# ymartin101/RTS

Hardware: AMD Instinct MI355X
Metric: Mrays/s (primary+bounces) & ms/pulse, 100k-tri scene (higher is better)
Workload: dtype f64

## Files before the change

include/rts_amd.h:

```cpp
#ifndef RTS_AMD_H
#define RTS_AMD_H

#include <stdint.h>
#include "rts_prd.h"

#ifdef __cplusplus
extern "C" {
#endif

typedef struct RtsContext* RtsHandle;

enum {
    RTS_OK = 0,
    RTS_ERR_INVALID = 1,
    RTS_ERR_NO_DEVICE = 2,
    RTS_ERR_HIP = 3,
    RTS_ERR_UNSUPPORTED = 4,
    RTS_ERR_CAPACITY = 5,
    RTS_ERR_IO = 6
};

typedef struct RtsParams {
    uint32_t width;
    uint32_t max_refl;
    uint32_t max_refr;
    uint32_t interpolate_smooth;
    int32_t device;
    uint32_t flags;
} RtsParams;

#define RTS_FLAG_KEEP_ALL_RAYS 1u
#define RTS_FLAG_DEVICE_BUILD 4u
#define RTS_FLAG_HOST_BUILD 16u
#define RTS_FLAG_NO_PREFILTER 8u
#define RTS_FLAG_NO_HORIZON 32u
#define RTS_FLAG_COUNT_TRAVERSAL 2u

typedef struct RtsMesh {
    const uint32_t* triangles;
    const double* vertices;
    const double* normals;
    uint32_t n_triangles, n_vertices, n_normals;
    uint32_t reserved;
    double refl_coeff;
    double refr_index;
} RtsMesh;

typedef struct RtsTargetMotion {
    double position[3];
    double velocity[3];
    double rotation[9];
    int32_t has_rotation;
    int32_t reserved;
} RtsTargetMotion;

typedef struct RtsReceiverSphere {
    double centre[3];
    double radius;
    double min_theta, max_theta, min_phi, max_phi;
} RtsReceiverSphere;

typedef struct RtsPulse {
    double ray_origin[3];
    double tx_span[3];
    double tx_dir[2];
    uint64_t ray_first;
    uint64_t ray_count;
    const RtsTargetMotion* motion;
    uint32_t interleave_tile, interleave_parts, interleave_part, reserved;
} RtsPulse;
#define RTS_INTERLEAVE_LIST 0xffffffffu

typedef struct RtsStats {
    uint64_t rays;
    uint64_t segments;
    uint64_t shaded;
    uint64_t received;
    uint64_t node_visits;
    uint64_t tri_tests;
    uint32_t n_prims, n_nodes;
    float ms_scene;
    float ms_trace;
    float ms_compact;
    float ms_aggregate;
    uint32_t bvh_rebuilt;
    uint32_t stack_overflows;
    uint64_t walked_segments;
    uint32_t coop_tiles;
    uint32_t cost_records_dropped;
} RtsStats;

typedef struct RtsResponse {
    uint64_t ray;
    int32_t rx;
    uint32_t n;
    double power, delay, doppler, phase;
} RtsResponse;

#define RTS_MAX_DEPTH 16
typedef struct RtsGroup {
    int32_t rx;
    uint32_t direct;
    int32_t path[RTS_MAX_DEPTH];
    uint64_t min_ray;
    double n, sum_sqrt_power, sum_delay, sum_phase, sum_doppler;
} RtsGroup;

int rts_create(const RtsParams* params, RtsHandle* out);
int rts_destroy(RtsHandle h);
const char* rts_last_error(void);
const char* rts_build_id(void);
int rts_bind_host_to_device(int device, int* numa_node);
int rts_device_count(int* n);

int rts_set_scene(RtsHandle h, const RtsMesh* meshes, uint32_t n_targets);
int rts_set_receivers(RtsHandle h, const RtsReceiverSphere* rx, uint32_t n_rx);
int rts_share_scene(RtsHandle dst, RtsHandle src);
typedef struct RtsSceneInfo {
    uint32_t n_targets, n_prims, n_nodes, n_leaves;
    uint32_t handles_sharing;
    uint32_t builder;
    double build_ms;
    uint64_t shared_device_bytes;
    uint64_t handle_device_bytes;
    uint64_t version_bytes;
    uint64_t horizon_bytes;
} RtsSceneInfo;
int rts_scene_info(RtsHandle h, RtsSceneInfo* out);
int rts_get_horizon(RtsHandle h, float* out, uint32_t capacity_prims);

int rts_trace_pulse(RtsHandle h, const RtsPulse* pulse);

int rts_reserve(RtsHandle h, uint64_t n_rays);
int rts_trace_pulse_begin(RtsHandle h, const RtsPulse* pulse);
int rts_trace_pulse_end(RtsHandle h);
int rts_link_handles(RtsHandle a, RtsHandle b);
int rts_get_stats(RtsHandle h, RtsStats* out);
int rts_get_block_timeline(RtsHandle h, double* out, uint32_t n);

int rts_get_lane_stats(RtsHandle h, uint64_t* out3);
int rts_get_walk_stats(RtsHandle h, uint64_t* out, uint32_t n);
int rts_received_count(RtsHandle h, uint64_t* count);
int rts_get_received(RtsHandle h, struct PerRayData* rays, int32_t* paths, double* rcs_angles, uint64_t* slots,
                     uint64_t capacity);

int rts_received_prefetch(RtsHandle h);
int rts_received_view(RtsHandle h, const struct PerRayData** rays, const int32_t** paths, const double** rcs_angles, const uint64_t** slots,
                      uint64_t* count);
int rts_finalise_values(RtsHandle h, const double* power, const double* doppler, uint64_t count);
int rts_aggregated_view(RtsHandle h, const double** power, const double** doppler, const double** delay, const double** phase,
                        const int32_t** path_match, uint64_t* count);

int rts_get_all_rays(RtsHandle h, struct PerRayData* results, int32_t* targ_intersect, double* rcs_angle,
                     int32_t* hit_prim, float* hit_t, uint64_t capacity);

int rts_finalise_uniform(RtsHandle h, const double* rcs_per_target, double wavelength, double gt, double gr,
                         double carrier, double cspeed);

int rts_trace_pulse_end_uniform(RtsHandle h, const double* rcs_per_target, double wavelength, double gt, double gr,
                                double carrier, double cspeed, int32_t cube_pulse, uint64_t recv_index_base);

#define RTS_PATTERN_CONSTANT 0u
#define RTS_PATTERN_SEPARABLE 1u
#define RTS_PATTERN_GRID 2u
#define RTS_PATTERN_ABS_U 1u
#define RTS_PATTERN_ABS_V 2u
#define RTS_PATTERN_MAX_AXIS 65536u
#define RTS_PATTERN_MAX_GRID 4194304u
typedef struct RtsPattern {
    uint32_t kind;
    uint32_t flags;
    uint32_t n_u, n_v;
    double scale;
    const double* u_samples;
    const double* u_values;
    const double* v_samples;
    const double* v_values;
    double u0, du, v0, dv;
    const double* grid;
    uint64_t reserved[2];
} RtsPattern;
typedef struct RtsPatternPulse {
    double wavelength, carrier, cspeed;
    const double* rx_position;
    const double* rx_rotation;
} RtsPatternPulse;
int rts_set_patterns(RtsHandle h, const RtsPattern* tx, const RtsPattern* rx, uint32_t n_rx, const RtsPattern* rcs,
                     uint32_t n_targets);
int rts_finalise_patterns(RtsHandle h, const RtsPatternPulse* pulse);
int rts_trace_pulse_end_patterns(RtsHandle h, const RtsPatternPulse* pulse, int32_t cube_pulse, uint64_t recv_index_base);
int rts_pattern_eval(const RtsPattern* p, const double* u, const double* v, uint32_t n, double* out);

#define RTS_BASE_USE_ROWS 0xffffffffffffffffULL
int rts_aggregate(RtsHandle h, double cspeed, double carrier, uint64_t recv_index_base);
int rts_group_count(RtsHandle h, uint32_t* count);
int rts_get_groups(RtsHandle h, RtsGroup* groups, uint32_t capacity);
int rts_get_aggregated(RtsHandle h, struct PerRayData* rays, double* delay, double* phase, int32_t* path_match,
                       uint64_t capacity);

int rts_merge_groups(const RtsGroup* in, uint32_t n_in, uint32_t depth, RtsGroup* out, uint32_t* n_out);
int rts_groups_to_responses(const RtsGroup* groups, uint32_t n_groups, RtsResponse* out, uint32_t capacity,
                            uint32_t* n_out);

typedef struct RtsCubeParams {
    uint32_t n_rx, n_pulses, n_bins, reserved;
    double t0, dt;
} RtsCubeParams;
int rts_cube_attach(RtsHandle h, const RtsCubeParams* params, void* device_ptr);
int rts_cube_accumulate(RtsHandle h, uint32_t pulse_index, double cspeed, double carrier);
int rts_cube_get(RtsHandle h, double* host_out, uint64_t capacity_doubles);
int rts_cube_accumulate_paths(RtsHandle h, uint32_t pulse_index);
int rts_cube_doppler(RtsHandle h, uint32_t n_fft, void* device_out);
// ... 413 lines not shown
```

rts_amd/_lib.py:

```python
import ctypes as C
import os
import subprocess

import numpy as np

_HERE = os.path.dirname(os.path.abspath(__file__))
LIB_PATH = os.environ.get("RTS_AMD_LIB", os.path.join(_HERE, "librts_amd.so"))
CSRC = os.path.join(_HERE, "csrc")

RTS_OK, RTS_ERR_INVALID, RTS_ERR_NO_DEVICE, RTS_ERR_HIP, RTS_ERR_UNSUPPORTED, RTS_ERR_CAPACITY, RTS_ERR_IO = range(7)
RTS_FLAG_KEEP_ALL_RAYS = 1
RTS_FLAG_COUNT_TRAVERSAL = 2
RTS_FLAG_DEVICE_BUILD = 4
RTS_FLAG_HOST_BUILD = 16
RTS_FLAG_NO_PREFILTER = 8
RTS_FLAG_NO_HORIZON = 32
RTS_MAX_DEPTH = 16
RTS_BASE_USE_ROWS = 0xffffffffffffffff

PRD_DTYPE = np.dtype({
    "names": ["rayLength", "refrIndex", "reflDepth", "refrDepth", "maxRayIndex", "rayDirection",
              "firstHitPoint", "prevHitPoint", "power", "doppler", "received", "end"],
    "formats": ["<f8", ("<f8", 2), "<u4", "<u4", "<u4", ("<f8", 3), ("<f8", 3), ("<f8", 3), "<f8", "<f8", "<i4", "u1"],
    "offsets": [0, 16, 32, 36, 40, 48, 72, 96, 120, 128, 136, 140],
    "itemsize": 144,
})


class RtsParams(C.Structure):
    _fields_ = [("width", C.c_uint32), ("max_refl", C.c_uint32), ("max_refr", C.c_uint32),
                ("interpolate_smooth", C.c_uint32), ("device", C.c_int32), ("flags", C.c_uint32)]


class RtsMesh(C.Structure):
    _fields_ = [("triangles", C.c_void_p), ("vertices", C.c_void_p), ("normals", C.c_void_p),
                ("n_triangles", C.c_uint32), ("n_vertices", C.c_uint32), ("n_normals", C.c_uint32),
                ("reserved", C.c_uint32), ("refl_coeff", C.c_double), ("refr_index", C.c_double)]


class RtsTargetMotion(C.Structure):
    _fields_ = [("position", C.c_double * 3), ("velocity", C.c_double * 3), ("rotation", C.c_double * 9),
                ("has_rotation", C.c_int32), ("reserved", C.c_int32)]


class RtsReceiverSphere(C.Structure):
    _fields_ = [("centre", C.c_double * 3), ("radius", C.c_double), ("min_theta", C.c_double),
                ("max_theta", C.c_double), ("min_phi", C.c_double), ("max_phi", C.c_double)]


class RtsPulse(C.Structure):
    _fields_ = [("ray_origin", C.c_double * 3), ("tx_span", C.c_double * 3), ("tx_dir", C.c_double * 2),
                ("ray_first", C.c_uint64), ("ray_count", C.c_uint64), ("motion", C.POINTER(RtsTargetMotion)),
                ("interleave_tile", C.c_uint32), ("interleave_parts", C.c_uint32), ("interleave_part", C.c_uint32), ("reserved", C.c_uint32)]


class RtsCubeParams(C.Structure):
    _fields_ = [("n_rx", C.c_uint32), ("n_pulses", C.c_uint32), ("n_bins", C.c_uint32), ("reserved", C.c_uint32),
                ("t0", C.c_double), ("dt", C.c_double)]


class RtsPlanItem(C.Structure):
    _fields_ = [("pulse", C.c_uint32), ("interleave_tile", C.c_uint32), ("interleave_parts", C.c_uint32), ("interleave_part", C.c_uint32),
                ("ray_first", C.c_uint64), ("ray_count", C.c_uint64)]


RTS_SHARD_PULSES, RTS_SHARD_RAYS, RTS_SHARD_PULSES_WHOLE = 0, 1, 2


RTS_PATTERN_CONSTANT, RTS_PATTERN_SEPARABLE, RTS_PATTERN_GRID = 0, 1, 2
RTS_PATTERN_ABS_U, RTS_PATTERN_ABS_V = 1, 2
RTS_PATTERN_MAX_AXIS, RTS_PATTERN_MAX_GRID = 65536, 4194304


class RtsPattern(C.Structure):
    _fields_ = [("kind", C.c_uint32), ("flags", C.c_uint32), ("n_u", C.c_uint32), ("n_v", C.c_uint32), ("scale", C.c_double),
                ("u_samples", C.c_void_p), ("u_values", C.c_void_p), ("v_samples", C.c_void_p), ("v_values", C.c_void_p),
                ("u0", C.c_double), ("du", C.c_double), ("v0", C.c_double), ("dv", C.c_double), ("grid", C.c_void_p),
                ("reserved", C.c_uint64 * 2)]


class RtsPatternPulse(C.Structure):
    _fields_ = [("wavelength", C.c_double), ("carrier", C.c_double), ("cspeed", C.c_double),
                ("rx_position", C.c_void_p), ("rx_rotation", C.c_void_p)]


RTS_RENDER_RAYS, RTS_RENDER_PATHS = 0, 1
RTS_RENDER_DOPPLER = 1
RTS_WAVEFORM_MAX_SAMPLES, RTS_WAVEFORM_MAX_TAPS, RTS_COMPRESS_MAX_BINS = 4096, 64, 8192


class RtsWaveform(C.Structure):
    _fields_ = [("samples", C.c_void_p), ("n_samples", C.c_uint32), ("taps", C.c_uint32), ("reserved", C.c_uint64 * 2)]


RTS_CFAR_CA, RTS_CFAR_GO, RTS_CFAR_SO = 0, 1, 2
RTS_CFAR_LOCAL_MAX = 1
RTS_CFAR_MAX_HALF, RTS_CFAR_DEFAULT_MAX_DETECTIONS = 16, 65536


# ... 186 lines not shown

class RtsEigParams(C.Structure):
    _fields_ = [("n", C.c_uint32), ("reserved0", C.c_uint32), ("device_cov", C.c_void_p), ("reserved", C.c_uint64 * 2)]


class RtsDoaScanParams(C.Structure):
    _fields_ = [("n", C.c_uint32), ("first_vector", C.c_uint32), ("m", C.c_uint32), ("flags", C.c_uint32), ("n_dirs", C.c_uint64),
                ("g", C.c_void_p), ("device_steering", C.c_void_p), ("device_vectors", C.c_void_p), ("reserved", C.c_uint64 * 2)]


assert C.sizeof(RtsEigParams) == 32 and C.sizeof(RtsDoaScanParams) == 64


class RtsSceneInfo(C.Structure):
    _fields_ = [("n_targets", C.c_uint32), ("n_prims", C.c_uint32), ("n_nodes", C.c_uint32), ("n_leaves", C.c_uint32),
                ("handles_sharing", C.c_uint32), ("builder", C.c_uint32), ("build_ms", C.c_double),
                ("shared_device_bytes", C.c_uint64), ("handle_device_bytes", C.c_uint64), ("version_bytes", C.c_uint64),
                ("horizon_bytes", C.c_uint64)]


class RtsStats(C.Structure):
    _fields_ = [("rays", C.c_uint64), ("segments", C.c_uint64), ("shaded", C.c_uint64), ("received", C.c_uint64),
                ("node_visits", C.c_uint64), ("tri_tests", C.c_uint64), ("n_prims", C.c_uint32), ("n_nodes", C.c_uint32),
                ("ms_scene", C.c_float), ("ms_trace", C.c_float), ("ms_compact", C.c_float), ("ms_aggregate", C.c_float),
                ("bvh_rebuilt", C.c_uint32), ("stack_overflows", C.c_uint32), ("walked_segments", C.c_uint64), ("coop_tiles", C.c_uint32), ("cost_records_dropped", C.c_uint32)]


RESPONSE_DTYPE = np.dtype([("ray", "<u8"), ("rx", "<i4"), ("n", "<u4"), ("power", "<f8"), ("delay", "<f8"),
                           ("doppler", "<f8"), ("phase", "<f8")])
GROUP_DTYPE = np.dtype([("rx", "<i4"), ("direct", "<u4"), ("path", "<i4", (RTS_MAX_DEPTH,)), ("min_ray", "<u8"),
                        ("n", "<f8"), ("sum_sqrt_power", "<f8"), ("sum_delay", "<f8"), ("sum_phase", "<f8"),
                        ("sum_doppler", "<f8")])
assert RESPONSE_DTYPE.itemsize == 48 and GROUP_DTYPE.itemsize == 120


def is_stale():
    if not os.path.exists(LIB_PATH):
        return True
    try:
        return build_id() != source_hash()
    except (OSError, AttributeError):
        return True


def source_hash():
    import hashlib
    names = sorted(f for f in os.listdir(CSRC) if f.endswith((".hip", ".cpp", ".h")) and f != "rts_build_id.h")
    h = hashlib.sha256()
    for path in [os.path.join(CSRC, f) for f in names] + [os.path.join(_HERE, "..", "include", f) for f in ("rts_amd.h", "rts_prd.h")]:
        with open(path, "rb") as f:
            h.update(f.read())
    return h.hexdigest()[:16]


def build_id(path=None):
    L = C.CDLL(path or LIB_PATH)
    L.rts_build_id.restype = C.c_char_p
    return L.rts_build_id().decode()


def require_built():
    if not os.path.exists(LIB_PATH):
        raise SystemExit("librts_amd.so is not built: run `python __graft_entry__.py` (or make -C rts_amd/csrc) first")
    if "RTS_AMD_LIB" not in os.environ:
        have, want = build_id(), source_hash()
        if have != want:
            raise SystemExit("librts_amd.so is stale: built from sources %s, the tree is %s -- run `python __graft_entry__.py` first" % (have, want))


def build(force=False, verbose=False):
    if force or is_stale():
        cmd = ["make", "-C", CSRC, "-j", "5"] + ([] if verbose else ["-s"])
        subprocess.check_call(cmd)
    return LIB_PATH


_lib = None

EXPORTS = ["rts_create", "rts_destroy", "rts_last_error", "rts_device_count", "rts_set_scene", "rts_share_scene", "rts_scene_info", "rts_set_receivers",
           "rts_trace_pulse", "rts_reserve", "rts_trace_pulse_begin", "rts_trace_pulse_end", "rts_link_handles", "rts_get_stats", "rts_get_block_timeline", "rts_received_count", "rts_get_received", "rts_get_all_rays",
           "rts_finalise_uniform", "rts_trace_pulse_end_uniform", "rts_aggregate", "rts_group_count", "rts_get_groups", "rts_get_aggregated",
           "rts_merge_groups", "rts_groups_to_responses", "rts_kernel_wrapper", "rts_vertex_rotation",
           "rts_rotation_matrix", "rts_rect_mesh", "rts_sphere_mesh", "rts_file_mesh", "rts_rx_sphere", "rts_get_bvh",
           "rts_build_id", "rts_bind_host_to_device", "rts_get_lane_stats", "rts_get_walk_stats", "rts_get_horizon", "rts_self_test_math", "rts_cube_attach", "rts_cube_accumulate", "rts_cube_get", "rts_cube_accumulate_paths", "rts_cube_doppler", "rts_cube_doppler_get", "rts_plan_cpi", "rts_cube_reduce", "rts_kernel_wrapper_on",
           "rts_received_prefetch", "rts_received_view", "rts_finalise_values", "rts_aggregated_view", "rts_build_hierarchy_host",
           "rts_tile_records_get", "rts_tile_records_set", "rts_deal_tiles", "rts_set_tile_list",
           "rts_set_patterns", "rts_finalise_patterns", "rts_trace_pulse_end_patterns", "rts_pattern_eval",
           "rts_cube_set_waveform", "rts_cube_render", "rts_cube_compress", "rts_waveform_eval",
           "rts_cube_add_noise", "rts_noise_eval", "rts_cube_add_sources", "rts_sources_eval", "rts_cube_detect", "rts_cube_detections_get",
           "rts_cube_detect_os", "rts_cfar_os_alpha", "rts_cfar_os_eval",
           "rts_cube_plots", "rts_cube_plots_get", "rts_plots_eval",
           "rts_cube_track", "rts_cube_tracks_get", "rts_cube_tracks_set", "rts_cube_tracks_reset", "rts_cube_track_rounds", "rts_tracks_eval",
           "rts_cube_tbd_step", "rts_cube_tbd_extract", "rts_cube_tbd_tracks_get", "rts_cube_tbd_paths_get", "rts_cube_tbd_merit_get", "rts_cube_tbd_ring_get",
           "rts_cube_tbd_info", "rts_cube_tbd_reset", "rts_tbd_step_eval", "rts_tbd_extract_eval",
           "rts_cube_backproject", "rts_cube_image_get", "rts_backproject_eval",
           "rts_cube_spectrogram", "rts_cube_spectrogram_get", "rts_stft_eval", "rts_window_make",
           "rts_cube_render_beat", "rts_beat_eval", "rts_cube_range_transform", "rts_cube_range_get", "rts_range_eval",
           "rts_cube_beamform", "rts_cube_beam_get", "rts_beamform_eval", "rts_steering_make",
           "rts_cube_covariance", "rts_cube_covariance_get", "rts_covariance_eval", "rts_cube_mvdr", "rts_cube_mvdr_get", "rts_mvdr_eval",
           "rts_cube_st_covariance", "rts_st_covariance_eval", "rts_cube_st_apply", "rts_cube_st_get", "rts_st_apply_eval", "rts_st_steering_make",
           "rts_cube_eig", "rts_cube_eig_get", "rts_eig_eval", "rts_cube_doa_scan", "rts_cube_doa_get", "rts_doa_scan_eval", "rts_doa_weights", "rts_source_count"]


def lib():
    global _lib
    if _lib is not None:
        return _lib
    if not os.path.exists(LIB_PATH):
        raise RuntimeError("librts_amd.so is not built (run `make -C rts_amd/csrc` or __graft_entry__.build()); "
                           "there is no Python/CPU fallback for the RTS hot path")
    L = C.CDLL(LIB_PATH)
    vp, u32, u64, dbl, i32 = C.c_void_p, C.c_uint32, C.c_uint64, C.c_double, C.c_int32
    L.rts_last_error.restype = C.c_char_p
    sig = {
        "rts_create": [C.POINTER(RtsParams), C.POINTER(vp)],
        "rts_destroy": [vp],
        "rts_device_count": [C.POINTER(C.c_int)],
        "rts_set_scene": [vp, C.POINTER(RtsMesh), u32],
        "rts_share_scene": [vp, vp],
        "rts_scene_info": [vp, C.POINTER(RtsSceneInfo)],
        "rts_set_receivers": [vp, C.POINTER(RtsReceiverSphere), u32],
        "rts_trace_pulse": [vp, C.POINTER(RtsPulse)],
        "rts_reserve": [vp, u64],
        "rts_trace_pulse_begin": [vp, C.POINTER(RtsPulse)],
        "rts_get_block_timeline": [vp, vp, u32],
        "rts_trace_pulse_end": [vp],
        "rts_link_handles": [vp, vp],
        "rts_get_stats": [vp, C.POINTER(RtsStats)],
        "rts_received_count": [vp, C.POINTER(u64)],
        "rts_get_received": [vp, vp, vp, vp, vp, u64],
        "rts_get_all_rays": [vp, vp, vp, vp, vp, vp, u64],
        "rts_finalise_uniform": [vp, vp, dbl, dbl, dbl, dbl, dbl],
        "rts_build_hierarchy_host": [vp, vp, u32, dbl, vp, u32, vp, u32, C.POINTER(u32), C.POINTER(u32), C.POINTER(C.c_int32)],
        "rts_received_prefetch": [vp],
        "rts_received_view": [vp, C.POINTER(vp), C.POINTER(vp), C.POINTER(vp), C.POINTER(vp), C.POINTER(u64)],
        "rts_finalise_values": [vp, vp, vp, u64],
        "rts_aggregated_view": [vp, C.POINTER(vp), C.POINTER(vp), C.POINTER(vp), C.POINTER(vp), C.POINTER(vp), C.POINTER(u64)],
        "rts_aggregate": [vp, dbl, dbl, u64],
        "rts_trace_pulse_end_uniform": [vp, vp, dbl, dbl, dbl, dbl, dbl, C.c_int32, u64],
        "rts_group_count": [vp, C.POINTER(u32)],
        "rts_get_groups": [vp, vp, u32],
        "rts_get_aggregated": [vp, vp, vp, vp, vp, u64],
        "rts_merge_groups": [vp, u32, u32, vp, C.POINTER(u32)],
        "rts_groups_to_responses": [vp, u32, vp, u32, C.POINTER(u32)],
        "rts_kernel_wrapper": [vp, vp, C.c_uint, C.c_uint, C.c_uint, C.c_uint, dbl, dbl, vp, vp, vp, vp, vp, vp],
        "rts_kernel_wrapper_on": [vp, vp, vp, C.c_uint, C.c_uint, C.c_uint, C.c_uint, dbl, dbl, vp, vp, vp, vp, vp, vp],
        "rts_vertex_rotation": [vp, u32, C.c_float, C.c_float, C.c_float],
        "rts_rotation_matrix": [C.c_float, C.c_float, C.c_float, vp],
        "rts_rect_mesh": [C.c_float] * 6 + [vp, vp, vp],
        "rts_sphere_mesh": [u32, C.c_float, C.c_float, C.c_float, C.c_float, vp, C.POINTER(u32), vp, C.POINTER(u32), vp],
        "rts_file_mesh": [C.c_char_p, C.c_char_p, C.c_float, C.c_float, C.c_float, vp, vp, vp, C.POINTER(u32)],
        "rts_rx_sphere": [vp, dbl, dbl, dbl, dbl, dbl, C.POINTER(RtsReceiverSphere)],
        "rts_get_bvh": [vp, vp, vp, vp, u32, u32, vp],
        "rts_cube_attach": [vp, C.POINTER(RtsCubeParams), vp],
        "rts_cube_accumulate": [vp, u32, dbl, dbl],
        "rts_cube_get": [vp, vp, u64], "rts_get_lane_stats": [vp, vp], "rts_get_walk_stats": [vp, vp, C.c_uint32], "rts_get_horizon": [vp, vp, u32], "rts_bind_host_to_device": [C.c_int, C.POINTER(C.c_int)],
        "rts_cube_accumulate_paths": [vp, u32], "rts_cube_doppler": [vp, u32, vp], "rts_cube_doppler_get": [vp, vp, u64],
        "rts_plan_cpi": [u64, u32, u32, u32, u32, u32, u32, vp, u32, C.POINTER(u32)],
        "rts_cube_reduce": [vp, u32, C.c_int],
        "rts_tile_records_get": [vp, vp, u32], "rts_tile_records_set": [vp, vp, u32], "rts_deal_tiles": [vp, u32, u64, u32, u32, vp, vp], "rts_set_tile_list": [vp, u32, vp, u32],
        "rts_self_test_math": [vp, vp, vp, vp, vp, vp, vp, vp, u32],
        "rts_set_patterns": [vp, C.POINTER(RtsPattern), C.POINTER(RtsPattern), u32, C.POINTER(RtsPattern), u32],
        "rts_finalise_patterns": [vp, C.POINTER(RtsPatternPulse)],
        "rts_trace_pulse_end_patterns": [vp, C.POINTER(RtsPatternPulse), C.c_int32, u64],
        "rts_pattern_eval": [C.POINTER(RtsPattern), vp, vp, u32, vp],
        "rts_cube_set_waveform": [vp, C.POINTER(RtsWaveform)],
        "rts_cube_render": [vp, u32, u32, u32, C.c_double, C.c_double],
        "rts_cube_compress": [vp, u32, u32],
        "rts_waveform_eval": [C.POINTER(RtsWaveform), vp, u32, vp],
        "rts_cube_add_noise": [vp, u32, u32, C.c_double, u64],
        "rts_noise_eval": [u64, vp, u32, C.c_double, vp],
        "rts_cube_add_sources": [vp, C.POINTER(RtsSourceParams)],
        "rts_sources_eval": [C.POINTER(RtsCubeParams), C.POINTER(RtsSourceParams), vp],
        "rts_cube_detect": [vp, C.POINTER(RtsCfarParams), vp, u32],
        "rts_cube_detections_get": [vp, vp, u32, C.POINTER(u32)],
        "rts_cube_detect_os": [vp, C.POINTER(RtsCfarOsParams), vp, u32],
        "rts_cfar_os_alpha": [u32, u32, C.c_double, C.POINTER(C.c_double)],
        "rts_cfar_os_eval": [C.POINTER(RtsCubeParams), vp, u32, C.POINTER(RtsCfarOsParams), vp, u32, C.POINTER(u32)],
        "rts_cube_plots": [vp, C.POINTER(RtsPlotParams)],
        "rts_cube_plots_get": [vp, vp, u32, C.POINTER(u32)],
        "rts_plots_eval": [C.POINTER(RtsCubeParams), vp, u32, u32, C.POINTER(RtsPlotParams), vp, u32, C.POINTER(u32)],
        "rts_cube_track": [vp, C.POINTER(RtsTrackParams), C.c_double],
        "rts_cube_tracks_get": [vp, vp, u32, C.POINTER(u32), C.POINTER(u64)],
        "rts_cube_tracks_set": [vp, vp, u32, u64, C.c_double],
        "rts_cube_tracks_reset": [vp],
        "rts_cube_track_rounds": [vp, C.POINTER(u32)],
        "rts_tracks_eval": [C.POINTER(RtsTrackParams), vp, u32, u64, C.c_double, vp, u32, vp, u32, C.POINTER(u32), C.POINTER(u64)],
        "rts_cube_tbd_step": [vp, C.POINTER(RtsTbdParams), C.c_double, vp, u32],
        "rts_cube_tbd_extract": [vp, C.POINTER(RtsTbdExtractParams)],
        "rts_cube_tbd_tracks_get": [vp, vp, u32, C.POINTER(u32)],
        "rts_cube_tbd_paths_get": [vp, vp, u32],
        "rts_cube_tbd_merit_get": [vp, vp, u64],
        "rts_cube_tbd_ring_get": [vp, vp, vp, u32, C.POINTER(u32)],
        "rts_cube_tbd_info": [vp, C.POINTER(u32 * 4), C.POINTER(u64)],
        "rts_cube_tbd_reset": [vp],
        "rts_tbd_step_eval": [C.POINTER(RtsCubeParams), vp, u32, vp, C.POINTER(RtsTbdParams), C.c_double, vp, vp, vp],
        "rts_tbd_extract_eval": [C.POINTER(RtsCubeParams), u32, C.POINTER(RtsTbdParams), vp, vp, vp, u32, C.POINTER(RtsTbdExtractParams), vp, vp, u32, C.POINTER(u32)],
        "rts_cube_backproject": [vp, C.POINTER(RtsImageParams), vp],
        "rts_cube_image_get": [vp, vp, u64],
        "rts_backproject_eval": [C.POINTER(RtsCubeParams), vp, C.POINTER(RtsImageParams), vp],
        "rts_cube_spectrogram": [vp, C.POINTER(RtsStftParams), vp, C.POINTER(u32)],
        "rts_cube_spectrogram_get": [vp, vp, u64],
        "rts_stft_eval": [C.POINTER(RtsCubeParams), vp, C.POINTER(RtsStftParams), vp, C.POINTER(u32)],
        "rts_window_make": [u32, u32, vp],
        "rts_cube_render_beat": [vp, u32, C.POINTER(RtsBeatParams), C.c_double, C.c_double],
        "rts_beat_eval": [C.POINTER(RtsCubeParams), C.POINTER(RtsBeatParams), vp, u32, u32, vp],
        "rts_cube_range_transform": [vp, C.POINTER(RtsRangeParams), vp],
        "rts_cube_range_get": [vp, vp, u64],
        "rts_range_eval": [C.POINTER(RtsCubeParams), vp, C.POINTER(RtsRangeParams), vp],
        "rts_cube_beamform": [vp, C.POINTER(RtsBeamParams), vp],
        "rts_cube_beam_get": [vp, vp, u64],
        "rts_beamform_eval": [C.POINTER(RtsCubeParams), vp, u32, C.POINTER(RtsBeamParams), vp],
        "rts_steering_make": [vp, u32, vp, u32, C.c_double, vp, vp],
        "rts_cube_covariance": [vp, C.POINTER(RtsCovParams), vp],
        "rts_cube_covariance_get": [vp, vp, u64],
        "rts_covariance_eval": [C.POINTER(RtsCubeParams), vp, u32, C.POINTER(RtsCovParams), vp],
        "rts_cube_mvdr": [vp, C.POINTER(RtsMvdrParams), vp],
        "rts_cube_mvdr_get": [vp, vp, u64],
        "rts_mvdr_eval": [vp, u32, C.POINTER(RtsMvdrParams), vp],
        "rts_cube_st_covariance": [vp, C.POINTER(RtsStCovParams), vp],
        "rts_st_covariance_eval": [C.POINTER(RtsCubeParams), vp, u32, C.POINTER(RtsStCovParams), vp],
        "rts_cube_st_apply": [vp, C.POINTER(RtsStApplyParams), vp],
        "rts_cube_st_get": [vp, vp, u64],
        "rts_st_apply_eval": [C.POINTER(RtsCubeParams), vp, u32, C.POINTER(RtsStApplyParams), vp],
        "rts_st_steering_make": [vp, u32, u32, vp, u32, u32, vp, vp],
        "rts_cube_eig": [vp, C.POINTER(RtsEigParams), vp, vp],
        "rts_cube_eig_get": [vp, vp, vp, u64, u64],
        "rts_eig_eval": [vp, u32, vp, vp, C.POINTER(u32)],
        "rts_cube_doa_scan": [vp, C.POINTER(RtsDoaScanParams), vp],
        "rts_cube_doa_get": [vp, vp, u64],
        "rts_doa_scan_eval": [vp, vp, u32, u32, vp, u64, u32, vp],
        "rts_doa_weights": [u32, vp, u32, u32, C.c_double, C.POINTER(u32), C.POINTER(u32), vp, C.POINTER(u32)],
        "rts_source_count": [vp, u32, u64, u32, C.POINTER(u32)],
    }
    for name, args in sig.items():
        fn = getattr(L, name, None)
        if fn is None:
            continue
        fn.argtypes = args
# ... 19 lines not shown
```

rts_amd/api.py:

```python
import ctypes as C

import numpy as np

from . import _lib as L
from ._lib import PRD_DTYPE, RESPONSE_DTYPE, GROUP_DTYPE, check, ptr


def rect_mesh(w, h, d, yaw=0.0, pitch=0.0, roll=0.0):
    v = np.zeros((8, 3)); t = np.zeros((12, 3), np.uint32); n = np.zeros((12, 3))
    check(L.lib().rts_rect_mesh(w, h, d, yaw, pitch, roll, ptr(v), ptr(t), ptr(n)))
    return v, t, n


def sphere_mesh(subdivisions, radius, yaw=0.0, pitch=0.0, roll=0.0):
    nv = C.c_uint32(); nt = C.c_uint32()
    check(L.lib().rts_sphere_mesh(subdivisions, radius, yaw, pitch, roll, None, C.byref(nv), None, C.byref(nt), None))
    v = np.zeros((nv.value, 3)); t = np.zeros((nt.value, 3), np.uint32); n = np.zeros((nv.value, 3))
    check(L.lib().rts_sphere_mesh(subdivisions, radius, yaw, pitch, roll, ptr(v), C.byref(nv), ptr(t), C.byref(nt), ptr(n)))
    return v, t, n


def file_mesh(v_file, n_file, yaw=0.0, pitch=0.0, roll=0.0):
    nt = C.c_uint32(0)
    check(L.lib().rts_file_mesh(v_file.encode(), n_file.encode(), yaw, pitch, roll, None, None, None, C.byref(nt)))
# ... 600 lines not shown


def doa_weights(method, values, n_sources=0, loading=0.0):
    values = np.ascontiguousarray(np.asarray(values, np.float64).ravel())
    first, m, flags = C.c_uint32(0), C.c_uint32(0), C.c_uint32(0); g = np.zeros(max(len(values), 1), np.float64)
    check(L.lib().rts_doa_weights(_DOA_METHODS.get(method, method), ptr(values), len(values), int(n_sources), float(loading),
                                  C.byref(first), C.byref(m), ptr(g), C.byref(flags)))
    return first.value, g[:m.value].copy(), bool(flags.value & L.RTS_DOA_INVERSE)


def source_count(values, K, criterion="mdl"):
    values = np.ascontiguousarray(np.asarray(values, np.float64).ravel())
    k = C.c_uint32(0)
    check(L.lib().rts_source_count(ptr(values), len(values), int(K), {"aic": L.RTS_DOA_AIC, "mdl": L.RTS_DOA_MDL}.get(criterion, criterion), C.byref(k)))
    return k.value


def _st_cov_params(taps, source, first, count, first_bin, n_bins, skip, device_in, n_rows_in):
    c = _cov_params(source, first, count, first_bin, n_bins, skip, device_in, n_rows_in)
    p = L.RtsStCovParams()
    for name in ("source", "n_rows_in", "first_row", "n_rows", "first_bin", "n_bins", "skip_first_bin", "skip_n_bins", "device_in"):
        setattr(p, name, getattr(c, name))
    p.n_taps = int(taps)
    return p


def st_covariance_eval(inp, taps, first=0, count=None, first_bin=0, n_bins=None, skip=None):
    inp = np.ascontiguousarray(np.asarray(inp, np.complex128))
    n_rx, rows, nb = inp.shape
    q = L.RtsCubeParams(n_rx, rows, nb, 0, 0.0, 1.0)
    p = _st_cov_params(taps, "cube", first, count, first_bin, n_bins, skip, None, 0)
    D = n_rx * max(int(taps), 0)
    out = np.zeros((D, D), np.complex128)
    check(L.lib().rts_st_covariance_eval(C.byref(q), ptr(inp.view(np.float64)), rows, C.byref(p), ptr(out.view(np.float64))))
    return out


def _st_apply_params(weights, taps, n_rx, source, first, count, power, device_in, n_rows_in):
    w = np.ascontiguousarray(np.asarray(weights, np.complex128))
    if w.ndim != 2 or w.shape[1] != int(taps) * n_rx:
        raise ValueError("st_apply: weights of shape %s for %d taps of %d receivers ([n_filters][taps n_rx])" % (w.shape, taps, n_rx))
    p = L.RtsStApplyParams()
    p.n_filters, p.source, p.n_taps = w.shape[0], _BEAM_SOURCES.get(source, source), int(taps)
    p.first_row, p.n_rows, p.n_rows_in = int(first), int(count or 0), int(n_rows_in)
    p.flags = L.RTS_BEAM_POWER if power else 0
    p.weights = ptr(w.view(np.float64))
    p.device_in = device_in if device_in else None
    return p, w


def st_apply_eval(inp, weights, taps, first=0, count=None, power=False):
    inp = np.ascontiguousarray(np.asarray(inp, np.complex128))
    n_rx, rows, nb = inp.shape
    q = L.RtsCubeParams(n_rx, rows, nb, 0, 0.0, 1.0)
    p, keep = _st_apply_params(weights, taps, n_rx, "cube", first, count, power, None, 0)
    out = _beam_out(p.n_filters, (p.n_rows if p.n_rows else rows - p.first_row) - p.n_taps + 1, nb, power, False)
    check(L.lib().rts_st_apply_eval(C.byref(q), ptr(inp.view(np.float64)), rows, C.byref(p), ptr(out.view(np.float64))))
    return out


def st_steering(spatial, dopplers, taps, tap_taper=None):
    a = np.ascontiguousarray(np.atleast_2d(np.asarray(spatial, np.complex128)))
    f = np.ascontiguousarray(np.asarray(dopplers, np.float64).ravel())
    t = None if tap_taper is None else np.ascontiguousarray(np.asarray(tap_taper, np.float64).ravel())
    if t is not None and len(t) != int(taps):
        raise ValueError("st_steering: a taper of %d values for %d taps" % (len(t), taps))
    out = np.zeros((a.shape[0] * len(f), max(int(taps), 0) * a.shape[1]), np.complex128)
    check(L.lib().rts_st_steering_make(ptr(a.view(np.float64)), a.shape[1], a.shape[0], ptr(f), len(f), int(taps), ptr(t), ptr(out.view(np.float64))))
    return out


def device_count():
    n = C.c_int(0)
    rc = L.lib().rts_device_count(C.byref(n))
    return n.value if rc == 0 else 0


import os as _os
_PY_LAP = {} if _os.environ.get("RTS_PY_LAP") == "1" else None


class Tracer:

    def __init__(self, width, max_refl, max_refr=0, smooth=True, device=0, keep_all=False, count_traversal=False, device_build=None, pre_filter=True, horizon=True):
        p = L.RtsParams(width, max_refl, max_refr, 1 if smooth else 0, device,
                        (L.RTS_FLAG_KEEP_ALL_RAYS if keep_all else 0) | (L.RTS_FLAG_COUNT_TRAVERSAL if count_traversal else 0) |
                        (0 if device_build is None else (L.RTS_FLAG_DEVICE_BUILD if device_build else L.RTS_FLAG_HOST_BUILD)) |
                         (0 if pre_filter else L.RTS_FLAG_NO_PREFILTER) | (0 if horizon else L.RTS_FLAG_NO_HORIZON))
        self.h = C.c_void_p()
        check(L.lib().rts_create(C.byref(p), C.byref(self.h)))
        self.width = width; self.max_refl = max_refl; self.depth = max_refl + (2 if max_refr else 0)
        self.n_targets = 0; self.keep_all = keep_all; self.device = device
        self._keep = []

    def close(self):
        if self.h:
            L.lib().rts_destroy(self.h); self.h = C.c_void_p()

    def __del__(self):
        try:
            self.close()
        except Exception:
            pass

    def set_scene(self, meshes):
        arr = (L.RtsMesh * max(len(meshes), 1))()
        keep = []
        for i, m in enumerate(meshes):
            t = np.ascontiguousarray(m["tris"], np.uint32); v = np.ascontiguousarray(m["verts"], np.float64)
            n = np.ascontiguousarray(m["normals"], np.float64)
            keep += [t, v, n]
            arr[i] = L.RtsMesh(t.ctypes.data, v.ctypes.data, n.ctypes.data, t.shape[0], v.shape[0], n.shape[0], 0,
                               float(m.get("refl_coeff", 1.0)), float(m.get("refr_index", 1.0)))
        check(L.lib().rts_set_scene(self.h, arr, len(meshes)))
        self.n_targets = len(meshes)

    def horizon(self, n_prims):
        out = np.zeros((int(n_prims), 2), np.float32)
        check(L.lib().rts_get_horizon(self.h, ptr(out), int(n_prims)))
        return out

    def walk_stats(self):
        ls = (C.c_uint64 * 11)()
        check(L.lib().rts_get_walk_stats(self.h, ls, 11))
        return [int(v) for v in ls]

    def share_scene(self, other):
        check(L.lib().rts_share_scene(self.h, other.h))
        self.n_targets = other.n_targets

    def scene_info(self):
        s = L.RtsSceneInfo()
        check(L.lib().rts_scene_info(self.h, C.byref(s)))
        return {k: getattr(s, k) for k, _ in L.RtsSceneInfo._fields_}

    def set_receivers(self, spheres):
        arr = (L.RtsReceiverSphere * max(len(spheres), 1))()
        for i, s in enumerate(spheres):
            arr[i] = L.RtsReceiverSphere((C.c_double * 3)(*s["centre"]), s["radius"], s["minTheta"], s["maxTheta"],
                                         s["minPhi"], s["maxPhi"])
        check(L.lib().rts_set_receivers(self.h, arr, len(spheres)))

    def trace(self, origin, tx_span, tx_dir, motion=None, ray_first=0, ray_count=0, want_stats=True, interleave=None):
        check(L.lib().rts_trace_pulse(self.h, C.byref(self._pulse(origin, tx_span, tx_dir, motion, ray_first, ray_count, interleave))))
        return self.stats() if want_stats else None

    def reserve(self, n_rays=0):
        check(L.lib().rts_reserve(self.h, n_rays))

    def trace_begin(self, origin, tx_span, tx_dir, motion=None, ray_first=0, ray_count=0, interleave=None):
        if _PY_LAP is None:
            check(L.lib().rts_trace_pulse_begin(self.h, C.byref(self._pulse(origin, tx_span, tx_dir, motion, ray_first, ray_count, interleave))))
            return
        import time
        t0 = time.perf_counter(); p = self._pulse(origin, tx_span, tx_dir, motion, ray_first, ray_count, interleave)
        t1 = time.perf_counter(); f = L.lib().rts_trace_pulse_begin
        t2 = time.perf_counter(); rc = f(self.h, C.byref(p))
        t3 = time.perf_counter(); check(rc)
        t4 = time.perf_counter()
        for k, v in zip(("marshal", "lookup", "call", "check"), (t1 - t0, t2 - t1, t3 - t2, t4 - t3)):
            _PY_LAP[k] = _PY_LAP.get(k, 0.0) + v
        _PY_LAP["n"] = _PY_LAP.get("n", 0) + 1

    def block_timeline(self):
        out = np.zeros(9, np.float64)
        check(L.lib().rts_get_block_timeline(self.h, ptr(out), 9))
        return dict(zip(("start_first", "start_p50", "start_last", "end_first", "end_p10", "end_p50", "end_p90", "end_last", "blocks"), out.tolist()))

    def trace_end(self):
        check(L.lib().rts_trace_pulse_end(self.h))

    def tile_records_get(self):
        n = (self.width ** 3 + 63) // 64
        out = np.zeros(n, np.uint32)
        check(L.lib().rts_tile_records_get(self.h, ptr(out), n))
        return out

    def tile_records_set(self, records):
        r = np.ascontiguousarray(records, np.uint32)
        check(L.lib().rts_tile_records_set(self.h, ptr(r), r.shape[0]))

    def set_tile_list(self, tile, tile_ids):
        ids = np.ascontiguousarray(tile_ids, np.uint32)
        check(L.lib().rts_set_tile_list(self.h, tile, ptr(ids) if ids.shape[0] else None, ids.shape[0]))

    def link(self, other):
        check(L.lib().rts_link_handles(self.h, other.h))

    def _pulse(self, origin, tx_span, tx_dir, motion, ray_first, ray_count, interleave):
        p = self._pulse_struct = getattr(self, "_pulse_struct", None) or L.RtsPulse()
        p.ray_origin[:] = origin; p.tx_span[:] = tx_span; p.tx_dir[:] = tx_dir
        p.ray_first = ray_first; p.ray_count = ray_count
        p.interleave_tile, p.interleave_parts, p.interleave_part = interleave if interleave is not None else (0, 0, 0)
        if motion is not None:
            assert len(motion) == self.n_targets
            marr = getattr(self, "_motion_arr", None)
            if marr is None or len(marr) != max(len(motion), 1):
                marr = self._motion_arr = (L.RtsTargetMotion * max(len(motion), 1))()
                self._motion_ptr = C.cast(marr, C.POINTER(L.RtsTargetMotion))
            for i, m in enumerate(motion):
                q = marr[i]
                q.position[:] = m["position"]; q.velocity[:] = m.get("velocity", (0.0, 0.0, 0.0))
                rot = m.get("rotation")
                if rot is not None:
                    q.rotation[:] = np.asarray(rot, np.float64).reshape(9).tolist(); q.has_rotation = 1
                else:
                    q.has_rotation = 0
# ... 471 lines not shown
```

rts_amd/csrc/rts_api.hip:

```cpp
#include <cmath>
#include <cstdarg>
#include <cstdio>
#include <cstring>
#include <cstdlib>
#include <dlfcn.h>
#include <algorithm>
#include <chrono>
#include <map>
#include <mutex>
#include <stdexcept>
#include <string>
#include "rts_internal.h"
#include "rts_raygen.h"
#include <atomic>

static thread_local char g_err[1024] = "";
void rts_set_error(const char* fmt, ...) { va_list ap; va_start(ap, fmt); vsnprintf(g_err, sizeof(g_err), fmt, ap); va_end(ap); }
extern "C" const char* rts_last_error(void) { return g_err; }
#include "rts_build_id.h"
extern "C" const char* rts_build_id(void) { return RTS_SOURCE_HASH; }

#include <dirent.h>
#include <sched.h>
extern "C" int rts_bind_host_to_device(int device, int* numa_node)
// ... 393 lines not shown
    if (p->motion) {
        if (!c->motion_valid || memcmp(c->motion.data(), p->motion, sizeof(RtsTargetMotion)*n_targets) != 0) moved = true;
        if (n_targets) memcpy(c->motion.data(), p->motion, sizeof(RtsTargetMotion)*n_targets);
        c->motion_valid = true;
    } else if (!c->motion_valid) {
        for (auto& m : c->motion) memset(&m, 0, sizeof(m));
        c->motion_valid = true; moved = true;
    }
    c->stats.bvh_rebuilt = 0;
    *moved_out = moved;
    if (!moved) return RTS_OK;
    for (uint32_t t = 0; t < n_targets; t++) for (int k = 0; k < 3; k++)
        if (!std::isfinite(c->motion[t].position[k]) || !std::isfinite(c->motion[t].velocity[k])) { rts_set_error("rts_trace_pulse: target %u has a non-finite position/velocity", t); return RTS_ERR_INVALID; }
    if (n_targets > 256) { rts_set_error("rts_trace_pulse: more than 256 targets"); return RTS_ERR_UNSUPPORTED; }
    RtsTargetDev* td = c->pin.p->td;
    for (uint32_t t = 0; t < n_targets; t++) {
        td[t].reflCoeff = c->scene->meshes[t].refl_coeff; td[t].vx = c->motion[t].velocity[0]; td[t].vy = c->motion[t].velocity[1]; td[t].vz = c->motion[t].velocity[2];
        td[t].tri_base = c->scene->meshes[t].tri_base; td[t].perface_normals = c->scene->meshes[t].perface ? 1u : 0u; td[t].refrIndex = c->scene->meshes[t].refr_index;
        int rc = fill_target_placement(c, t, td[t]); if (rc != RTS_OK) { c->bvh_valid = false; c->motion_valid = false; return rc; }
        c->pin.p->motion[t] = c->motion[t];
    }
    c->bvh_valid = false;
    return RTS_OK;
}

static void pulse_fill_constants(RtsContext* c, const RtsPulse& p, const RtsRayRange& r, bool pre_filter)
{
    const uint32_t W = c->params.width;
    RtsLaunchConsts& lc = c->last_lc; memset(&lc, 0, sizeof(lc));
    fill_launch_constants(lc, p, W);
    lc.ray_first = r.first; lc.W = W; lc.il_tile = r.il_tile; lc.il_parts = r.il_parts; lc.il_part = r.il_part; lc.il_list = r.il_list ? c->d_il_list.p : nullptr;
    const RtsDivMagic d = rts_div_magic(W); lc.w_magic = d.magic; lc.w_more = d.more;
    fill_mask_frame(lc, pre_filter && c->scene->n_prims > 0);
    for (int k = 0; k < 3; k++) { lc.f_bs[k] = (float)(&lc.bsx)[k]; lc.f_st[k] = (float)(&lc.stx)[k]; }
    for (int i = 0; i < 3; i++) for (int j = 0; j < 3; j++) lc.f_m[3 * i + j] = (float)(lc.rot1[3 * i] * lc.rot[j] + lc.rot1[3 * i + 1] * lc.rot[3 + j] + lc.rot1[3 * i + 2] * lc.rot[6 + j]);
}

static uint32_t* pulse_mask_words(const RtsContext* c) { return c->d_tile_ctr.p + RTS_ZERO_WORDS; }

static int pulse_upload_and_fill(RtsContext* c, bool moved)
{
    const uint32_t n_targets = (uint32_t)c->scene->meshes.size(); const RtsMaskFrame& mask = c->last_lc.mask;
    c->pin.p->lc = c->last_lc;
    RTS_HIP(hipMemcpyAsync(c->d_params.p, &c->pin.p->lc, moved && n_targets ? offsetof(RtsPinned, td) + sizeof(RtsTargetDev) * n_targets : sizeof(RtsLaunchConsts), hipMemcpyHostToDevice, c->stream));
    { int rc = rts_zero_block_reserve(c); if (rc != RTS_OK) return rc; }
    RTS_HIP(hipMemsetAsync(c->d_tile_ctr.p, 0, sizeof(uint32_t) * (((RTS_ZERO_WORDS + (mask.n ? (size_t)mask.n * mask.n / 32u + 1u : 0u)) + 63u) & ~(size_t)63u), c->stream));
    return RTS_OK;
}

static int pulse_scene_place(RtsContext* c, bool moved)
{
    { int rc = rts_scene_place(c, c->last_lc, moved, pulse_mask_words(c)); if (rc != RTS_OK) return rc; }
    if (moved) { RTS_STAGE(c, "scene_place"); c->bvh_valid = true; c->stats.bvh_rebuilt = 1; }
    RTS_HIP(hipEventRecord(c->ev[1], c->stream));
    return RTS_OK;
}

static int pulse_args_and_buffers(RtsContext* c, RtsPulseLaunch& L)
{
    RtsTraceArgs& a = L.a; memset(&a, 0, sizeof(a));
    const uint32_t n = L.n; const RtsLaunchConsts& lc = c->last_lc; hipStream_t st = c->stream;
    a.lc = c->p_lc;
    a.ray_first = L.r.first; a.n_rays = n; a.W = c->params.width; a.max_refl = c->params.max_refl; a.smooth = c->params.interpolate_smooth ? 1u : 0u;
    a.n_prims = c->scene->n_prims; a.n_targets = (uint32_t)c->scene->meshes.size(); a.n_rx = c->n_rx; a.keep_all = L.keep_all ? 1u : 0u;
    a.max_refr = c->params.max_refr; a.rows = a.max_refr ? c->params.max_refl + 3 : 1;
    if ((uint64_t)n * rts_chains(a.max_refr) > 0xfffffff0ULL) { rts_set_error("rts_trace_pulse: rays x chains exceeds 2^32"); return RTS_ERR_UNSUPPORTED; }
    a.total_threads = L.grid * RTS_BLOCK;
    a.coop_spread = c->tune.coop_spread;
    a.coop_walk_steps_lo = std::min(c->tune.coop_walk_steps_lo, c->tune.coop_walk_steps);
    a.coop_walk_steps = c->tune.coop_walk_steps; a.coop_min_cost = c->tune.coop_walk_steps ? std::min<uint32_t>(c->tune.coop_floor, 1875u) : 0u;
    a.slab_threads = a.total_threads + rts_coop_threads(c);
    const RtsLaunchSizes sz = rts_launch_sizes(n, a.total_threads, a.total_threads, rts_coop_threads(c), (uint64_t)L.grid + c->tune.coop_grid_max, a.max_refl, a.max_refr, L.keep_all);
    { int rc = rts_launch_buffers_reserve(c, sz); if (rc != RTS_OK) return rc; }
    if (L.keep_all) {
        rts_fill_i32(st, c->d_hit_prim.p, -2, sz.hit_prim - 1);
        RTS_HIP(hipMemsetAsync(c->d_hit_t.p, 0, sizeof(float) * (sz.hit_t - 1), st));
    }
    a.pmask = lc.mask.n ? pulse_mask_words(c) : nullptr; a.pre_filter = L.pre_filter ? 1u : 0u;
    a.nodes4 = c->scene->d_nodes4.p; a.nodes4v = c->tune.node_versions ? c->scene->d_nodes4v.p : nullptr; a.stack_lds = c->tune.stack_lds; a.leaves = c->d_leaves.p; a.tri_nidx = c->scene->d_tri_nidx.p; a.normals = c->d_normals_world.p;
    a.targets = c->p_targets; a.rx = c->d_rx.p;
    a.recv_records = c->d_recv.p; a.all_records = c->d_all.p; a.counters = c->p_counters; a.block_counters = c->d_block_counters.p; a.dir_hist = c->d_dir_hist.p;
    a.hit_prim = c->d_hit_prim.p; a.hit_t = c->d_hit_t.p; a.stack_ovf = c->d_stack_ovf.p; a.child = c->d_child.p;
    a.rx_window_screen = c->tune.rx_window_screen ? 1u : 0u;
    a.horizon = (c->params.flags & RTS_FLAG_NO_HORIZON) ? 0u : 1u;
    a.coop_versions = c->tune.coop_versions ? 1u : 0u;
    a.tile_ctr = c->d_tile_ctr.p;
    return RTS_OK;
}

static int pulse_tile_order(RtsContext* c, RtsPulseLaunch& L)
{
    RtsTraceArgs& a = L.a;
    const RtsLaunchShape s = rts_launch_shape(L.n, L.r.first, L.r.il_tile, L.r.il_parts, L.r.il_part, rts_lattice_size(c->params.width));
    const uint32_t n_tiles = s.n_tiles, resident_waves = L.grid * (RTS_BLOCK / RTS_WTILE);
    a.batch_dead = s.aligned ? (uint32_t)c->tune.batch_dead : 0u;
    if (!(c->tune.tile_lpt && s.aligned && n_tiles > resident_waves)) { c->tile_cost_pending = false; c->tile_last_valid = false; return RTS_OK; }
    { int rc = rts_hist_ensure(c, s.n_hist); if (rc != RTS_OK) return rc; }
    if (c->tile_cost_pending || c->hist->any) {
        c->coop_big_now = (L.r.il_parts > 1 && !L.shared_gpu && c->tune.coop_big_part > c->tune.coop_big) ? c->tune.coop_big_part : c->tune.coop_big;
        int rc = rts_tile_order_build(c, c->tile_cost_sig, c->tile_cost_pending, s.sig, n_tiles, resident_waves); if (rc != RTS_OK) return rc;
        a.tile_order = c->d_tile_order.p; a.tile_head = c->tune.coop_frac > 0.0 ? c->d_tile_ctr.p + RTS_OFF_HEAD + 2 : nullptr; a.tile_head_all = a.tile_head; c->hist->any = true;
        a.tile_live = c->d_tile_ctr.p + RTS_OFF_LIVE;
    }
    const bool merged_all = c->tile_cost_pending && rts_wave_tiles(c->tile_cost_sig[0]) >= n_tiles && c->d_tile_cost.cap >= n_tiles;
    RTS_HIP(c->d_tile_cost.reserve(n_tiles));
    if (!merged_all) RTS_HIP(hipMemsetAsync(c->d_tile_cost.p, 0, sizeof(uint32_t) * n_tiles, c->stream));
    a.tile_cost = c->d_tile_cost.p;
    c->tile_cost_pending = true; memcpy(c->tile_cost_sig, s.sig, sizeof(s.sig)); memcpy(c->tile_last_sig, s.sig, sizeof(s.sig)); c->tile_last_valid = true;
    return RTS_OK;
}

static int pulse_timelines(RtsContext* c, RtsPulseLaunch& L)
{
    const size_t blocks2 = (size_t)L.grid * 2;
    RtsLaunchTuning lt; if (L.count_trav) rts_tuning_read(&lt, rts_env);
    L.tl_path = lt.timeline;
    L.cnt_tl = blocks2 + 2 * (size_t)rts_wave_tiles(L.n);
    c->tl_blocks = 0;
    const size_t words = L.tl_path ? L.cnt_tl + 1 : (!L.count_trav && c->tune.timeline_blocks) ? blocks2 + 1 : 0;
    if (!words) return RTS_OK;
    RTS_HIP(c->d_timeline.reserve(words)); RTS_HIP(hipMemsetAsync(c->d_timeline.p, 0, sizeof(unsigned long long) * words, c->stream)); L.a.timeline = c->d_timeline.p;
    if (!L.tl_path) c->tl_blocks = L.grid;
    return RTS_OK;
}

static int pulse_launch(RtsContext* c, RtsPulseLaunch& L)
{
    RtsTraceArgs& a = L.a; hipStream_t st = c->stream;
    RTS_STAGE(c, "pre-trace");
    c->tstream_now = (c->tune.trace_own_stream && !L.shared_gpu && c->gate->refs.load() == 1) ? st : c->tstream;
    if (c->tstream_now != st) {
        RTS_HIP(hipEventRecord(c->ev[8], st));
        RTS_HIP(hipStreamWaitEvent(c->tstream_now, c->ev[8], 0));
    }
    RTS_HIP(hipEventRecord(c->ev[2], c->tstream_now));
    unsigned coop_grid = 0;
    if (a.tile_head) {
        if (c->hist->head_hint_valid) c->n_head_hint = c->hist->head_hint;
        const bool grouped = a.nodes4v && a.coop_versions && !L.keep_all && !a.max_refr;
        coop_grid = rts_coop_grid(c->n_head_hint, grouped, c->tune.coop_grid_max);
        if (coop_grid == 0) a.tile_head = nullptr;
        c->last_args = a;
    }
    if (c->tune.debug_coop) fprintf(stderr, "[rts] launch: n_rays %u grid %u head hint %u coop grid %u walk-steps threshold %u min cost %u order %d\n", L.n, L.grid, c->n_head_hint, coop_grid, a.coop_walk_steps, a.coop_min_cost, a.tile_order ? 1 : 0);
    c->last_coop_grid = coop_grid;
    int rc = rts_trace_launch(c, a, L.count_trav, coop_grid);
    if (rc != RTS_OK) return rc;
    RTS_STAGE(c, "k_trace");
    RTS_HIP(hipEventRecord(c->ev[3], c->tstream_now));
    if (c->tstream_now != st) RTS_HIP(hipStreamWaitEvent(st, c->ev[3], 0));
    return RTS_OK;
}

static int pulse_timeline_dump(RtsContext* c, const RtsPulseLaunch& L)
{
    RTS_HIP(hipStreamSynchronize(c->stream));
    std::vector<unsigned long long> h(L.cnt_tl + 2);
    h[0] = L.grid; h[1] = rts_wave_tiles(L.n);
    RTS_HIP(hipMemcpy(h.data() + 2, c->d_timeline.p, sizeof(unsigned long long) * L.cnt_tl, hipMemcpyDeviceToHost));
    if (FILE* f = fopen(L.tl_path, "wb")) { fwrite(h.data(), sizeof(unsigned long long), h.size(), f); fclose(f); }
    return RTS_OK;
}

extern "C" int rts_trace_pulse_begin(RtsHandle c, const RtsPulse* p)
{
    if (!c) { rts_set_error("null handle"); return RTS_ERR_INVALID; }
    RtsLapTimer lt(c);
// ... 781 lines not shown
```

rts_amd/csrc/rts_bvh.hip:

```cpp
#include <cstring>
#include <hip/hip_runtime.h>
#include "rts_internal.h"
#include "rts_ray_ops.h"

__device__ __forceinline__ void place_one(const double* __restrict__ local, double* __restrict__ world, const uint32_t* __restrict__ targ_of,
                                          const RtsTargetMotion* __restrict__ motion, uint32_t i, bool add_position)
{
    const RtsTargetMotion m = motion[targ_of[i]];
    double x = local[3*i], y = local[3*i+1], z = local[3*i+2];
    if (m.has_rotation) {
        double rx = 0.0, ry = 0.0, rz = 0.0;
        rx += m.rotation[0] * x; rx += m.rotation[1] * y; rx += m.rotation[2] * z;
        ry += m.rotation[3] * x; ry += m.rotation[4] * y; ry += m.rotation[5] * z;
        rz += m.rotation[6] * x; rz += m.rotation[7] * y; rz += m.rotation[8] * z;
        x = rx; y = ry; z = rz;
    }
    if (add_position) { x += m.position[0]; y += m.position[1]; z += m.position[2]; }
    world[3*i] = x; world[3*i+1] = y; world[3*i+2] = z;
}
__global__ void k_place(const double* __restrict__ v_local, double* __restrict__ v_world, const uint32_t* __restrict__ v_targ, uint32_t n_verts,
                        const double* __restrict__ n_local, double* __restrict__ n_world, const uint32_t* __restrict__ n_targ, uint32_t n_normals,
                        const RtsTargetMotion* __restrict__ motion)
{
    const uint32_t i = blockIdx.x * blockDim.x + threadIdx.x;
// ... 5 lines not shown
static_assert(RTS_MASK_N / 32u <= RTS_MASK_TILE_WORDS, "a band of the mask tile holds at least one whole row");
struct RtsMaskLds { uint32_t tile[RTS_MASK_TILE_WORDS]; int box[4]; };
__device__ __forceinline__ void rts_mask_mark(RtsMaskLds& S, const bool have, const double (&p)[9], const double ox, const double oy, const double oz, const RtsMaskFrame& f, uint32_t* __restrict__ mask)
{
    uint32_t* flag = mask + (size_t)f.n * f.n / 32u;
    if (threadIdx.x == 0) { S.box[0] = 0x7fffffff; S.box[1] = 0x7fffffff; S.box[2] = -1; S.box[3] = -1; }
    __syncthreads();
    int iu0 = 0, iu1 = -1, iv0 = 0, iv1 = -1;
    if (have) {
        double u[3], v[3]; bool finite = true, front = true;
        for (int k = 0; k < 3; k++) {
            const double px = p[3*k] - ox, py = p[3*k + 1] - oy, pz = p[3*k + 2] - oz;
            finite = finite && isfinite(px) && isfinite(py) && isfinite(pz);
            const double w = px * (double)f.bx + py * (double)f.by + pz * (double)f.bz;
            front = front && (w > 0.0) && (w * w > 1.0e-6 * (px*px + py*py + pz*pz));
            u[k] = (px * (double)f.ux + py * (double)f.uy + pz * (double)f.uz) / w;
            v[k] = (px * (double)f.vx + py * (double)f.vy + pz * (double)f.vz) / w;
        }
        if (finite && !front) atomicExch(flag, 1u);
        if (finite && front) {
            const double fu0 = (fmin(fmin(u[0], u[1]), u[2]) - (double)f.u0) * (double)f.inv_du, fu1 = (fmax(fmax(u[0], u[1]), u[2]) - (double)f.u0) * (double)f.inv_du;
            const double fv0 = (fmin(fmin(v[0], v[1]), v[2]) - (double)f.v0) * (double)f.inv_dv, fv1 = (fmax(fmax(v[0], v[1]), v[2]) - (double)f.v0) * (double)f.inv_dv;
            const double nn = (double)f.n;
            if (!(fu1 < -1.0 || fv1 < -1.0 || fu0 > nn || fv0 > nn)) {
                iu0 = (int)fmax(floor(fu0) - 1.0, 0.0); iu1 = (int)fmin(floor(fu1) + 1.0, nn - 1.0);
                iv0 = (int)fmax(floor(fv0) - 1.0, 0.0); iv1 = (int)fmin(floor(fv1) + 1.0, nn - 1.0);
                if ((long long)(iu1 - iu0 + 1) * (long long)(iv1 - iv0 + 1) > RTS_MASK_MAX_CELLS) { atomicExch(flag, 1u); iu1 = iu0 - 1; }
            }
        }
    }
    const bool any = iu1 >= iu0 && iv1 >= iv0;
    {
        int b0 = any ? iu0 : 0x7fffffff, b1 = any ? iv0 : 0x7fffffff, b2 = any ? iu1 : -1, b3 = any ? iv1 : -1;
        for (int d = warpSize / 2; d > 0; d >>= 1) {
            b0 = min(b0, __shfl_xor(b0, d)); b1 = min(b1, __shfl_xor(b1, d)); b2 = max(b2, __shfl_xor(b2, d)); b3 = max(b3, __shfl_xor(b3, d));
        }
        if ((threadIdx.x & (warpSize - 1)) == 0 && b2 >= 0) { atomicMin(&S.box[0], b0); atomicMin(&S.box[1], b1); atomicMax(&S.box[2], b2); atomicMax(&S.box[3], b3); }
    }
    __syncthreads();
    if (S.box[2] < 0) return;
    const int W0 = S.box[0] >> 5, V0 = S.box[1], TW = (S.box[2] >> 5) - W0 + 1, TH = S.box[3] - V0 + 1;
    const int band = RTS_MASK_TILE_WORDS / TW;
    for (int b0 = 0; b0 < TH; b0 += band) {
        const int B0 = V0 + b0, bh = min(band, TH - b0), nw = TW * bh;
        if (b0) __syncthreads();
        for (int w = threadIdx.x; w < nw; w += blockDim.x) S.tile[w] = 0u;
        __syncthreads();
        if (any) {
            for (int iv = max(iv0, B0); iv <= min(iv1, B0 + bh - 1); iv++) {
                for (int w0 = iu0 >> 5; w0 <= (iu1 >> 5); w0++) {
                    const int lo = max(iu0, w0 << 5) & 31, hi = min(iu1, (w0 << 5) + 31) & 31;
                    const uint32_t bits = (hi == 31 ? 0xffffffffu : ((1u << (hi + 1)) - 1u)) & ~((1u << lo) - 1u);
                    atomicOr(&S.tile[(iv - B0) * TW + (w0 - W0)], bits);
                }
            }
        }
        __syncthreads();
        for (int w = threadIdx.x; w < nw; w += blockDim.x) {
            const uint32_t bits = S.tile[w];
            if (bits) atomicOr(&mask[((size_t)(B0 + w / TW) * f.n >> 5) + (size_t)(W0 + w % TW)], bits);
        }
    }
}

__device__ __forceinline__ void place_vertex(const double* __restrict__ local, const RtsTargetMotion& m, uint32_t i, double* __restrict__ out3)
{
    double x = local[3*(size_t)i], y = local[3*(size_t)i+1], z = local[3*(size_t)i+2];
    if (m.has_rotation) {
        double rx = 0.0, ry = 0.0, rz = 0.0;
        rx += m.rotation[0] * x; rx += m.rotation[1] * y; rx += m.rotation[2] * z;
        ry += m.rotation[3] * x; ry += m.rotation[4] * y; ry += m.rotation[5] * z;
        rz += m.rotation[6] * x; rz += m.rotation[7] * y; rz += m.rotation[8] * z;
        x = rx; y = ry; z = rz;
    }
    x += m.position[0]; y += m.position[1]; z += m.position[2];
    out3[0] = x; out3[1] = y; out3[2] = z;
}
template <bool LEAVES, bool MASK, bool PLACE = false>
__global__ void __launch_bounds__(256) k_leaves(const uint32_t* __restrict__ order, const uint32_t* __restrict__ tri_vidx, const double* __restrict__ verts,
                                                const uint32_t* __restrict__ prim_targ, RtsLeafTri* __restrict__ leaves, uint32_t n,
                                                double ox, double oy, double oz, RtsMaskFrame f, uint32_t* __restrict__ mask,
                                                const RtsTargetMotion* __restrict__ motion = nullptr, uint32_t prim_blocks = 0, const double* __restrict__ n_local = nullptr,
                                                double* __restrict__ n_world = nullptr, const uint32_t* __restrict__ n_targ = nullptr, uint32_t n_normals = 0,
                                                const float* __restrict__ horizon = nullptr)
{
    __shared__ __attribute__((aligned(16))) uint32_t s_raw[MASK ? sizeof(RtsMaskLds) / 4 : 1];
    if (PLACE && blockIdx.x >= prim_blocks) {
        const uint32_t q = (blockIdx.x - prim_blocks) * blockDim.x + threadIdx.x;
        if (q < n_normals) place_one(n_local, n_world, n_targ, motion, q, false);
        return;
    }
    const uint32_t i = blockIdx.x * blockDim.x + threadIdx.x;
    double p[9] = {0, 0, 0, 0, 0, 0, 0, 0, 0};
    if (i < n) {
        const uint32_t g = order[i];
        const uint32_t a = tri_vidx[3*(size_t)g], b = tri_vidx[3*(size_t)g+1], c = tri_vidx[3*(size_t)g+2];
        if (PLACE) {
            const RtsTargetMotion m = motion[prim_targ[g]];
            place_vertex(verts, m, a, p); place_vertex(verts, m, b, p + 3); place_vertex(verts, m, c, p + 6);
        } else {
        p[0] = verts[3*(size_t)a]; p[1] = verts[3*(size_t)a+1]; p[2] = verts[3*(size_t)a+2];
        p[3] = verts[3*(size_t)b]; p[4] = verts[3*(size_t)b+1]; p[5] = verts[3*(size_t)b+2];
        p[6] = verts[3*(size_t)c]; p[7] = verts[3*(size_t)c+1]; p[8] = verts[3*(size_t)c+2];
        }
        if (LEAVES) {
            dvec3 e0, e1, nn;
            tri_terms(mk3(p[0], p[1], p[2]), mk3(p[3], p[4], p[5]), mk3(p[6], p[7], p[8]), e0, e1, nn);
            RtsLeafTri L;
            L.p0x = p[0]; L.p0y = p[1]; L.p0z = p[2]; L.e0x = e0.x; L.e0y = e0.y; L.e0z = e0.z; L.e1x = e1.x; L.e1y = e1.y; L.e1z = e1.z;
            L.nx = nn.x; L.ny = nn.y; L.nz = nn.z;
            L.prim = g; L.targ = prim_targ[g]; L.hz[0] = horizon ? horizon[2*(size_t)g] : 1.0f; L.hz[1] = horizon ? horizon[2*(size_t)g+1] : 1.0f;
            leaves[g] = L;
        }
    }
    if (MASK) rts_mask_mark(*reinterpret_cast<RtsMaskLds*>(s_raw), i < n, p, ox, oy, oz, f, mask);
}

static inline unsigned blocks_for(size_t n, unsigned bs) { return (unsigned)((n + bs - 1) / bs); }

int rts_scene_place(RtsContext* c, const RtsLaunchConsts& lc, bool place, uint32_t* pmask)
{
    hipStream_t st = c->stream;
    const RtsMaskFrame& f = lc.mask;
    const bool mask = f.n != 0;
    const RtsScene* sc = c->scene;
    if (place && sc->n_prims) {
        const unsigned gp = blocks_for(sc->n_prims, 256), gn = blocks_for(sc->n_normals, 256);
        if (mask) k_leaves<true, true, true><<<gp + gn, 256, 0, st>>>(sc->d_prim_order.p, sc->d_tri_vidx.p, sc->d_verts_local.p, sc->d_prim_targ.p, c->d_leaves.p, sc->n_prims, lc.ox, lc.oy, lc.oz, f, pmask,
                                                                     c->p_motion, gp, sc->d_normals_local.p, c->d_normals_world.p, sc->d_norm_targ.p, sc->n_normals, sc->d_horizon.p);
        else k_leaves<true, false, true><<<gp + gn, 256, 0, st>>>(sc->d_prim_order.p, sc->d_tri_vidx.p, sc->d_verts_local.p, sc->d_prim_targ.p, c->d_leaves.p, sc->n_prims, lc.ox, lc.oy, lc.oz, f, nullptr,
                                                                  c->p_motion, gp, sc->d_normals_local.p, c->d_normals_world.p, sc->d_norm_targ.p, sc->n_normals, sc->d_horizon.p);
        c->verts_world_valid = false;
        RTS_HIP(hipGetLastError());
        return RTS_OK;
    }
    if (place) {
        if (sc->n_verts + sc->n_normals) k_place<<<blocks_for((size_t)sc->n_verts + sc->n_normals, 256), 256, 0, st>>>(sc->d_verts_local.p, c->d_verts_world.p, sc->d_vert_targ.p, sc->n_verts,
                                                                                                                         sc->d_normals_local.p, c->d_normals_world.p, sc->d_norm_targ.p, sc->n_normals, c->p_motion);
        c->verts_world_valid = true;
    } else if (mask) {
        if (!c->verts_world_valid && sc->n_verts) {
            k_place<<<blocks_for((size_t)sc->n_verts, 256), 256, 0, st>>>(sc->d_verts_local.p, c->d_verts_world.p, sc->d_vert_targ.p, sc->n_verts, sc->d_normals_local.p, c->d_normals_world.p, sc->d_norm_targ.p, 0u, c->p_motion);
            c->verts_world_valid = true;
        }
        if (sc->n_prims) k_leaves<false, true><<<blocks_for(sc->n_prims, 256), 256, 0, st>>>(sc->d_prim_order.p, sc->d_tri_vidx.p, c->d_verts_world.p, sc->d_prim_targ.p, nullptr, sc->n_prims, lc.ox, lc.oy, lc.oz, f, pmask);
    }
    RTS_HIP(hipGetLastError());
    return RTS_OK;
}
```

rts_amd/csrc/rts_horizon.hip:

```cpp
#include <cmath>
#include "rts_internal.h"
#include "rts_ray_ops.h"

#define RTS_HZ_BLOCK 64u
#define RTS_HZ_WORK_CAP (1ull << 31)
#define RTS_HZ_SLICES 8u

struct RtsHzPrim { double cx, cy, cz, r, nx, ny, nz, d; };
struct RtsHzBlk { double cx, cy, cz, r; uint32_t tlo, thi; };

__global__ void k_hz_prims(const uint32_t* __restrict__ order, const uint32_t* __restrict__ tri_vidx, const double* __restrict__ verts, const uint32_t* __restrict__ prim_targ,
                           uint32_t n, const RtsHorizonMesh* __restrict__ mesh, uint32_t* __restrict__ mesh_off, RtsHzPrim* __restrict__ hp, double* __restrict__ pv)
{
    const uint32_t i = blockIdx.x * blockDim.x + threadIdx.x;
    if (i >= n) return;
    const uint32_t g = order[i], t = prim_targ[g];
    double p[9];
    for (int k = 0; k < 3; k++) { const uint32_t v = tri_vidx[3 * (size_t)g + k]; for (int a = 0; a < 3; a++) p[3 * k + a] = verts[3 * (size_t)v + a]; }
    for (int k = 0; k < 9; k++) pv[(size_t)i * 9 + k] = p[k];
    dvec3 e0, e1, nn;
    tri_terms(mk3(p[0], p[1], p[2]), mk3(p[3], p[4], p[5]), mk3(p[6], p[7], p[8]), e0, e1, nn);
    const double nl = sqrt(nn.x * nn.x + nn.y * nn.y + nn.z * nn.z);
    const double l0 = sqrt(e0.x * e0.x + e0.y * e0.y + e0.z * e0.z), l1 = sqrt(e1.x * e1.x + e1.y * e1.y + e1.z * e1.z);
    const double e2x = p[6] - p[3], e2y = p[7] - p[4], e2z = p[8] - p[5], l2 = sqrt(e2x * e2x + e2y * e2y + e2z * e2z);
    const double longest = fmax(l0, fmax(l1, l2));
    const bool good = isfinite(nl) && isfinite(longest) && longest > 0.0 && nl / longest >= RTS_HZ_DEGEN * mesh[t].extent;
    if (!good) atomicOr(&mesh_off[t], 1u);
    RtsHzPrim q;
    q.cx = (p[0] + p[3] + p[6]) / 3.0; q.cy = (p[1] + p[4] + p[7]) / 3.0; q.cz = (p[2] + p[5] + p[8]) / 3.0;
    double r2 = 0.0;
    for (int k = 0; k < 3; k++) { const double dx = p[3 * k] - q.cx, dy = p[3 * k + 1] - q.cy, dz = p[3 * k + 2] - q.cz; r2 = fmax(r2, dx * dx + dy * dy + dz * dz); }
    q.r = sqrt(r2) * (1.0 + 1e-12);
    const double inv = good ? 1.0 / nl : 0.0;
    q.nx = nn.x * inv; q.ny = nn.y * inv; q.nz = nn.z * inv; q.d = q.nx * p[0] + q.ny * p[1] + q.nz * p[2];
    hp[i] = q;
}

__global__ void k_hz_blocks(const uint32_t* __restrict__ order, const uint32_t* __restrict__ prim_targ, uint32_t n, uint32_t n_blocks, const RtsHzPrim* __restrict__ hp, RtsHzBlk* __restrict__ hb)
{
    const uint32_t b = blockIdx.x * blockDim.x + threadIdx.x;
    if (b >= n_blocks) return;
    const uint32_t i0 = b * RTS_HZ_BLOCK, i1 = min(n, i0 + RTS_HZ_BLOCK);
    double cx = 0, cy = 0, cz = 0; uint32_t tlo = 0xffffffffu, thi = 0u;
    for (uint32_t i = i0; i < i1; i++) { cx += hp[i].cx; cy += hp[i].cy; cz += hp[i].cz; const uint32_t t = prim_targ[order[i]]; tlo = min(tlo, t); thi = max(thi, t); }
    const double m = 1.0 / (double)(i1 - i0); cx *= m; cy *= m; cz *= m;
    double r = 0.0;
    for (uint32_t i = i0; i < i1; i++) { const double dx = hp[i].cx - cx, dy = hp[i].cy - cy, dz = hp[i].cz - cz; r = fmax(r, sqrt(dx * dx + dy * dy + dz * dz) + hp[i].r); }
    RtsHzBlk o; o.cx = cx; o.cy = cy; o.cz = cz; o.r = isfinite(r) ? r * (1.0 + 1e-12) : INFINITY; o.tlo = tlo; o.thi = thi;
    hb[b] = o;
}

__device__ __forceinline__ double hz_raise(double s, double hmax, double gap, double h0)
{
    if (!(hmax <= h0)) s = (gap > 0.0) ? fmax(s, fmin(1.0, hmax / gap)) : 1.0;
    return s;
}

__global__ void __launch_bounds__(256) k_hz_main(const uint32_t* __restrict__ order, const uint32_t* __restrict__ prim_targ, uint32_t n, uint32_t n_blocks, const RtsHorizonMesh* __restrict__ mesh,
                                                 const uint32_t* __restrict__ mesh_off, const RtsHzPrim* __restrict__ hp, const RtsHzBlk* __restrict__ hb, const double* __restrict__ pv,
                                                 uint32_t* __restrict__ horizon)
{
    const uint32_t i = blockIdx.x * blockDim.x + threadIdx.x, slice = blockIdx.y;
    if (i >= n) return;
    const uint32_t g = order[i], t = prim_targ[g];
    double sp = 0.0, sm = 0.0;
    if (mesh_off[t]) { sp = 1.0; sm = 1.0; }
    else {
        const RtsHzPrim T = hp[i];
        const double h0 = RTS_HZ_H0 * mesh[t].extent, rho = RTS_HZ_RHO * mesh[t].extent;
        for (uint32_t b = slice; b < n_blocks && !(sp >= 1.0 && sm >= 1.0); b += RTS_HZ_SLICES) {
            const RtsHzBlk B = hb[b];
            if (t < B.tlo || t > B.thi) continue;
            const double hc = T.nx * B.cx + T.ny * B.cy + T.nz * B.cz - T.d;
            const double dx = B.cx - T.cx, dy = B.cy - T.cy, dz = B.cz - T.cz;
            const double gap = sqrt(dx * dx + dy * dy + dz * dz) - B.r - T.r - rho;
            if (hz_raise(sp, hc + B.r, gap, h0) <= sp && hz_raise(sm, -hc + B.r, gap, h0) <= sm) continue;
            const uint32_t j0 = b * RTS_HZ_BLOCK, j1 = min(n, j0 + RTS_HZ_BLOCK);
            for (uint32_t j = j0; j < j1; j++) {
                if (j == i || prim_targ[order[j]] != t) continue;
                const RtsHzPrim U = hp[j];
                const double* u = pv + (size_t)j * 9;
                const double a0 = T.nx * u[0] + T.ny * u[1] + T.nz * u[2] - T.d, a1 = T.nx * u[3] + T.ny * u[4] + T.nz * u[5] - T.d, a2 = T.nx * u[6] + T.ny * u[7] + T.nz * u[8] - T.d;
                const double ex = U.cx - T.cx, ey = U.cy - T.cy, ez = U.cz - T.cz;
                const double pg = sqrt(ex * ex + ey * ey + ez * ez) - U.r - T.r - rho;
                sp = hz_raise(sp, fmax(a0, fmax(a1, a2)), pg, h0);
                sm = hz_raise(sm, fmax(-a0, fmax(-a1, -a2)), pg, h0);
            }
        }
    }
    float fp = (float)sp, fm = (float)sm;
    if ((double)fp < sp) fp = __uint_as_float(__float_as_uint(fp) + 1u);
    if ((double)fm < sm) fm = __uint_as_float(__float_as_uint(fm) + 1u);
    atomicMax(&horizon[2 * (size_t)g], __float_as_uint(fminf(fp, 1.0f))); atomicMax(&horizon[2 * (size_t)g + 1], __float_as_uint(fminf(fm, 1.0f)));
}

int rts_horizon_build(RtsContext* c, RtsScene* ns, const RtsSceneFlat& flat)
{
    const uint32_t n = ns->n_prims, n_targets = (uint32_t)ns->meshes.size();
    ns->hz.assign(n_targets, RtsHorizonMesh{0.0, 0.0, 0.0});
    if (!n) return RTS_OK;
    const uint32_t n_blocks = (n + RTS_HZ_BLOCK - 1u) / RTS_HZ_BLOCK;
    std::vector<uint32_t> off(n_targets, 0u);
    for (uint32_t t = 0; t < n_targets; t++) {
        RtsBlasInfo b; rts_mesh_bounds(flat, t, &b);
        double e2 = 0; for (int a = 0; a < 3; a++) e2 += (b.hi[a] - b.lo[a]) * (b.hi[a] - b.lo[a]);
        const double E = std::sqrt(e2);
        ns->hz[t].extent = E; ns->hz[t].h0 = RTS_HZ_H0 * E; ns->hz[t].rho = RTS_HZ_RHO * E;
        if (!(E > 0.0) || !std::isfinite(E) || (unsigned long long)ns->meshes[t].n_tris * n_blocks > RTS_HZ_WORK_CAP) off[t] = 1u;
    }
    DevBuf<RtsHorizonMesh> d_mesh; DevBuf<uint32_t> d_off; DevBuf<RtsHzPrim> d_hp; DevBuf<RtsHzBlk> d_hb; DevBuf<double> d_pv;
    RTS_HIP(d_mesh.reserve(n_targets)); RTS_HIP(d_off.reserve(n_targets)); RTS_HIP(d_hp.reserve(n)); RTS_HIP(d_hb.reserve(n_blocks)); RTS_HIP(d_pv.reserve((size_t)n * 9));
    RTS_HIP(ns->d_horizon.reserve((size_t)n * 2));
    RTS_HIP(hipStreamSynchronize(c->stream));
    RTS_HIP(hipMemcpy(d_mesh.p, ns->hz.data(), sizeof(RtsHorizonMesh) * n_targets, hipMemcpyHostToDevice));
    RTS_HIP(hipMemcpy(d_off.p, off.data(), sizeof(uint32_t) * n_targets, hipMemcpyHostToDevice));
    k_hz_prims<<<(n + 255u) / 256u, 256, 0, c->stream>>>(ns->d_prim_order.p, ns->d_tri_vidx.p, ns->d_verts_local.p, ns->d_prim_targ.p, n, d_mesh.p, d_off.p, d_hp.p, d_pv.p);
    k_hz_blocks<<<(n_blocks + 255u) / 256u, 256, 0, c->stream>>>(ns->d_prim_order.p, ns->d_prim_targ.p, n, n_blocks, d_hp.p, d_hb.p);
    RTS_HIP(hipMemsetAsync(ns->d_horizon.p, 0, sizeof(float) * 2 * (size_t)n, c->stream));
    k_hz_main<<<dim3((n + 255u) / 256u, RTS_HZ_SLICES), 256, 0, c->stream>>>(ns->d_prim_order.p, ns->d_prim_targ.p, n, n_blocks, d_mesh.p, d_off.p, d_hp.p, d_hb.p, d_pv.p, reinterpret_cast<uint32_t*>(ns->d_horizon.p));
    RTS_HIP(hipGetLastError());
    RTS_HIP(hipMemcpyAsync(off.data(), d_off.p, sizeof(uint32_t) * n_targets, hipMemcpyDeviceToHost, c->stream));
    RTS_HIP(hipStreamSynchronize(c->stream));
    for (uint32_t t = 0; t < n_targets; t++) if (off[t]) ns->hz[t].rho = 0.0;
    return RTS_OK;
}

extern "C" int rts_get_horizon(RtsHandle c, float* out, uint32_t capacity_prims)
{
    CHECK_HANDLE(c);
    if (!out) { rts_set_error("rts_get_horizon: null argument"); return RTS_ERR_INVALID; }
    const RtsScene* sc = c->scene;
    if (capacity_prims < sc->n_prims) { rts_set_error("rts_get_horizon: capacity too small (%u primitives)", sc->n_prims); return RTS_ERR_CAPACITY; }
    RTS_HIP(hipStreamSynchronize(c->stream));
    if (sc->n_prims) RTS_HIP(hipMemcpy(out, sc->d_horizon.p, sizeof(float) * 2 * (size_t)sc->n_prims, hipMemcpyDeviceToHost));
    return RTS_OK;
}
```

rts_amd/csrc/rts_internal.h:

```cpp
#pragma once
#include <hip/hip_runtime.h>
#include <stdint.h>
#include <stddef.h>
#include <atomic>
#include <string>
#include <vector>
#include "../../include/rts_amd.h"
#include "rts_device_math.h"
#include "rts_pattern.h"
#include "rts_waveform.h"
#include "rts_noise.h"
#include "rts_image.h"
#include "rts_cube_source.h"
#include "rts_stft.h"
#include "rts_beat.h"
#include "rts_beam.h"
#include "rts_adapt.h"
#include "rts_stap.h"
#include "rts_doa.h"
#include "rts_cfar_os.h"
#include "rts_track.h"
#include "rts_tbd.h"
#include "rts_source.h"
#include "rts_plot.h"
#include "rts_owned.h"
#include "rts_launch_plan.h"
#include "rts_post_plan.h"
#include "rts_pulse_state.h"
#include "rts_scene_host.h"
#include "rts_tuning.h"
static_assert(RtsTuning().img_split_below == RTS_IMAGE_SPLIT_BELOW, "the default of RTS_IMAGE_SPLIT_BELOW is rts_image.h's");


struct __attribute__((aligned(16))) RtsLeafTri {
    double p0x, p0y, p0z, e0x, e0y, e0z, e1x, e1y, e1z, nx, ny, nz;
    uint32_t prim;
    uint32_t targ;
    float hz[2];
};
static_assert(sizeof(RtsLeafTri) == 112, "leaf size");
#define RTS_HZ_H0 9.5367431640625e-07
#define RTS_HZ_RHO 0.00390625
#define RTS_HZ_DEGEN 9.5367431640625e-07
#define RTS_HZ_MARGIN 0.00390625f
struct RtsHorizonMesh { double extent, h0, rho; };
static_assert(offsetof(RtsLeafTri, p0x) == 0 && offsetof(RtsLeafTri, p0z) == 16 && offsetof(RtsLeafTri, e0y) == 32 && offsetof(RtsLeafTri, e1x) == 48 &&
              offsetof(RtsLeafTri, e1z) == 64 && offsetof(RtsLeafTri, ny) == 80 && offsetof(RtsLeafTri, prim) == 96 && offsetof(RtsLeafTri, targ) == 100,
              "leaf record offsets of the walk step's decode");

struct RtsTargetDev {
    double reflCoeff;
    double refrIndex;
    double vx, vy, vz;
    uint32_t tri_base;
    uint32_t perface_normals;
    double rinv[9];
    double px, py, pz;
    double cx, cy, cz, r2;
    float hz_h0, hz_rho;
    float ew;
    int32_t root;
};

struct RtsRxDev { double cx, cy, cz, radius, minTheta, maxTheta, minPhi, maxPhi; };

struct __attribute__((aligned(16))) RtsEndRecord {
    double rayLength, power, doppler;
    double prevx, prevy, prevz;
    double firstx, firsty, firstz;
    uint64_t path_lo, path_hi;
    uint32_t slot;
    int32_t received;
    uint32_t reflDepth;
    uint32_t pad;
};
static_assert(sizeof(RtsEndRecord) == 112, "end record size");
static_assert(sizeof(RtsDetection) == 72 && sizeof(RtsCfarParams) == 72 && sizeof(RtsCfarOsParams) == 72, "CFAR ABI sizes (rts_amd/_lib.py mirrors them)");
static_assert(sizeof(RtsPlot) == 104 && sizeof(RtsPlotParams) == 56, "plot ABI sizes (rts_amd/_lib.py mirrors them)");
static_assert(sizeof(RtsTrack) == 88 && sizeof(RtsTrackParams) == 96, "track ABI sizes (rts_amd/_lib.py mirrors them)");
static_assert(sizeof(RtsTbdParams) == 72 && sizeof(RtsTbdExtractParams) == 40 && sizeof(RtsTbdTrack) == 48, "track-before-detect ABI sizes (rts_amd/_lib.py mirrors them)");
static_assert(sizeof(RtsSourceParams) == 72, "source ABI size (rts_amd/_lib.py mirrors it)");
struct RtsTrackMeta { uint64_t next_id; uint32_t n, total, rounds, reserved; };

struct __attribute__((aligned(16))) RtsChildState {
    double prevx, prevy, prevz, firstx, firsty, firstz;
    double rayLength, power, doppler, refx, refy;
    float dx, dy, dz;
    uint32_t refrDepth, refr_code, end, pad0, pad1;
};
static_assert(sizeof(RtsChildState) == 128, "child state size");

#ifndef RTS_TILE_CTRS
#define RTS_TILE_CTRS 64
#endif
#define RTS_TILE_BUCKETS 1024
#define RTS_TILE_CTR_STRIDE 32
#define RTS_XCD 8
#define RTS_SEG_STRIPES 8
#define RTS_TILE_CTRS_LAYOUT ((RTS_XCD + 1) * RTS_SEG_STRIPES + 8)
#define RTS_OFF_CTR_COOP (RTS_TILE_CTRS_LAYOUT * RTS_TILE_CTR_STRIDE)
#define RTS_OFF_HEAD (2 * RTS_TILE_CTRS_LAYOUT * RTS_TILE_CTR_STRIDE)
#define RTS_OFF_LIVE (RTS_OFF_HEAD + 4)
#define RTS_OFF_COUNTERS (RTS_OFF_HEAD + 8)
#define RTS_OFF_BINS (RTS_OFF_COUNTERS + 48)
#define RTS_OFF_TAKEN (RTS_OFF_BINS + RTS_TILE_BUCKETS)
#define RTS_ZERO_WORDS (RTS_OFF_TAKEN + RTS_TILE_BUCKETS)
#ifndef RTS_RX_LDS
#define RTS_RX_LDS 16
#endif

#define RTS_MASK_MIN_CELL 1.0e-5
#define RTS_MASK_N 1024u
#define RTS_MASK_WORDS (RTS_MASK_N * RTS_MASK_N / 32u + 1u)
#define RTS_MASK_MAX_CELLS 4096
struct RtsMaskFrame { float bx, by, bz, ux, uy, uz, vx, vy, vz; float u0, v0, inv_du, inv_dv; uint32_t n, pad0, pad1; };

struct RtsLaunchConsts {
    double ox, oy, oz;
    double bsx, bsy, bsz;
    double stx, sty, stz;
    double rot[9];
    double rot1[9];
    double w1x, w1y, w1z;
    uint64_t ray_first;
    uint32_t W, pad;
    uint32_t w_magic, w_more;
    uint32_t il_tile, il_parts, il_part, pad2;
    const uint32_t* il_list;
    RtsMaskFrame mask;
    float f_bs[3], f_st[3], f_m[9], f_pad;
};
static_assert(sizeof(RtsLaunchConsts) % 8 == 0, "launch constants are copied to LDS dword by dword");

struct RtsTraceArgs {
    const RtsLaunchConsts* lc;
    uint64_t ray_first;
    uint32_t n_rays, W;
    uint32_t max_refl, smooth;
    uint32_t n_prims, n_targets, n_rx, keep_all;
    uint32_t max_refr, rows;
    RtsChildState* child;
    const RtsNode4* nodes4;
    const RtsNode4* nodes4v;
    const RtsLeafTri* leaves;
    const uint32_t* tri_nidx;
    const double* normals;
    const RtsTargetDev* targets;
    const RtsRxDev* rx;
    RtsEndRecord* recv_records;
    RtsEndRecord* all_records;
    unsigned long long* counters;
    unsigned long long* block_counters;
    float* dir_hist;
    int32_t* hit_prim;
    float* hit_t;
    int32_t* stack_ovf;
    uint32_t total_threads;
    uint32_t slab_threads;
    const uint32_t* tile_order;
    uint32_t* tile_cost;
    uint32_t* tile_ctr;
    uint32_t coop_spread;
    const uint32_t* tile_head;
    const uint32_t* tile_head_all;
    const uint32_t* tile_live;
    uint32_t rx_window_screen;
    uint32_t coop_versions;
    uint32_t batch_dead;
    uint32_t coop_walk_steps_lo;
    uint32_t coop_min_cost, coop_walk_steps;
    unsigned long long* timeline;
    uint32_t pre_filter;
    const uint32_t* pmask;
    uint32_t stack_lds;
    uint32_t horizon;
};

#define RTS_PIN_GROUPS 4096
static inline uint32_t rts_agg_spec(uint32_t R) { return R < RTS_PIN_GROUPS ? R : RTS_PIN_GROUPS; }
struct RtsPinned {
    RtsLaunchConsts lc;
    RtsTargetMotion motion[256];
    RtsTargetDev td[256];
    unsigned long long cnt[24];
    uint32_t G, pad;
    double rcs[256];
    double gsum[5 * RTS_PIN_GROUPS]; uint64_t gkey[RTS_PIN_GROUPS]; uint64_t grow[RTS_PIN_GROUPS]; uint32_t gmin[RTS_PIN_GROUPS];
};

struct RtsGate { hipStream_t tstream = nullptr; std::atomic<int> refs{0}; int device = 0; };

struct RtsScene {
    std::atomic<int> refs{1}; int device = 0;
    std::vector<RtsMeshHost> meshes;
    uint32_t n_prims = 0, n_verts = 0, n_normals = 0;
    DevBuf<uint32_t> d_tri_vidx, d_tri_nidx, d_vert_targ, d_norm_targ, d_prim_targ;
    DevBuf<double> d_verts_local, d_normals_local;
    std::vector<RtsBlasInfo> blas; uint32_t n_nodes = 0, n_leaves = 0;
    DevBuf<RtsNode4> d_nodes4; DevBuf<uint32_t> d_leaf_prim;
    DevBuf<uint32_t> d_prim_order;
    DevBuf<RtsNode4> d_nodes4v;
    DevBuf<float> d_horizon;
    std::vector<RtsHorizonMesh> hz;
    double build_ms = 0; uint32_t builder = 0;
    size_t device_bytes() const {
        return d_tri_vidx.cap * 4 + d_tri_nidx.cap * 4 + d_vert_targ.cap * 4 + d_norm_targ.cap * 4 + d_prim_targ.cap * 4 + d_verts_local.cap * 8 +
               d_normals_local.cap * 8 + (d_nodes4.cap + d_nodes4v.cap) * sizeof(RtsNode4) + d_leaf_prim.cap * 4 + d_prim_order.cap * 4 + d_horizon.cap * 4;
    }
};

struct RtsTileHist { std::atomic<int> refs{1}; DevBuf<uint32_t> d; uint32_t n = 0; bool any = false; uint32_t head_hint = 0; bool head_hint_valid = false; };

struct RtsSpecParams { std::vector<double> rcs; double wl = 0, gt = 0, gr = 0, carrier = 0, cspeed = 0; int32_t cube_pulse = -1; uint64_t base = 0;
                       int mode = 0;
                       int fin = 0;
                       std::vector<double> pat_rx; double pat_org[3] = {0, 0, 0}, pat_dir[2] = {0, 0};
};
struct RtsPatArgs { const RtsPatView* pats; const double* rx; uint32_t n_rx, n_targets; double ox, oy, oz, tx_az, tx_el, wl, carrier, cspeed; };
struct RtsHostMirror {
    PinBuf<char> buf; uint32_t cap = 0, D = 0;
    size_t o_rays = 0, o_paths = 0, o_angles = 0, o_slots = 0, o_apower = 0, o_adoppler = 0, o_adelay = 0, o_aphase = 0, o_apm = 0, o_vpower = 0, o_vdoppler = 0;
    bool recv_valid = false, agg_valid = false;
    bool want = false;
};
struct RtsAggPending { bool valid = false, rows = false; uint32_t R = 0, D = 0, spec = 0; RtsKeyPlan key = {}; uint64_t base = 0; double* gsum = nullptr; };

struct RtsCubeProduct {
    DevBuf<double> own; double* p = nullptr; size_t doubles = 0; bool valid = false;
    hipError_t place(void* device_out, size_t n, double** out)
    {
        *out = (double*)device_out; if (*out) return hipSuccess;
        if (n > own.cap) { p = nullptr; doubles = 0; valid = false; }
        const hipError_t e = own.reserve(n); *out = own.p; return e;
    }
    void record(double* out, size_t n) { p = out; doubles = n; valid = true; }
};

struct RtsCubeState {
    RtsCubeParams params = {}; double* p = nullptr; DevBuf<double> own; bool set = false;
    DevBuf<double> d_wave; uint32_t wave_M = 0, wave_L = 0; bool wave_set = false;
    RtsCubeProduct doppler; uint32_t doppler_n = 0;
    DevBuf<uint32_t> d_det_cnt, d_det_off; DevBuf<uint8_t> d_det_tmp; DevBuf<RtsDetection> d_det; uint32_t det_nseg = 0, det_max = 0; bool det_valid = false;
    uint32_t det_nd = 0;
    DevBuf<uint64_t> d_plot_key; DevBuf<uint32_t> d_plot_parent, d_plot_idx, d_plot_lab_s, d_plot_idx_s, d_plot_len, d_plot_flag, d_plot_off; DevBuf<uint8_t> d_plot_tmp;
    DevBuf<RtsPlot> d_plot; uint32_t plot_cap = 0, plot_max = 0; bool plot_valid = false, plot_own_list = false;
    DevBuf<RtsTrack> d_trk[2]; DevBuf<RtsTrackMeta> d_trk_meta; DevBuf<RtsTrackPred> d_trk_pred;
    DevBuf<double> d_trk_zd, d_trk_zf, d_trk_pw, d_trk_cd, d_trk_md2; DevBuf<uint64_t> d_trk_best_d;
    DevBuf<uint32_t> d_trk_zrx, d_trk_cj, d_trk_cn, d_trk_of_track, d_trk_of_plot, d_trk_best_t, d_trk_rounds, d_trk_flag, d_trk_off; DevBuf<uint8_t> d_trk_tmp;
    uint32_t trk_cur = 0, trk_max = 0, trk_loaded = 0; bool trk_live = false; double trk_time = 0.0;
    DevBuf<double> d_tbd_merit[2]; DevBuf<uint8_t> d_tbd_ptr, d_tbd_tmp; DevBuf<int32_t> d_tbd_shift;
    DevBuf<uint32_t> d_tbd_cnt, d_tbd_off, d_tbd_paths; DevBuf<RtsTbdTrack> d_tbd_out;
    uint32_t tbd_rx = 0, tbd_nd = 0, tbd_nb = 0, tbd_depth = 0, tbd_hd = 0, tbd_hr = 0, tbd_cur = 0; uint64_t tbd_frames = 0;
    double tbd_time = 0.0, tbd_t0 = 0.0, tbd_dt = 0.0;
    uint32_t tbd_ext_nseg = 0, tbd_ext_max = 0, tbd_ext_depth = 0; bool tbd_ext_valid = false;
    StagedUpload<double> os_alpha; std::vector<double> os_tab; uint32_t os_tab_key[5] = {0, 0, 0, 0, 0}; double os_tab_pfa = 0.0; bool os_tab_sent = false;
    RtsCubeProduct image; uint32_t img_nx = 0, img_ny = 0;
    StagedUpload<double> img_geo; DevBuf<double> d_img_scratch;
    RtsCubeProduct stft;
    StagedUpload<double> stft_win; DevBuf<double> d_stft_part;
    DevBuf<double> d_beat_part;
    RtsCubeProduct range;
    StagedUpload<double> range_win;
    RtsCubeProduct beam;
    StagedUpload<double> beam_w;
    StagedUpload<double> src_tab;
    RtsCubeProduct cov; uint32_t cov_n = 0; DevBuf<double> d_cov_part;
    RtsCubeProduct mvdr;
    StagedUpload<double> mvdr_s; DevBuf<uint32_t> d_mvdr_status;
    RtsCubeProduct st;
    StagedUpload<double> st_w;
    RtsCubeProduct eig_val, eig_vec; uint32_t eig_n = 0; DevBuf<uint32_t> d_eig_status;
    RtsCubeProduct doa;
    StagedUpload<double> doa_g;
    void end_products() { doppler.valid = false; det_valid = false; plot_valid = false; image.valid = false; stft.valid = false; range.valid = false; beam.valid = false; cov.valid = false; mvdr.valid = false; st.valid = false;
                          eig_val.valid = false; eig_vec.valid = false; doa.valid = false; }
};

struct RtsPulseResults {
    uint64_t n_recv = 0;
    const unsigned long long* recv_dev = nullptr;
    std::vector<RtsGroup> groups; bool agg_valid = false; uint64_t recv_index_base = 0;
    RtsAggPending agg_pending;
    bool agg_delay_in = true;
    int64_t agg_base_local = 0;
    RtsHostMirror mirror;
// ... 150 lines not shown
```

rts_amd/csrc/rts_results_api.hip:

```cpp
#include <cstring>
#include "rts_internal.h"

template <class T> static hipError_t rts_copy_home(T* dst, const T* src, size_t n) { return dst && n ? hipMemcpy(dst, src, sizeof(T) * n, hipMemcpyDeviceToHost) : hipSuccess; }

template <class T> static hipError_t rts_view_fill(RtsPulseResults& r, unsigned bit, std::vector<T>& v, const T* src, size_t n, const T** out)
{
    if (!(r.v_recv_have & bit)) { v.resize(n); const hipError_t e = hipMemcpy(v.data(), src, sizeof(T) * n, hipMemcpyDeviceToHost); if (e != hipSuccess) return e; r.v_recv_have |= bit; }
    if (out) *out = v.data();
    return hipSuccess;
}

extern "C" int rts_get_stats(RtsHandle c, RtsStats* out)
{
    if (!c || !out) { rts_set_error("rts_get_stats: null argument"); return RTS_ERR_INVALID; }
    CHECK_CLOSED(c);
    if (c->stats_pending) {
        RTS_HIP(hipSetDevice(c->device));
        RTS_HIP(hipStreamSynchronize(c->stream));
        RtsStats& s = c->stats; float ms = 0;
        RTS_HIP(hipEventElapsedTime(&s.ms_scene, c->ev[0], c->ev[1]));
        RTS_HIP(hipEventElapsedTime(&s.ms_trace, c->ev[2], c->ev[3]));
        RTS_HIP(hipEventElapsedTime(&s.ms_compact, c->ev[4], c->ev[5]));
        s.ms_aggregate = 0;
        if (c->res.fin_timed || c->res.agg_timed) { RTS_HIP(hipEventElapsedTime(&ms, c->ev[6], c->ev[7])); s.ms_aggregate = ms; }
        c->stats_pending = false;
    }
    *out = c->stats; return RTS_OK;
}

extern "C" int rts_get_block_timeline(RtsHandle c, double* out, uint32_t n)
{
    if (!c || !out) { rts_set_error("rts_get_block_timeline: null argument"); return RTS_ERR_INVALID; }
    CHECK_CLOSED(c);
    if (!c->tune.timeline_blocks || c->tl_summary[8] == 0.0) { rts_set_error("rts_get_block_timeline: the handle records no block timeline (create it with RTS_TIMELINE_BLOCKS=1, product build) or has not traced yet"); return RTS_ERR_INVALID; }
    for (uint32_t k = 0; k < n && k < 9; k++) out[k] = c->tl_summary[k];
    return RTS_OK;
}

static int rts_walk_counters(RtsContext* c, const char* who, uint64_t* out, uint32_t n)
{
    if (!c || !out) { rts_set_error("%s: null argument", who); return RTS_ERR_INVALID; }
    CHECK_CLOSED(c);
    const int src[11] = {8, 9, 10, 11, 15, 16, 17, 18, 19, 20, 21};
    for (uint32_t k = 0; k < n && k < 11u; k++) out[k] = c->pin.p->cnt[src[k]];
    return RTS_OK;
}
extern "C" int rts_get_lane_stats(RtsHandle c, uint64_t* out3) { return rts_walk_counters(c, "rts_get_lane_stats", out3, 3); }
extern "C" int rts_get_walk_stats(RtsHandle c, uint64_t* out, uint32_t n) { return rts_walk_counters(c, "rts_get_walk_stats", out, n); }

extern "C" int rts_received_count(RtsHandle c, uint64_t* count)
{
    if (!c || !count) { rts_set_error("rts_received_count: null argument"); return RTS_ERR_INVALID; }
    CHECK_CLOSED(c);
    *count = c->res.n_recv; return RTS_OK;
}

extern "C" int rts_get_received(RtsHandle c, PerRayData* rays, int32_t* paths, double* rcs_angles, uint64_t* slots, uint64_t capacity)
{
    CHECK_HANDLE(c);
    CHECK_CLOSED(c);
    const uint64_t R = c->res.n_recv; const uint32_t D = c->depth;
    if (capacity < R) { rts_set_error("rts_get_received: capacity %llu < %llu received rays", (unsigned long long)capacity, (unsigned long long)R); return RTS_ERR_CAPACITY; }
    if (R == 0) return RTS_OK;
    RTS_HIP(hipStreamSynchronize(c->stream));
    RTS_HIP(rts_copy_home(rays, c->d_rx_rays.p, R)); RTS_HIP(rts_copy_home(paths, c->d_rx_paths.p, R * D));
    RTS_HIP(rts_copy_home(rcs_angles, c->d_rx_angles.p, 2 * R * D)); RTS_HIP(rts_copy_home(slots, c->d_rx_slots.p, R));
    return RTS_OK;
}

extern "C" int rts_get_all_rays(RtsHandle c, PerRayData* results, int32_t* targ_intersect, double* rcs_angle, int32_t* hit_prim, float* hit_t, uint64_t capacity)
{
    CHECK_HANDLE(c);
    CHECK_CLOSED(c);
    if (!(c->params.flags & RTS_FLAG_KEEP_ALL_RAYS)) { rts_set_error("rts_get_all_rays: handle was not created with RTS_FLAG_KEEP_ALL_RAYS"); return RTS_ERR_INVALID; }
    const uint64_t n1 = c->n_rays, n = n1 * c->last_args.rows; const uint32_t D = c->depth, H = rts_hit_rows(c->params.max_refl);
    if (capacity < n) { rts_set_error("rts_get_all_rays: capacity too small (%llu rows)", (unsigned long long)n); return RTS_ERR_CAPACITY; }
    if (n == 0) return RTS_OK;
    RTS_HIP(hipStreamSynchronize(c->stream));
    RTS_HIP(rts_copy_home(results, c->d_all_rays.p, n)); RTS_HIP(rts_copy_home(targ_intersect, c->d_all_paths.p, n * D)); RTS_HIP(rts_copy_home(rcs_angle, c->d_all_angles.p, 2 * n * D));
    RTS_HIP(rts_copy_home(hit_prim, c->d_hit_prim.p, n1 * H)); RTS_HIP(rts_copy_home(hit_t, c->d_hit_t.p, n1 * H));
    return RTS_OK;
}

extern "C" int rts_received_view(RtsHandle c, const PerRayData** rays, const int32_t** paths, const double** rcs_angles, const uint64_t** slots, uint64_t* count)
{
    CHECK_HANDLE(c);
    if (!count) { rts_set_error("rts_received_view: null count"); return RTS_ERR_INVALID; }
    CHECK_CLOSED(c);
    RtsPulseResults& r = c->res; const uint64_t R = r.n_recv; const uint32_t D = c->depth;
    *count = R;
    if (rays) *rays = nullptr; if (paths) *paths = nullptr; if (rcs_angles) *rcs_angles = nullptr; if (slots) *slots = nullptr;
    if (R == 0) return RTS_OK;
    RTS_HIP(rts_stream_wait(c, c->stream));
    const RtsHostMirror& m = r.mirror;
    if (m.recv_valid && R <= m.cap) {
        if (rays) *rays = (const PerRayData*)(m.buf.p + m.o_rays); if (paths) *paths = (const int32_t*)(m.buf.p + m.o_paths);
        if (rcs_angles) *rcs_angles = (const double*)(m.buf.p + m.o_angles); if (slots) *slots = (const uint64_t*)(m.buf.p + m.o_slots);
        return RTS_OK;
    }
    if (rays) RTS_HIP(rts_view_fill(r, 1u, r.v_rays, c->d_rx_rays.p, R, rays));
    if (paths && D) RTS_HIP(rts_view_fill(r, 2u, r.v_paths, c->d_rx_paths.p, R * D, paths));
    if (rcs_angles && D) RTS_HIP(rts_view_fill(r, 4u, r.v_angles, c->d_rx_angles.p, 2 * R * D, rcs_angles));
    if (slots) RTS_HIP(rts_view_fill(r, 8u, r.v_slots, c->d_rx_slots.p, R, slots));
    return RTS_OK;
}

extern "C" int rts_finalise_values(RtsHandle c, const double* power, const double* doppler, uint64_t count)
{
    CHECK_HANDLE(c);
    CHECK_CLOSED(c);
    if (count != c->res.n_recv) { rts_set_error("rts_finalise_values: %llu values for %llu received rays", (unsigned long long)count, (unsigned long long)c->res.n_recv); return RTS_ERR_INVALID; }
    if (count == 0) return RTS_OK;
    if (!power || !doppler) { rts_set_error("rts_finalise_values: null array"); return RTS_ERR_INVALID; }
    return rts_finalise_bracket(c, [&]() -> int {
        RtsHostMirror& m = c->res.mirror;
        if (!m.buf.p) { int rc = rts_mirror_reserve(c, RTS_SMALL_CAP32); if (rc != RTS_OK) return rc; }
        if (count <= m.cap) {
            memcpy(m.buf.p + m.o_vpower, power, sizeof(double) * count); memcpy(m.buf.p + m.o_vdoppler, doppler, sizeof(double) * count);
            return rts_post_set_values(c, (const double*)(m.buf.dev + m.o_vpower), (const double*)(m.buf.dev + m.o_vdoppler));
        }
        RTS_HIP(c->d_delay.reserve(count)); RTS_HIP(c->d_phase.reserve(count));
        RTS_HIP(hipMemcpyAsync(c->d_delay.p, power, sizeof(double) * count, hipMemcpyHostToDevice, c->stream));
        RTS_HIP(hipMemcpyAsync(c->d_phase.p, doppler, sizeof(double) * count, hipMemcpyHostToDevice, c->stream));
        int rc = rts_post_set_values(c, c->d_delay.p, c->d_phase.p); if (rc != RTS_OK) return rc;
        RTS_HIP(hipStreamSynchronize(c->stream));
        return RTS_OK;
    });
// ... 64 lines not shown
```

rts_amd/csrc/rts_scene.hip:

```cpp
#include <cstdio>
#include <cstring>
#include <algorithm>
#include <chrono>
#include <memory>
#include <thread>
#include "rts_internal.h"
#include "rts_prim_order.h"

__global__ void k_children_to_prims(RtsNode4* __restrict__ nodes, uint32_t n, const uint32_t* __restrict__ leaf_prim)
{
    const uint32_t i = blockIdx.x * blockDim.x + threadIdx.x;
    if (i >= n) return;
    for (int k = 0; k < 4; k++) { const int32_t ch = nodes[i].child[k]; nodes[i].pad[k] = ch; if (ch < 0) nodes[i].child[k] = ~(int32_t)leaf_prim[~ch]; }
}

__global__ void k_node_versions(const RtsNode4* __restrict__ nodes, uint32_t n, RtsNode4* __restrict__ out, int key_mode)
{
    const uint32_t g = blockIdx.x * blockDim.x + threadIdx.x;
    if (g >= n * 8u) return;
    const uint32_t i = g >> 3, o = g & 7u;
    const RtsNode4 nd = nodes[i];
    const bool mx = (o & 1u) != 0u, my = (o & 2u) != 0u, mz = (o & 4u) != 0u;
    float key[4]; int ord[4];
    for (int k = 0; k < 4; k++) {
// ... 97 lines not shown
    }
    return RTS_OK;
}

int rts_attach_scene(RtsContext* c)
{
    const RtsScene* sc = c->scene; const uint32_t n_targets = (uint32_t)sc->meshes.size();
    RTS_HIP(c->d_leaves.reserve((size_t)sc->n_prims + 1));
    RTS_HIP(c->d_verts_world.reserve(3*(size_t)sc->n_verts + 1)); RTS_HIP(c->d_normals_world.reserve(3*(size_t)sc->n_normals + 1));
    {
        const size_t span = offsetof(RtsPinned, cnt);
        RTS_HIP(c->d_params.reserve(span));
        c->p_lc = reinterpret_cast<RtsLaunchConsts*>(c->d_params.p + offsetof(RtsPinned, lc));
        c->p_motion = reinterpret_cast<RtsTargetMotion*>(c->d_params.p + offsetof(RtsPinned, motion));
        c->p_targets = reinterpret_cast<RtsTargetDev*>(c->d_params.p + offsetof(RtsPinned, td));
        c->rcs_uploaded = false;
    }
    c->verts_world_valid = false; c->order_sum_valid = false;
    if (c->hist->refs.load() > 1) { rts_hist_unref(c->hist); c->hist = new RtsTileHist(); }
    c->motion.assign(n_targets, RtsTargetMotion{}); c->motion_valid = false; c->bvh_valid = false; c->hist->n = 0; c->hist->any = false; c->hist->head_hint_valid = false; c->tile_cost_pending = false; c->tile_last_valid = false;
    return RTS_OK;
}

static int scene_swap(RtsContext* c, RtsScene* ns)
{
    rts_scene_unref(c->scene);
    c->scene = ns;
    return rts_attach_scene(c);
}

extern "C" int rts_set_scene(RtsHandle c, const RtsMesh* meshes, uint32_t n_targets)
{
    CHECK_HANDLE(c);
    CHECK_CLOSED(c);
    { int rc = check_key_width(c->depth, n_targets, c->n_rx, "rts_set_scene"); if (rc != RTS_OK) return rc; }
    RtsSceneFlat flat;
    { int rc = rts_scene_flatten(meshes, n_targets, c->params.interpolate_smooth, &flat); if (rc != RTS_OK) return rc; }
    std::unique_ptr<RtsScene> ns(new RtsScene()); ns->device = c->device;
    { int rc = scene_upload(c, ns.get(), flat); if (rc != RTS_OK) return rc; }
    const auto t_build0 = std::chrono::steady_clock::now();
    RtsSceneTuning st; st.device_build = (c->params.flags & RTS_FLAG_HOST_BUILD) == 0;
    rts_tuning_read(&st, rts_env);
    { int rc = scene_build(c, ns.get(), meshes, flat, st); if (rc != RTS_OK) return rc; }
    { int rc = scene_finish(c, ns.get(), st); if (rc != RTS_OK) return rc; }
    {
        const auto t_hz0 = std::chrono::steady_clock::now();
        int rc = rts_horizon_build(c, ns.get(), flat); if (rc != RTS_OK) return rc;
        if (st.debug_build) fprintf(stderr, "[rts] horizon: %.2f ms\n", std::chrono::duration<double, std::milli>(std::chrono::steady_clock::now() - t_hz0).count());
    }
    ns->build_ms = std::chrono::duration<double, std::milli>(std::chrono::steady_clock::now() - t_build0).count();
    return scene_swap(c, ns.release());
}

extern "C" int rts_share_scene(RtsHandle dst, RtsHandle src)
{
    if (!dst || !src || dst == src) { rts_set_error("rts_share_scene: needs two distinct handles"); return RTS_ERR_INVALID; }
    if (dst->device != src->device) { rts_set_error("rts_share_scene: handles live on different devices (%d, %d)", dst->device, src->device); return RTS_ERR_INVALID; }
    if (dst->params.interpolate_smooth && !src->params.interpolate_smooth) {
        for (const RtsMeshHost& m : src->scene->meshes) if (m.n_tris && m.n_normals == 0) { rts_set_error("rts_share_scene: the scene has a mesh without normals but the receiving handle interpolates normals"); return RTS_ERR_INVALID; }
    }
    RtsContext* c = dst;
    CHECK_HANDLE(c);
    CHECK_CLOSED(c);
    RTS_HIP(hipStreamSynchronize(c->stream));
    if (dst->scene == src->scene) return RTS_OK;
    rts_scene_unref(dst->scene);
    dst->scene = src->scene; dst->scene->refs++;
    { int rc = rts_attach_scene(dst); if (rc != RTS_OK) return rc; }
    if (dst->tune.share_history && src->tune.share_history && dst->params.width == src->params.width) {
        rts_hist_unref(dst->hist);
        dst->hist = src->hist; dst->hist->refs++;
    }
    return RTS_OK;
}

extern "C" int rts_scene_info(RtsHandle c, RtsSceneInfo* out)
{
    if (!c || !out) { rts_set_error("rts_scene_info: null argument"); return RTS_ERR_INVALID; }
    const RtsScene* sc = c->scene;
    memset(out, 0, sizeof(*out));
    out->n_targets = (uint32_t)sc->meshes.size(); out->n_prims = sc->n_prims; out->n_nodes = sc->n_nodes; out->n_leaves = sc->n_leaves;
    out->handles_sharing = (uint32_t)sc->refs.load(); out->builder = sc->builder; out->build_ms = sc->build_ms;
    out->shared_device_bytes = sc->device_bytes(); out->version_bytes = sc->d_nodes4v.cap * sizeof(RtsNode4);
    out->horizon_bytes = sc->d_horizon.cap * sizeof(float);
    out->handle_device_bytes = c->d_leaves.cap * sizeof(RtsLeafTri) + c->d_verts_world.cap * 8 + c->d_normals_world.cap * 8 + c->d_params.cap;
    return RTS_OK;
}

extern "C" int rts_get_bvh(RtsHandle c, void* nodes128, uint32_t* leaf_prim, int32_t* roots, uint32_t node_capacity, uint32_t leaf_capacity, uint32_t* n_leaves)
{
    CHECK_HANDLE(c);
    if (n_leaves) *n_leaves = c->scene->n_leaves;
    if ((nodes128 && node_capacity < c->scene->n_nodes) || (leaf_prim && leaf_capacity < c->scene->n_leaves)) { rts_set_error("rts_get_bvh: capacity too small (%u nodes, %u leaves)", c->scene->n_nodes, c->scene->n_leaves); return RTS_ERR_CAPACITY; }
    RTS_HIP(hipStreamSynchronize(c->stream));
    if (nodes128 && c->scene->n_nodes) {
        RTS_HIP(hipMemcpy(nodes128, c->scene->d_nodes4.p, sizeof(RtsNode4)*c->scene->n_nodes, hipMemcpyDeviceToHost));
        RtsNode4* nd = static_cast<RtsNode4*>(nodes128);
        for (uint32_t i = 0; i < c->scene->n_nodes; i++) for (int k = 0; k < 4; k++) { nd[i].child[k] = nd[i].pad[k]; nd[i].pad[k] = 0; }
    }
    if (leaf_prim && c->scene->n_leaves) RTS_HIP(hipMemcpy(leaf_prim, c->scene->d_leaf_prim.p, sizeof(uint32_t)*c->scene->n_leaves, hipMemcpyDeviceToHost));
    if (roots) for (size_t t = 0; t < c->scene->blas.size(); t++) roots[t] = c->scene->blas[t].root;
    return RTS_OK;
}
```

rts_amd/csrc/rts_trace.hip:

```cpp
#include "rts_internal.h"
#include "rts_raygen.h"
#include "rts_ray_ops.h"

struct RtsSlabRay { float iNx, cNx, iFx, cFx, iNy, cNy, iFy, cFy, iNz, cNz, iFz, cFz; };
__device__ __forceinline__ void rts_slab_axis(float o, float d, float E, float& iN_, float& cN_, float& iF_, float& cF_)
{
    const float iv = 1.0f / d;
    const bool pos = !(iv < 0.0f);
    const float oN = o + (pos ? E : -E), oF = o - (pos ? E : -E);
    const float iN = iv * 0.9999994f, iF = iv * 1.0000006f;
    const float cN = -(oN * iN), cF = -(oF * iF);
    const bool drop = !(fabsf(iv) < 1.0e30f);
    const float NINF = -__builtin_inff(), PINF = __builtin_inff();
    iN_ = drop ? 0.0f : iN; cN_ = drop ? NINF : cN;
    iF_ = drop ? 0.0f : iF; cF_ = drop ? PINF : cF;
}
__device__ __forceinline__ RtsSlabRay rts_slab_setup(const dvec3& o, const dvec3& d, float extra)
{
    RtsSlabRay r;
    const float ox = (float)o.x, oy = (float)o.y, oz = (float)o.z;
    const float E = fmaxf(fmaxf(fabsf(ox), fabsf(oy)), fabsf(oz)) * 4.5e-7f + extra + 1.0e-30f;
    rts_slab_axis(ox, (float)d.x, E, r.iNx, r.cNx, r.iFx, r.cFx);
    rts_slab_axis(oy, (float)d.y, E, r.iNy, r.cNy, r.iFy, r.cFy);
    rts_slab_axis(oz, (float)d.z, E, r.iNz, r.cNz, r.iFz, r.cFz);
// ... 179 lines not shown
        if (h.ok) {
            const float tf = (float)h.t;
            if ((tf > tmin) && (tf < best_t || (tf == best_t && L.prim < best_prim))) {
                best_t = tf; best_leaf = leaf; best_prim = L.prim;
                t_prune = f32_next_up_pos(tf);
            }
        }
        node = below; sp--;
    }
}

__device__ __forceinline__ float rts_wave_min_f32(float v) { for (int o = 32; o > 0; o >>= 1) v = fminf(v, __shfl_xor(v, o)); return v; }
__device__ __forceinline__ unsigned long long rts_wave_min_u64(unsigned long long v) { for (int o = 32; o > 0; o >>= 1) { const unsigned long long w = __shfl_xor(v, o); v = w < v ? w : v; } return v; }
template <bool COUNT, bool VERS = false, uint32_t CG = 64u>
__device__ __forceinline__ void rts_walk_coop(const RtsTraceArgs& a, int32_t* s_stack, int32_t* s_exch, uint32_t tid, uint32_t gtid, uint32_t lane, int lds_cap, uint32_t* n_spill_lds,
                                              int root, const RtsSlabRay& lr, const dvec3& prev, const dvec3& dir, float tmin,
                                              float& best_t, int& best_leaf, uint32_t& best_prim, float& t_prune, uint32_t& n_nodes, uint32_t& n_tris, bool& hard_overflow)
{
    const int SENTINEL = RTS_STACK_SENTINEL;
    const uint32_t g0 = lane & ~(CG - 1u);
    const unsigned long long gmask = CG == 64u ? ~0ULL : (((1ULL << (CG & 63u)) - 1ULL) << g0);
    const unsigned long long below_me = (1ULL << lane) - 1ULL;
    volatile int32_t* row = s_exch + (tid & ~63u) + g0;
    s_stack[tid] = SENTINEL;
    int sp = 1, bot = 1;
    int node = (lane & (CG - 1u)) == 0u ? root : SENTINEL;
    uint32_t steps = 0;
    const RtsSlabRay lp = VERS ? lr : rts_slab_by_plane(lr);
    for (;;) {
        const bool busy = node != SENTINEL;
        const unsigned long long busy_m = __ballot(busy);
        if (busy_m == 0ULL) break;
        if (++steps > (1u << 24)) { hard_overflow = true; break; }
        const unsigned long long idle_m = __ballot(true) & ~busy_m;
        if (idle_m != 0ULL) {
            const bool can = busy && sp > bot && bot < lds_cap;
            const unsigned long long can_m = __ballot(can);
            if (can_m != 0ULL) {
                const unsigned long long idle_g = idle_m & gmask, can_g = can_m & gmask;
                const uint32_t n_give = min((uint32_t)__popcll(idle_g), (uint32_t)__popcll(can_g));
                const uint32_t r_can = (uint32_t)__popcll(can_g & below_me), r_idle = (uint32_t)__popcll(idle_g & below_me);
                if (can && r_can < n_give) { row[r_can] = s_stack[bot * RTS_BLOCK + tid]; s_stack[bot * RTS_BLOCK + tid] = SENTINEL; bot++; }
                __builtin_amdgcn_wave_barrier();
                if (!busy && r_idle < n_give) { node = row[r_idle]; sp = 1; bot = 1; }
                __builtin_amdgcn_wave_barrier();
            }
        }
        bool improved = false;
        if (node != SENTINEL) {
            const float before = t_prune;
            rts_walk_step<COUNT, VERS ? RTS_WALK_VERSIONS : RTS_WALK_PLANES>(a, s_stack, tid, gtid, lds_cap, n_spill_lds, node, sp, lp, prev, dir, tmin, best_t, best_leaf, best_prim, t_prune, n_nodes, n_tris, hard_overflow);
            improved = t_prune != before;
        }
        if (__any(improved)) { for (int o = (int)CG / 2; o > 0; o >>= 1) t_prune = fminf(t_prune, __shfl_xor(t_prune, o)); }
    }
    const unsigned long long key = best_leaf >= 0 ? (((unsigned long long)__float_as_uint(best_t) << 32) | best_prim) : ~0ULL;
    unsigned long long kmin = key;
    for (int o = (int)CG / 2; o > 0; o >>= 1) { const unsigned long long w = __shfl_xor(kmin, o); kmin = w < kmin ? w : kmin; }
    const unsigned long long has_m = __ballot(key == kmin) & gmask;
    const int win = has_m ? __ffsll((long long)has_m) - 1 : (int)lane;
    const int leaf_w = __shfl(best_leaf, win);
    if (kmin != ~0ULL) {
        best_leaf = leaf_w; best_t = __uint_as_float((uint32_t)(kmin >> 32)); best_prim = (uint32_t)kmin;
        t_prune = f32_next_up_pos(best_t);
    }
}

#define RTS_RXP_QQW 3
#define RTS_RXP_R2W 4
#define RTS_RXP_QN 5
#define RTS_RXP_QQ 6
#define RTS_RXP_R2 7
#define RTS_RXP_E2 8
#define RTS_RXP_CT 9
#define RTS_RXP_ST 10
#define RTS_RXP_CH 11
#define RTS_RXP_SLO 12
#define RTS_RXP_SHI 13
#define RTS_RXP_OK 14
#define RTS_RXP_RW 15
#define RTS_RXP_N 16
struct RtsUnitLds { int32_t* stack; int32_t* exch; double* first; unsigned long long* path; uint32_t* n; const RtsRxDev* rx; const float (*rxp)[RTS_RXP_N]; uint32_t* lane_scratch; uint32_t* walk; };
#define RTS_SKIP_SHIFT 23
#define RTS_SHADED_MASK 0x007fffffu
struct RtsRay { dvec3 dir, prev; double rayLength, power, doppler, refx, refy; uint32_t reflDepth, refrDepth; int received; bool end, chain_start; };

template <bool KEEP_ALL, bool REFR, bool COOP, uint32_t CG = 64u>
__device__ __forceinline__ bool rts_shade(const RtsTraceArgs& a, const RtsUnitLds& L_, const uint32_t tid, const uint32_t gtid, const uint32_t lane, const uint32_t slot,
                                          const uint32_t chain, const uint32_t D, const uint32_t max_refr, const dvec3& origin, const bool primary, const bool may_rx,
                                          const float best_t, const int best_leaf, const uint32_t best_prim, const float tmin, RtsRay& S, uint32_t& pending, uint32_t& refr_code0)
{
    double* const s_first = L_.first; unsigned long long* const s_path = L_.path; uint32_t* const s_n = L_.n; const RtsRxDev* const s_rx = L_.rx;
    dvec3& dir = S.dir; dvec3& prev = S.prev;
    double& rayLength = S.rayLength; double& power = S.power; double& doppler = S.doppler; double& refx = S.refx; double& refy = S.refy;
    uint32_t& reflDepth = S.reflDepth; uint32_t& refrDepth = S.refrDepth; int& received = S.received; bool& end = S.end; bool& chain_start = S.chain_start;
        if (KEEP_ALL && chain == 0 && (!COOP || (lane & (CG - 1u)) == 0u)) {
            const size_t hidx = (size_t)slot * (a.max_refl + 1) + reflDepth;
            a.hit_prim[hidx] = (best_leaf >= 0) ? (int32_t)best_prim : -1;
            a.hit_t[hidx] = (best_leaf >= 0) ? best_t : 0.0f;
        }

        if (best_leaf < 0) {
            if (end == false && (!primary || may_rx)) {
                for (uint32_t Rx_i = 0; Rx_i < a.n_rx; Rx_i++) {
                    const RtsRxDev rx = Rx_i < RTS_RX_LDS ? s_rx[Rx_i] : a.rx[Rx_i];
                    double t[2] = {0, 0};
                    const double A = (dir.x)*(dir.x) + (dir.y)*(dir.y) + (dir.z)*(dir.z);
                    const double B = 2*(((prev.x - rx.cx)*dir.x) + ((prev.y - rx.cy)*dir.y) + ((prev.z - rx.cz)*dir.z));
                    const double C = prev.x*prev.x + prev.y*prev.y + prev.z*prev.z + (rx.cx*rx.cx) + (rx.cy*rx.cy) + (rx.cz*rx.cz) -
                                     2*((rx.cx*prev.x) + (rx.cy*prev.y) + (rx.cz*prev.z)) - rx.radius*rx.radius;
                    double discriminant = B*B - 4*A*C;
                    if (discriminant > 0.f) {
                        discriminant = sqrt(discriminant);
                        t[0] = (-B - discriminant)/(2*A);
                        t[1] = (-B + discriminant)/(2*A);
                        unsigned int received_root = 2;
    #pragma unroll
                        for (int i = 0; i < 2; i++) {
                            if ((t[i] >= 0) && ((rayLength + t[i]) > SCENE_EPS) && ((rayLength + t[i]) > SCENE_EPS_R)) {
                                const dvec3 ep = mk3(prev.x + t[i]*dir.x, prev.y + t[i]*dir.y, prev.z + t[i]*dir.z);
                                double theta = rts_atan2f((float)(ep.y - rx.cy), (float)(ep.x - rx.cx));
                                double phi = rts_atan2f((float)(ep.z - rx.cz), (float)sqrt(((ep.y - rx.cy) * (ep.y - rx.cy)) + ((ep.x - rx.cx) * (ep.x - rx.cx))));
                                if ((phi < -RTS_PI/2)) { theta += RTS_PI; phi = -RTS_PI - phi; }
                                if ((phi > RTS_PI/2)) { theta += RTS_PI; phi = RTS_PI - phi; }
                                double maxTheta1 = rx.maxTheta, minTheta1 = rx.minTheta, maxTheta2 = maxTheta1, minTheta2 = minTheta1;
                                double maxPhi1 = rx.maxPhi, minPhi1 = rx.minPhi, maxPhi2 = maxPhi1, minPhi2 = minPhi1;
                                if ((minPhi1 < -RTS_PI/2)) { maxTheta2 += RTS_PI; minTheta2 += RTS_PI; maxPhi2 = -RTS_PI - minPhi1; minPhi2 = -RTS_PI/2; minPhi1 = -RTS_PI/2; }
                                if ((maxPhi1 > RTS_PI/2)) { maxTheta2 += RTS_PI; minTheta2 += RTS_PI; minPhi2 = RTS_PI - maxPhi1; maxPhi2 = RTS_PI/2; maxPhi1 = RTS_PI/2; }
                                if (((rts_angle_in_range(theta, minTheta1, maxTheta1)) && (rts_angle_in_range(phi, minPhi1, maxPhi1))) ||
                                    ((rts_angle_in_range(theta, minTheta2, maxTheta2)) && (rts_angle_in_range(phi, minPhi2, maxPhi2)))) {
                                    if (received_root == 2) received_root = i;
                                    else if (t[received_root] > t[i]) received_root = i;
                                }
                            }
                        }
                        if (received_root < 2) {
                            end = true;
                            const double tr = received_root == 0 ? t[0] : t[1];
                            const dvec3 ep = mk3(prev.x + tr*dir.x, prev.y + tr*dir.y, prev.z + tr*dir.z);
                            if ((reflDepth == 0) && (refrDepth == 0)) {
                                const dvec3 RxRange = sub3(ep, origin);
                                if (len3(RxRange) >= SCENE_EPS) {
                                    power = 1/(4*RTS_PI*4*RTS_PI*(magsq3(RxRange)));
                                    doppler = 0;
                                    rayLength += tr;
                                    received = (int)Rx_i;
                                }
                            } else {
                                const dvec3 RxRange = sub3(ep, prev);
                                if (len3(RxRange) >= SCENE_EPS_R) {
                                    power *= 1/((magsq3(RxRange))*4*RTS_PI*4*RTS_PI);
                                    rayLength += tr;
                                    received = (int)Rx_i;
                                }
                            }
                        }
                    }
                }
            }
            if (KEEP_ALL && end == false && rayLength > 0) {
                const double d_earthRadius = 6378136;
                const double A = (dir.x)*(dir.x) + (dir.y)*(dir.y) + (dir.z)*(dir.z);
                const double B = 2*(prev.x*dir.x + prev.y*dir.y + prev.z*dir.z);
                const double C = prev.x*prev.x + prev.y*prev.y + prev.z*prev.z - d_earthRadius*d_earthRadius;
                double discriminant = B*B - 4*A*C;
                if (discriminant > 0.f) {
                    discriminant = sqrt(discriminant);
// ... 15 lines not shown
                const uint64_t code = (uint64_t)(L.targ + 1);
                unsigned long long* pw = &s_path[(col < 8 ? 0 : RTS_BLOCK) + tid];
                const uint32_t sh = 8 * (col & 7u);
                *pw = (*pw & ~(0xffULL << sh)) | (code << sh);
            }
        }
        const float hit_t = best_t;
        const dvec3 hitPoint = mk3(prev.x + (double)hit_t*dir.x, prev.y + (double)hit_t*dir.y, prev.z + (double)hit_t*dir.z);
        rayLength += hit_t;
        if ((reflDepth == 0) && (refrDepth == 0)) {
            s_first[tid] = hitPoint.x; s_first[RTS_BLOCK + tid] = hitPoint.y; s_first[2 * RTS_BLOCK + tid] = hitPoint.z;
            const dvec3 TxRange = sub3(hitPoint, origin);
            if (len3(TxRange) >= SCENE_EPS) power = 1/((magsq3(TxRange))*4*RTS_PI);
            else end = true;
        } else {
            const dvec3 TargRange = sub3(hitPoint, prev);
            if (len3(TargRange) >= SCENE_EPS_R) power *= 1/((magsq3(TargRange))*4*RTS_PI);
            else end = true;
        }
        const TriHit h = tri_test(L, prev, dir, tmin, RTS_DEFAULT_TMAX);
        prev = hitPoint;
        dvec3 normal;
        if (a.smooth) {
            const uint32_t* ni = a.tri_nidx + 3*(size_t)L.prim;
            if (T.perface_normals) {
                const double* n = a.normals + 3*(size_t)ni[0];
                normal = mk3(n[0], n[1], n[2]);
            } else {
                const double* n0 = a.normals + 3*(size_t)ni[0]; const double* n1 = a.normals + 3*(size_t)ni[1]; const double* n2 = a.normals + 3*(size_t)ni[2];
                const double w = 1.0f - h.beta - h.gamma;
                normal = mk3(n1[0]*h.beta + n2[0]*h.gamma + n0[0]*w, n1[1]*h.beta + n2[1]*h.gamma + n0[1]*w, n1[2]*h.beta + n2[2]*h.gamma + n0[2]*w);
            }
            normal = unit3(normal);
        } else {
            normal = unit3(h.n);
        }
        const fvec3 dirf = (chain == 0 && chain_start) ? unit3_to_f32(dir) : mk3f((float)dir.x, (float)dir.y, (float)dir.z);
        const fvec3 nf = unit3_to_f32(normal);

        const double rrefx = refy;
        if (REFR) {
            if ((fabs(T.reflCoeff) != 1.00000f) && (refrDepth < max_refr) && (reflDepth == 0)) {
                const double rrefy = (rrefx == 1) ? T.refrIndex : 1.0;
                const float ratio = (float)(rrefy / rrefx);
                fvec3 rd;
                if (refract3f(rd, dirf, nf, ratio)) {
                    RtsChildState cs;
                    cs.prevx = prev.x; cs.prevy = prev.y; cs.prevz = prev.z; cs.firstx = s_first[tid]; cs.firsty = s_first[RTS_BLOCK + tid]; cs.firstz = s_first[2 * RTS_BLOCK + tid];
                    cs.rayLength = rayLength; cs.refx = rrefx; cs.refy = rrefy; cs.end = end ? 1u : 0u;
                    double cpower = power;
                    if ((reflDepth + 1) < (a.max_refl + 1)) cpower *= (1 - fabs(T.reflCoeff));
                    cs.power = cpower;
                    cs.refrDepth = refrDepth + 1;
                    const dvec3 k0 = unit3(dir);
                    const dvec3 nd3 = widen3(rd);
                    const dvec3 k1 = unit3(nd3);
                    cs.doppler = doppler + dot3(mk3(T.vx, T.vy, T.vz), sub3(k1, k0));
                    cs.dx = rd.x; cs.dy = rd.y; cs.dz = rd.z;
                    cs.refr_code = (chain == 0) ? (L.targ + 1) : (uint32_t)(s_path[tid] & 0xff);
                    if (chain == 0) refr_code0 = L.targ + 1;
                    a.child[(size_t)chain * a.slab_threads + gtid] = cs;
                    pending |= 1u << (chain + 1);
                    float* dh = a.dir_hist + (size_t)((chain + 1) * (a.max_refl + 1)) * 3 * a.n_rays;
                    if (!COOP || (lane & (CG - 1u)) == 0u) { dh[slot] = rd.x; dh[(size_t)a.n_rays + slot] = rd.y; dh[2*(size_t)a.n_rays + slot] = rd.z; }
                }
            }
        }
        reflDepth++;
        refy = rrefx; refx = rrefx;
        chain_start = false;
        if (!(reflDepth < a.max_refl + 1)) return false;
        const fvec3 nd = reflect3f(dirf, nf);
        power *= T.reflCoeff;
        if (KEEP_ALL || REFR) {
            const dvec3 k0 = unit3(dir);
            const dvec3 k1 = unit3(widen3(nd));
            doppler += dot3(mk3(T.vx, T.vy, T.vz), sub3(k1, k0));
        }
        dir = widen3(nd);
        if (!REFR) {
            uint32_t skip = 0u;
            if (a.horizon) {
                const double dn = dir.x*L.nx + dir.y*L.ny + dir.z*L.nz, dl = sqrt(dir.x*dir.x + dir.y*dir.y + dir.z*dir.z), nl = sqrt(L.nx*L.nx + L.ny*L.ny + L.nz*L.nz);
                const double c = fabs(dn) / (dl * nl), S = (double)(dn > 0.0 ? L.hz[0] : L.hz[1]);
                const double ht = fabs((double)hit_t);
                const double delta = ht * 0x1p-22 + (fmax(fmax(fabs(prev.x), fabs(prev.y)), fabs(prev.z)) + ht) * 0x1p-45;
                const double reach = dl * (double)SCENE_EPS_R;
                if ((c - delta / reach > S + (double)RTS_HZ_MARGIN) && (c * reach >= 2.0 * ((double)T.hz_h0 + delta)) && (4.0 * delta <= (double)T.hz_rho)) skip = L.targ + 1u;
            }
            atomicAnd(&s_n[RTS_BLOCK + tid], RTS_SHADED_MASK); if (skip) atomicOr(&s_n[RTS_BLOCK + tid], skip << RTS_SKIP_SHIFT);
        }
        {
            const size_t plane = REFR ? (size_t)chain * (a.max_refl + 1) + reflDepth : (size_t)(reflDepth - 1);
            float* dh = a.dir_hist + plane * 3 * a.n_rays;
            if (!COOP || (lane & (CG - 1u)) == 0u) { dh[slot] = nd.x; dh[(size_t)a.n_rays + slot] = nd.y; dh[2*(size_t)a.n_rays + slot] = nd.z; }
        }
    return true;
}


template <bool KEEP_ALL, bool REFR, bool COOP, uint32_t CG = 64u>
__device__ __forceinline__ void rts_write_back(const RtsTraceArgs& a, const RtsUnitLds& L_, const uint32_t tid, const uint32_t lane, const uint32_t slot, const uint32_t chain,
                                               const RtsRay& S, const uint32_t pending, const uint32_t refr_code0)
{
    const double* const s_first = L_.first; const unsigned long long* const s_path = L_.path;
    const dvec3& prev = S.prev; const double rayLength = S.rayLength, power = S.power, doppler = S.doppler;
    const uint32_t reflDepth = S.reflDepth, refrDepth = S.refrDepth; const int received = S.received;
    const bool recv = received >= 0;
    if ((recv || KEEP_ALL) && (!COOP || (lane & (CG - 1u)) == 0u)) {
        RtsEndRecord r;
        r.rayLength = rayLength; r.power = power; r.doppler = (KEEP_ALL || REFR) ? doppler : 0.0;
        r.prevx = prev.x; r.prevy = prev.y; r.prevz = prev.z;
        r.firstx = s_first[tid]; r.firsty = s_first[RTS_BLOCK + tid]; r.firstz = s_first[2 * RTS_BLOCK + tid];
        r.path_lo = s_path[tid]; r.path_hi = s_path[RTS_BLOCK + tid]; r.slot = slot; r.received = received; r.reflDepth = reflDepth;
        r.pad = chain | (refrDepth << 2) | ((chain == 0 ? refr_code0 : 0u) << 8) | ((pending & 6u) << 15);
        if (KEEP_ALL) a.all_records[(size_t)chain * a.n_rays + slot] = r;
        if (recv) {
            unsigned long long idx = atomicAdd(&a.counters[0], 1ULL);
            a.recv_records[idx] = r;
        }
    }
}

__device__ __forceinline__ bool rts_rx_maybe(const float* K, const float dx, const float dy, const float dz, const float dd, const float delta)
{
    const float qx = K[0], qy = K[1], qz = K[2], qn = K[RTS_RXP_QN];
    const float b = qx*dx + qy*dy + qz*dz;
    const float R = K[RTS_RXP_RW] + qn * delta, r2w = delta > 0.0f ? R * R : K[RTS_RXP_R2W];
    const bool inside = K[RTS_RXP_QQW] <= K[RTS_RXP_R2W] * 1.01f;
    const bool ahead = b > -(1.0e-3f + delta) * qn && (b*b - (K[RTS_RXP_QQW] - r2w) * dd) >= 0.0f;
    if (!(inside || ahead)) return false;
    if (K[RTS_RXP_OK] == 0.0f) return true;
    const float e2 = K[RTS_RXP_E2], s2 = b*b - (K[RTS_RXP_QQ] - K[RTS_RXP_R2]);
    if (!(s2 >= 16.0f * e2)) return true;
    const float s = __builtin_sqrtf(s2);
    float dt = 0.0f;
    if (delta > 0.0f) {
        const float qd = qn * delta;
        if (!(s2 - qd * (2.2f * fabsf(b) + qd) >= 0.5f * s2)) return true;
        dt = qd * (1.0f + (2.0f * fabsf(b) + qd) / (1.7f * s));
    }
    const float et = 0.75f * e2 / s + 1.0e-6f * qn;
    const float tl_min = fabsf(b >= 0.0f ? b + s : b - s) - et - dt;
    const bool small_gone = tl_min > 0.0f && (fabsf(K[RTS_RXP_QQ] - K[RTS_RXP_R2]) + e2) / tl_min + et < 0.004999f;
    bool maybe = false;
#pragma unroll
    for (int k = 0; k < 2; k++) {
        const float t = k == 0 ? b - s : b + s;
        if (t + et + dt < 0.004999f) continue;
        if (small_gone && (k == 0) == (b >= 0.0f)) continue;
        const float px = __builtin_fmaf(t, dx, -qx), py = __builtin_fmaf(t, dy, -qy), pz = __builtin_fmaf(t, dz, -qz);
        const float ep = et + dt + (fabsf(t) + qn) * (2.0e-6f + delta);
        const float rho = __builtin_sqrtf(px*px + py*py);
        if (!(ep <= 0.25f * rho)) { maybe = true; continue; }
        const bool az_out = (px * K[RTS_RXP_CT] + py * K[RTS_RXP_ST]) < rho * (K[RTS_RXP_CH] - 1.1f * ep / rho - 2.0e-6f);
        const bool el_out = pz < K[RTS_RXP_SLO] - 2.0f * ep - 2.0e-6f * qn || pz > K[RTS_RXP_SHI] + 2.0f * ep + 2.0e-6f * qn;
        maybe = maybe || !(az_out || el_out);
    }
    return maybe;
}

__device__ __forceinline__ void rts_prefilter(const RtsLaunchConsts& lc, const uint32_t slot, const bool mask_on, const uint32_t* __restrict__ pmask, const uint32_t n_rx,
                                              const float (*rxp)[RTS_RXP_N], bool& may_target, bool& may_rx)
{
    uint32_t lx, ly, lz; rts_lattice_coords(lc, slot, lx, ly, lz);
    const float vx = __builtin_fmaf(lc.f_st[0], (float)lx, lc.f_bs[0]), vy = __builtin_fmaf(lc.f_st[1], (float)ly, lc.f_bs[1]), vz = __builtin_fmaf(lc.f_st[2], (float)lz, lc.f_bs[2]);
    float dx = lc.f_m[0]*vx + lc.f_m[1]*vy + lc.f_m[2]*vz, dy = lc.f_m[3]*vx + lc.f_m[4]*vy + lc.f_m[5]*vz, dz = lc.f_m[6]*vx + lc.f_m[7]*vy + lc.f_m[8]*vz;
    const float inv = __frsqrt_rn(dx*dx + dy*dy + dz*dz); dx *= inv; dy *= inv; dz *= inv;
    if (mask_on) {
        const RtsMaskFrame& mf = lc.mask;
        const float w = dx * mf.bx + dy * mf.by + dz * mf.bz;
        const float iw = __builtin_amdgcn_rcpf(w);
        const float fu = ((dx * mf.ux + dy * mf.uy + dz * mf.uz) * iw - mf.u0) * mf.inv_du, fv = ((dx * mf.vx + dy * mf.vy + dz * mf.vz) * iw - mf.v0) * mf.inv_dv;
        if (w > 0.0f && fu >= 0.0f && fv >= 0.0f && fu < (float)mf.n && fv < (float)mf.n) {
            const uint32_t cell = (uint32_t)fv * mf.n + (uint32_t)fu;
            may_target = ((pmask[cell >> 5] >> (cell & 31u)) & 1u) != 0u;
        }
    }
    may_rx = false;
    const float dd = dx*dx + dy*dy + dz*dz;
    for (uint32_t Rx_i = 0; Rx_i < n_rx; Rx_i++) may_rx = may_rx || rts_rx_maybe(rxp[Rx_i], dx, dy, dz, dd, 0.0f);
}

__device__ __forceinline__ bool rts_segment_maybe(const RtsLaunchConsts& lc, const uint32_t lx_a, const uint32_t lx_b, const uint32_t ly, const uint32_t lz, const bool has_prims, const bool mask_on,
                                                  const uint32_t* __restrict__ pmask, const uint32_t n_rx, const float (*rxp)[RTS_RXP_N])
{
    const float vy = __builtin_fmaf(lc.f_st[1], (float)ly, lc.f_bs[1]), vz = __builtin_fmaf(lc.f_st[2], (float)lz, lc.f_bs[2]);
    const float vxa = __builtin_fmaf(lc.f_st[0], (float)lx_a, lc.f_bs[0]), vxb = __builtin_fmaf(lc.f_st[0], (float)lx_b, lc.f_bs[0]);
    float ax = lc.f_m[0]*vxa + lc.f_m[1]*vy + lc.f_m[2]*vz, ay = lc.f_m[3]*vxa + lc.f_m[4]*vy + lc.f_m[5]*vz, az = lc.f_m[6]*vxa + lc.f_m[7]*vy + lc.f_m[8]*vz;
    float bx = lc.f_m[0]*vxb + lc.f_m[1]*vy + lc.f_m[2]*vz, by = lc.f_m[3]*vxb + lc.f_m[4]*vy + lc.f_m[5]*vz, bz = lc.f_m[6]*vxb + lc.f_m[7]*vy + lc.f_m[8]*vz;
    { const float ia = __frsqrt_rn(ax*ax + ay*ay + az*az), ib = __frsqrt_rn(bx*bx + by*by + bz*bz); ax *= ia; ay *= ia; az *= ia; bx *= ib; by *= ib; bz *= ib; }
    if (has_prims) {
        if (!mask_on) return true;
        const RtsMaskFrame& mf = lc.mask;
        const float wa = ax * mf.bx + ay * mf.by + az * mf.bz, wb = bx * mf.bx + by * mf.by + bz * mf.bz;
        if (!(wa > 0.0f && wb > 0.0f)) return true;
        const float iwa = __builtin_amdgcn_rcpf(wa), iwb = __builtin_amdgcn_rcpf(wb);
        const float fua = ((ax * mf.ux + ay * mf.uy + az * mf.uz) * iwa - mf.u0) * mf.inv_du, fva = ((ax * mf.vx + ay * mf.vy + az * mf.vz) * iwa - mf.v0) * mf.inv_dv;
        const float fub = ((bx * mf.ux + by * mf.uy + bz * mf.uz) * iwb - mf.u0) * mf.inv_du, fvb = ((bx * mf.vx + by * mf.vy + bz * mf.vz) * iwb - mf.v0) * mf.inv_dv;
        const float ulo = fminf(fua, fub), uhi = fmaxf(fua, fub), vlo = fminf(fva, fvb), vhi = fmaxf(fva, fvb);
        if (!(ulo >= 0.0f && vlo >= 0.0f && uhi < (float)mf.n && vhi < (float)mf.n)) return true;
        const bool major_u = (uhi - ulo) >= (vhi - vlo);
        float a0 = major_u ? fua : fva, a1 = major_u ? fub : fvb, b0 = major_u ? fva : fua, b1 = major_u ? fvb : fub;
        if (a0 > a1) { const float t0 = a0; a0 = a1; a1 = t0; const float t1 = b0; b0 = b1; b1 = t1; }
        const uint32_t c0 = (uint32_t)a0, c1 = (uint32_t)a1;
        if (c1 - c0 > 96u) return true;
        const float slope = (a1 - a0) > 1.0e-6f ? (b1 - b0) / (a1 - a0) : 0.0f;
        const float nmax = (float)(mf.n - 1u);
        uint32_t found = 0u;
        for (uint32_t c = c0; c <= c1; c++) {
            const float la = fmaxf(a0, (float)c), ha = fminf(a1, (float)(c + 1u));
            const float bl = b0 + slope * (la - a0), bh = b0 + slope * (ha - a0);
            const uint32_t r0 = (uint32_t)fminf(fmaxf(fminf(bl, bh) - 0.03125f, 0.0f), nmax), r1 = (uint32_t)fminf(fmaxf(fmaxf(bl, bh) + 0.03125f, 0.0f), nmax);
            for (uint32_t r = r0; r <= r1; r++) { const uint32_t cell = major_u ? r * mf.n + c : c * mf.n + r; found |= pmask[cell >> 5] >> (cell & 31u); }
        }
        if (found & 1u) return true;
    }
    const float ex = ax - bx, ey = ay - by, ez = az - bz;
    const float delta = 1.6f * __builtin_sqrtf(ex*ex + ey*ey + ez*ez) + 4.0e-6f;
    const float dd = ax*ax + ay*ay + az*az;
    for (uint32_t Rx_i = 0; Rx_i < n_rx; Rx_i++) if (rts_rx_maybe(rxp[Rx_i], ax, ay, az, dd, delta)) return true;
    return false;
}
__device__ __forceinline__ bool rts_tile_maybe(const RtsLaunchConsts& lc, const uint32_t tile, const uint32_t n_rays, const bool has_prims, const bool mask_on, const uint32_t* __restrict__ pmask,
                                               const uint32_t n_rx, const float (*rxp)[RTS_RXP_N])
{
    const uint32_t s0 = tile * 64u, s1 = min(s0 + 63u, n_rays - 1u);
    uint32_t lx, ly, lz;
    rts_lattice_coords(lc, s0, lx, ly, lz);
    uint32_t left = s1 - s0 + 1u;
    bool maybe = false;
    while (left != 0u && !maybe) {
        const uint32_t n = min(left, lc.W - lx);
        maybe = rts_segment_maybe(lc, lx, lx + n - 1u, ly, lz, has_prims, mask_on, pmask, n_rx, rxp);
        left -= n; lx = 0u;
        if (++ly == lc.W) { ly = 0u; lz++; }
    }
    return maybe;
}

__device__ __forceinline__ void rts_primary_setup(const RtsTraceArgs& a, const RtsLaunchConsts& lc, const RtsUnitLds& L_, const uint32_t tid, const uint32_t slot, const bool pre_on,
                                                  const bool mask_on, const dvec3& origin, RtsRay& S, bool& may_target, bool& may_rx, const bool pre_done = false)
{
    double* const s_first = L_.first; unsigned long long* const s_path = L_.path; const float (*const s_rxp)[RTS_RXP_N] = L_.rxp;
    dvec3& dir = S.dir; dvec3& prev = S.prev; double& rayLength = S.rayLength; double& power = S.power; double& doppler = S.doppler;
    if (pre_on && !pre_done) rts_prefilter(lc, slot, mask_on, a.pmask, a.n_rx, s_rxp, may_target, may_rx);
    dir = (may_target || may_rx) ? rts_primary_dir(lc, slot) : mk3(0.0, 0.0, 0.0);
    prev = origin;
    s_first[tid] = 0.0; s_first[RTS_BLOCK + tid] = 0.0; s_first[2 * RTS_BLOCK + tid] = 0.0;
    s_path[tid] = 0ULL; s_path[RTS_BLOCK + tid] = 0ULL; atomicAnd(&L_.n[RTS_BLOCK + tid], RTS_SHADED_MASK);
    rayLength = 0; power = 0; doppler = 0;
}

template <bool COUNT, bool KEEP_ALL, bool REFR, bool COOP, bool VERS = false>
__device__ __forceinline__ void rts_trace_unit(const RtsTraceArgs& a, const RtsLaunchConsts& lc, const RtsUnitLds& L_, const uint32_t tid, const uint32_t gtid, const uint32_t lane,
                                               const uint32_t slot, const bool pre_on, const bool mask_on, const uint32_t D, const uint32_t max_refr, const dvec3& origin,
                                               uint32_t& n_nodes, uint32_t& n_tris, bool& hard_overflow, unsigned long long (&lane_stats)[11],
                                               const uint32_t pre = 0u)
{
      int32_t* const s_stack = L_.stack; int32_t* const s_exch = L_.exch; double* const s_first = L_.first; unsigned long long* const s_path = L_.path; uint32_t* const s_n = L_.n;
      constexpr uint32_t CG = (COOP && VERS) ? (uint32_t)RTS_COOP_GROUP : 64u;

      uint32_t pending = 0;
      uint32_t refr_code0 = 0;
      for (uint32_t chain = 0; chain < (REFR ? 3u : 1u); chain++) {
        RtsRay S;
        dvec3& dir = S.dir; dvec3& prev = S.prev;
        double& rayLength = S.rayLength; double& power = S.power; double& doppler = S.doppler; double& refx = S.refx; double& refy = S.refy;
        uint32_t& reflDepth = S.reflDepth; uint32_t& refrDepth = S.refrDepth; bool& end = S.end; bool& chain_start = S.chain_start;
        refx = 1; refy = 1; reflDepth = 0; refrDepth = 0; S.received = -1; end = false;
        bool may_target = a.n_prims > 0, may_rx = a.n_rx > 0;
        if (pre & 1u) { may_target = (pre & 2u) != 0u; may_rx = (pre & 4u) != 0u; }
        if (chain == 0) {
            rts_primary_setup(a, lc, L_, tid, slot, pre_on, mask_on, origin, S, may_target, may_rx, (pre & 1u) != 0u);
        } else {
            if (!REFR || !(pending & (1u << chain))) continue;
            const RtsChildState cs = a.child[(size_t)(chain - 1) * a.slab_threads + gtid];
            dir = mk3((double)cs.dx, (double)cs.dy, (double)cs.dz);
            prev = mk3(cs.prevx, cs.prevy, cs.prevz);
            s_first[tid] = cs.firstx; s_first[RTS_BLOCK + tid] = cs.firsty; s_first[2 * RTS_BLOCK + tid] = cs.firstz;
            rayLength = cs.rayLength; power = cs.power; doppler = cs.doppler; refx = cs.refx; refy = cs.refy;
            refrDepth = cs.refrDepth; end = cs.end != 0;
            const uint64_t code = cs.refr_code;
            uint64_t path_lo = 0, path_hi = 0;
            for (uint32_t col = 0; col < (chain == 1 ? D : 2u); col++) { if (col < 8) path_lo |= code << (8 * col); else path_hi |= code << (8 * (col - 8)); }
            s_path[tid] = path_lo; s_path[RTS_BLOCK + tid] = path_hi;
        }
        chain_start = true;

        for (;;) {
            if (!COOP || (lane & (CG - 1u)) == 0u) atomicAdd(&s_n[tid], RTS_SEG_ONE);
            if (!COOP) { const unsigned long long ex_ = __ballot(true);
                         if (__builtin_amdgcn_mbcnt_hi((uint32_t)(ex_ >> 32), __builtin_amdgcn_mbcnt_lo((uint32_t)ex_, 0u)) == 0u) atomicAdd(&L_.walk[2u * __builtin_amdgcn_readfirstlane(tid >> 6) + 1u], 1u); }
            const float tmin = chain_start ? SCENE_EPS : SCENE_EPS_R;
            float best_t = RTS_DEFAULT_TMAX;
            int best_leaf = -1; uint32_t best_prim = 0xffffffffu;
            const bool primary = chain == 0 && chain_start;
            const bool may_hit = primary ? may_target : a.n_prims > 0;
            uint32_t steps = 0;
            bool escaped = false;
            if (may_hit) {
                float t_prune = RTS_DEFAULT_TMAX;
                for (uint32_t targ = 0; targ < a.n_targets; targ++) {
                    const RtsTargetDev& TG = a.targets[targ];
                    if (TG.root < 0) continue;
                    if (!REFR && (s_n[RTS_BLOCK + tid] >> RTS_SKIP_SHIFT) == targ + 1u) { if (COUNT) escaped = true; continue; }
                    {
                        const dvec3 q = mk3(TG.cx - prev.x, TG.cy - prev.y, TG.cz - prev.z);
                        const double qq = q.x*q.x + q.y*q.y + q.z*q.z, b = q.x*dir.x + q.y*dir.y + q.z*dir.z;
                        if (qq > TG.r2) {
                            const double dd = dir.x*dir.x + dir.y*dir.y + dir.z*dir.z;
                            if (!(b > 0.0) || !(b*b >= (qq - TG.r2) * dd * 0.999999)) continue;
                        }
                    }
                    const dvec3 q = mk3(prev.x - TG.px, prev.y - TG.py, prev.z - TG.pz);
                    const dvec3 ol = mk3(TG.rinv[0]*q.x + TG.rinv[1]*q.y + TG.rinv[2]*q.z, TG.rinv[3]*q.x + TG.rinv[4]*q.y + TG.rinv[5]*q.z, TG.rinv[6]*q.x + TG.rinv[7]*q.y + TG.rinv[8]*q.z);
                    const dvec3 dl = mk3(TG.rinv[0]*dir.x + TG.rinv[1]*dir.y + TG.rinv[2]*dir.z, TG.rinv[3]*dir.x + TG.rinv[4]*dir.y + TG.rinv[5]*dir.z, TG.rinv[6]*dir.x + TG.rinv[7]*dir.y + TG.rinv[8]*dir.z);
                    const RtsSlabRay lr = rts_slab_setup(ol, dl, TG.ew);
                    const uint32_t oct = VERS ? ((__float_as_uint(lr.iNx) >> 31) | ((__float_as_uint(lr.iNy) >> 31) << 1) | ((__float_as_uint(lr.iNz) >> 31) << 2)) : 0u;
                    const int SENTINEL = RTS_STACK_SENTINEL;
                    const int lds_cap = (int)a.stack_lds;
                    if (COOP) {
                        rts_walk_coop<COUNT, VERS, CG>(a, s_stack, s_exch, tid, gtid, lane, lds_cap, &s_n[2 * RTS_BLOCK + tid], VERS ? (int)(((uint32_t)TG.root << 3) | oct) : TG.root, lr, prev, dir, tmin, best_t, best_leaf, best_prim, t_prune,
                                             n_nodes, n_tris, hard_overflow);
                        if (COUNT) steps = 1u;
                    } else {
                        s_stack[tid] = SENTINEL;
                        int sp = 1;
                        int node = VERS ? (int)(((uint32_t)TG.root << 3) | oct) : TG.root;
                        uint32_t wave_steps = 0;
                        while (node != SENTINEL) {
                            wave_steps = __builtin_amdgcn_readfirstlane(wave_steps) + 1u;
                            if (wave_steps > (1u << 24)) { hard_overflow = true; break; }
                            if (COUNT) steps++;
                            rts_walk_step<COUNT, VERS ? RTS_WALK_VERSIONS : RTS_WALK_ROLES>(a, s_stack, tid, gtid, lds_cap, &s_n[2 * RTS_BLOCK + tid], node, sp, lr, prev, dir, tmin, best_t, best_leaf, best_prim, t_prune,
                                                 n_nodes, n_tris, hard_overflow);
                        }
                        { const unsigned long long ex_ = __ballot(true);
                          if (__builtin_amdgcn_mbcnt_hi((uint32_t)(ex_ >> 32), __builtin_amdgcn_mbcnt_lo((uint32_t)ex_, 0u)) == 0u) { atomicAdd(&L_.walk[2u * __builtin_amdgcn_readfirstlane(tid >> 6)], wave_steps); } }
                    }
                }
            }
            if (COUNT && !COOP) {
                uint32_t* ls = L_.lane_scratch + 2u * (tid >> 6);
                const unsigned long long act = __ballot(true);
                if (lane == (uint32_t)(__ffsll((long long)act) - 1)) { ls[0] = 0u; ls[1] = 0u; }
                atomicMax(&ls[0], steps); atomicAdd(&ls[1], steps);
                const uint32_t smax = ls[0], ssum = ls[1];
                lane_stats[0] += 64ull * smax; lane_stats[1] += (unsigned long long)__popcll(act) * smax; lane_stats[2] += ssum;
                lane_stats[3] += (unsigned long long)__popcll(__ballot(steps > 0u));
                lane_stats[4] += (unsigned long long)__popcll(__ballot(steps == 0u)) * smax;
            }
            if (COUNT && escaped && (!COOP || (lane & (CG - 1u)) == 0u)) lane_stats[5] += 1ull;
            if (COUNT && !COOP) {
                const unsigned long long act_ = __ballot(true);
                if (lane == (uint32_t)(__ffsll((long long)act_) - 1)) {
                    const uint32_t smax_ = L_.lane_scratch[2u * (tid >> 6)];
                    if (primary) { lane_stats[9] += smax_; lane_stats[10] += 1ull; }
                    else { lane_stats[8] += 1ull; lane_stats[6] += smax_; if (smax_ == 0u) lane_stats[7] += 1ull; }
                }
            }
            if (COUNT && COOP && steps) lane_stats[3] += 1ull;
            {
                const bool go_on_ = rts_shade<KEEP_ALL, REFR, COOP, CG>(a, L_, tid, gtid, lane, slot, chain, D, max_refr, origin, primary, may_rx, best_t, best_leaf, best_prim, tmin, S, pending, refr_code0);
                if (!go_on_) break;
            }
        }

        rts_write_back<KEEP_ALL, REFR, COOP, CG>(a, L_, tid, lane, slot, chain, S, pending, refr_code0);
      }
}

#define RTS_COST_UNITS(ticks) (((unsigned long long)(ticks) * 3ULL) >> 3)

template <bool COUNT, bool KEEP_ALL, bool REFR, bool COOP, bool VERS = false>
__global__ void __launch_bounds__(RTS_BLOCK, (REFR && COOP) ? 2 : ((REFR || COOP) ? 3 : 4)) k_trace(const RtsTraceArgs a)
{
    __shared__ __attribute__((aligned(16))) int32_t s_stack[RTS_STACK_LDS * RTS_BLOCK];
    const uint32_t tid = threadIdx.x;
    const uint32_t gtid = (COOP ? a.total_threads : 0u) + blockIdx.x * RTS_BLOCK + tid;
    __shared__ __attribute__((aligned(16))) RtsLaunchConsts s_lc;
    __shared__ __attribute__((aligned(16))) RtsRxDev s_rx[RTS_RX_LDS];
    __shared__ __attribute__((aligned(16))) double s_first[3 * RTS_BLOCK];
    __shared__ __attribute__((aligned(16))) unsigned long long s_path[2 * RTS_BLOCK];
    __shared__ uint32_t s_n[3 * RTS_BLOCK];
    s_n[threadIdx.x] = 0; s_n[RTS_BLOCK + threadIdx.x] = 0; s_n[2 * RTS_BLOCK + threadIdx.x] = 0;
    {
        const uint32_t* src = reinterpret_cast<const uint32_t*>(a.lc); uint32_t* dst = reinterpret_cast<uint32_t*>(&s_lc);
        for (uint32_t i = threadIdx.x; i < sizeof(RtsLaunchConsts) / 4; i += RTS_BLOCK) dst[i] = src[i];
        const uint32_t n_rx_lds = a.n_rx < RTS_RX_LDS ? a.n_rx : RTS_RX_LDS;
        const uint32_t* rsrc = reinterpret_cast<const uint32_t*>(a.rx); uint32_t* rdst = reinterpret_cast<uint32_t*>(s_rx);
        for (uint32_t i = threadIdx.x; i < n_rx_lds * (sizeof(RtsRxDev) / 4); i += RTS_BLOCK) rdst[i] = rsrc[i];
    }
    __syncthreads();
    const RtsLaunchConsts& lc = s_lc;
    const dvec3 origin = mk3(lc.ox, lc.oy, lc.oz);
    __shared__ float s_rxp[RTS_RX_LDS][RTS_RXP_N];
    if (tid < RTS_RX_LDS && tid < a.n_rx) {
        const RtsRxDev r = s_rx[tid];
        const double qx = r.cx - lc.ox, qy = r.cy - lc.oy, qz = r.cz - lc.oz, qq = qx*qx + qy*qy + qz*qz;
        const double w2 = lc.ox*lc.ox + lc.oy*lc.oy + lc.oz*lc.oz + r.cx*r.cx + r.cy*r.cy + r.cz*r.cz;
        const double r2wd = r.radius * r.radius * 1.001 + 1.0e-5 * qq + 1.0e-6 + 1.0e-14 * w2;
        s_rxp[tid][0] = (float)qx; s_rxp[tid][1] = (float)qy; s_rxp[tid][2] = (float)qz; s_rxp[tid][RTS_RXP_QQW] = (float)qq * 1.000001f;
        s_rxp[tid][RTS_RXP_R2W] = (float)r2wd;
        s_rxp[tid][RTS_RXP_QN] = (float)sqrt(qq);
        const double th_c = 0.5 * (r.minTheta + r.maxTheta), th_h = 0.5 * (r.maxTheta - r.minTheta);
        const bool ok = r.minPhi >= -RTS_PI / 2 && r.maxPhi <= RTS_PI / 2 && r.minPhi < r.maxPhi && th_h > 0.0 && th_h < 1.5 && r.radius > 0.0 && isfinite(th_c) && isfinite(qq);
        s_rxp[tid][RTS_RXP_QQ] = (float)qq; s_rxp[tid][RTS_RXP_R2] = (float)(r.radius * r.radius);
        s_rxp[tid][RTS_RXP_E2] = (float)(2.0e-6 * qq + 1.0e-6 * r.radius * r.radius + 1.0e-14 * w2 + 1.0e-12);
        s_rxp[tid][RTS_RXP_CT] = (float)cos(th_c); s_rxp[tid][RTS_RXP_ST] = (float)sin(th_c); s_rxp[tid][RTS_RXP_CH] = (float)cos(th_h);
        s_rxp[tid][RTS_RXP_SLO] = (float)(r.radius * sin(r.minPhi)); s_rxp[tid][RTS_RXP_SHI] = (float)(r.radius * sin(r.maxPhi));
        s_rxp[tid][RTS_RXP_OK] = (ok && a.rx_window_screen) ? 1.0f : 0.0f;
        s_rxp[tid][RTS_RXP_RW] = (float)(sqrt(r2wd) * 1.000001);
    }
    __syncthreads();
    uint32_t n_nodes = 0, n_tris = 0;
    bool hard_overflow = false;
    const bool mask_on = a.pmask != nullptr && lc.mask.n != 0 && a.pmask[(size_t)lc.mask.n * lc.mask.n / 32u] == 0u;
    const bool pre_on = lc.W > 1 && a.n_rx <= RTS_RX_LDS && (mask_on || a.n_prims == 0) && a.pre_filter;
    const uint32_t max_refr = REFR ? 2u : 0u;
    const uint32_t D = a.max_refl + max_refr;

    unsigned long long tl_t0 = 0;
    if (!COOP && a.timeline && tid == 0) { tl_t0 = wall_clock64(); a.timeline[(size_t)blockIdx.x * 2] = tl_t0; }
    const uint32_t n_tiles = (a.n_rays + 63u) / 64u;
    const uint32_t lane = tid & 63u;
    const uint32_t wave_u = __builtin_amdgcn_readfirstlane(tid >> 6);
    const uint32_t stripe = __builtin_amdgcn_readfirstlane((blockIdx.x * (RTS_BLOCK / 64u) + (tid >> 6)) % RTS_TILE_CTRS);
    const uint32_t n_head = (a.tile_head && a.tile_order) ? min(min(__builtin_amdgcn_readfirstlane(a.tile_head[0]), n_tiles), 16384u) : 0u;
    constexpr uint32_t CG = (COOP && VERS) ? (uint32_t)RTS_COOP_GROUP : 64u;
    constexpr uint32_t RPU = 64u / CG;
    const uint32_t n_units = COOP ? CG * n_head : n_tiles - n_head;
    __shared__ int32_t s_exch[COOP ? RTS_BLOCK : 1];
    __shared__ uint32_t s_lane_scratch[COUNT ? 2 * (RTS_BLOCK / 64) : 1];
    __shared__ uint32_t s_walk[2 * (RTS_BLOCK / 64)];
    const RtsUnitLds ul = {s_stack, s_exch, s_first, s_path, s_n, s_rx, s_rxp, s_lane_scratch, s_walk};
    unsigned long long lane_stats[11] = {0ull, 0ull, 0ull, 0ull, 0ull, 0ull, 0ull, 0ull, 0ull, 0ull, 0ull};
#define RTS_OPAQUE_S(x) ({ uint32_t o_ = (x); asm volatile("" : "+s"(o_)); o_; })
    uint32_t coop_x = 0, coop_sweep = 0, coop_len = 0;
    const uint32_t coop_P = COOP ? a.coop_spread : 1u, coop_G = RTS_XCD / coop_P;
#define RTS_COOP_LEN(x) (n_head > ((x) % coop_G) ? (n_head - ((x) % coop_G) + coop_G - 1u) / coop_G : 0u)
    if (COOP) {
        asm volatile("s_getreg_b32 %0, hwreg(HW_REG_XCC_ID)" : "=s"(coop_x));
        coop_x &= (RTS_XCD - 1u);
        coop_len = RTS_COOP_LEN(coop_x);
    }
    const uint32_t S = COOP ? (uint32_t)RTS_SEG_STRIPES : (uint32_t)RTS_TILE_CTRS;
#define RTS_LSTRIPE (COOP ? (stripe & (RTS_SEG_STRIPES - 1u)) : RTS_OPAQUE_S(stripe))
    const uint32_t per_stripe_all = (n_units + RTS_TILE_CTRS - 1u) / RTS_TILE_CTRS;
    constexpr bool BATCHABLE = !COOP && !KEEP_ALL;
    __shared__ uint32_t s_sched[(RTS_BLOCK / 64) * 8];
#define RTS_SCHED(k) s_sched[RTS_OPAQUE_S(wave_u) * 8u + (k)]
    const uint32_t single_draws_nobatch = per_stripe_all >= 1024u ? per_stripe_all / 4u : per_stripe_all;
    if (BATCHABLE) {
        uint32_t k_dead = per_stripe_all;
        if (a.batch_dead != 0u && pre_on) {
            if (a.batch_dead == 2u) k_dead = 0u;
            else if (a.tile_live && a.tile_order) {
                const uint32_t lv = __builtin_amdgcn_readfirstlane(a.tile_live[0]);
                if (lv) { const uint32_t v_dead = lv - 1u > n_head ? lv - 1u - n_head : 0u; k_dead = min(per_stripe_all, v_dead > stripe ? (v_dead - stripe + RTS_TILE_CTRS - 1u) / RTS_TILE_CTRS : 0u); }
            }
        }
        const uint32_t s1 = min(single_draws_nobatch, k_dead);
        if (lane == 0) { RTS_SCHED(0) = s1; RTS_SCHED(1) = (k_dead - s1 + 3u) / 4u; RTS_SCHED(2) = k_dead; }
    }
    const uint32_t single_draws_all = single_draws_nobatch;
    __shared__ uint32_t s_draw[RTS_BLOCK / 64];
    uint32_t draw_next = 0;
#define RTS_DRAW() { const uint32_t dv_ = atomicAdd(&a.tile_ctr[(COOP ? RTS_OFF_CTR_COOP : 0) + ((COOP ? coop_x * S : 0u) + RTS_LSTRIPE) * RTS_TILE_CTR_STRIDE], 1u); if (COUNT || KEEP_ALL) s_draw[wave_u] = dv_; else draw_next = dv_; }
    if (lane == 0) RTS_DRAW()
    for (;;) {
      const uint32_t draw = __builtin_amdgcn_readfirstlane((COUNT || KEEP_ALL) ? s_draw[wave_u] : draw_next);
      const uint32_t per_stripe = COOP ? (coop_len * (CG / coop_P) + RTS_SEG_STRIPES - 1u) / RTS_SEG_STRIPES : per_stripe_all;
      const uint32_t single_draws = COOP ? per_stripe : (BATCHABLE ? __builtin_amdgcn_readfirstlane(RTS_SCHED(0)) : single_draws_all);
      const uint32_t four_draws = BATCHABLE ? __builtin_amdgcn_readfirstlane(RTS_SCHED(1)) : 0u, k_dead = BATCHABLE ? __builtin_amdgcn_readfirstlane(RTS_SCHED(2)) : 0u;
      const bool batch = BATCHABLE && draw >= single_draws + four_draws;
      const uint32_t k0 = draw < single_draws ? draw : (batch ? k_dead + 64u * (draw - single_draws - four_draws) : single_draws + 4u * (draw - single_draws));
      const uint32_t kn = draw < single_draws ? 1u : (batch ? 64u : (BATCHABLE ? min(4u, k_dead - k0) : 4u));
      if (k0 >= per_stripe) {
          if (COOP) {
              if (++coop_sweep >= RTS_XCD) break;
              coop_x = (coop_x + 1u) & (RTS_XCD - 1u);
              coop_len = RTS_COOP_LEN(coop_x);
              if (lane == 0) RTS_DRAW()
              continue;
          }
          break;
      }
      const uint32_t seg_len = COOP ? coop_len * (CG / coop_P) : n_units;
      const bool ahead = draw >= single_draws;
      if (ahead && lane == 0) RTS_DRAW()
     if (BATCHABLE && batch) {
         const uint64_t vl = (uint64_t)(k0 + lane) * S + RTS_LSTRIPE;
         bool maybe = false;
         if (k0 + lane < per_stripe && vl < seg_len) {
             const uint32_t tp = (uint32_t)vl + n_head;
             const uint32_t tj = a.tile_order ? a.tile_order[tp] : ((tp & 1u) ? (n_tiles - 1u) / 2u + (tp + 1u) / 2u : (n_tiles - 1u) / 2u - tp / 2u);
             const uint32_t* pm_ = a.pmask; asm volatile("" : "+s"(pm_));
             maybe = rts_tile_maybe(lc, tj, a.n_rays, a.n_prims > 0, mask_on, pm_, a.n_rx, s_rxp);
             if (!maybe) {
                 atomicAdd(&s_n[tid], min(64u, a.n_rays - tj * 64u));
                 if (a.tile_cost) a.tile_cost[tj] = 1u;
             }
         }
         const unsigned long long live_m = __ballot(maybe);
         if (lane == 0) { RTS_SCHED(3) = (uint32_t)live_m; RTS_SCHED(4) = (uint32_t)(live_m >> 32); }
     }
     for (uint32_t kb = 0; kb < kn; kb++) {
      uint32_t kq = kb;
      if (BATCHABLE && kn == 64u) {
          const uint32_t m_lo = __builtin_amdgcn_readfirstlane(RTS_SCHED(3)), m_hi = __builtin_amdgcn_readfirstlane(RTS_SCHED(4));
          if ((m_lo | m_hi) == 0u) break;
          kq = m_lo ? (uint32_t)__builtin_ctz(m_lo) : 32u + (uint32_t)__builtin_ctz(m_hi);
          if (lane == 0) { if (m_lo) RTS_SCHED(3) = m_lo & (m_lo - 1u); else RTS_SCHED(4) = m_hi & (m_hi - 1u); }
      }
      const uint64_t vloc64 = (uint64_t)(k0 + kq) * S + RTS_LSTRIPE;
      if (vloc64 >= seg_len) break;
      uint32_t vpos = (uint32_t)vloc64;
      if (COOP) {
          const uint32_t per = CG / coop_P, j = (uint32_t)vloc64 / per, i = (uint32_t)vloc64 - j * per, h = (coop_x % coop_G) + coop_G * j;
          vpos = (h << 6) | ((((coop_x - h) & (RTS_XCD - 1u)) / coop_G) + coop_P * i);
      }
      const bool coop_unit = COOP;
      const uint32_t tpos = COOP ? (vpos >> 6) : vpos + n_head;
      const uint32_t tile = a.tile_order ? a.tile_order[tpos] : ((tpos & 1u) ? (n_tiles - 1u) / 2u + (tpos + 1u) / 2u : (n_tiles - 1u) / 2u - tpos / 2u);
      const uint32_t slot = coop_unit ? tile * 64u + (vpos & 63u) * RPU + lane / CG : tile * 64u + lane;
      uint32_t pre = 0u;
      if (!COOP && !KEEP_ALL && pre_on) {
          bool pre_target = a.n_prims > 0, pre_rx = a.n_rx > 0;
          if (slot < a.n_rays) rts_prefilter(lc, slot, mask_on, a.pmask, a.n_rx, s_rxp, pre_target, pre_rx);
          if (!__any(slot < a.n_rays && (pre_target || pre_rx))) {
              if (slot < a.n_rays) atomicAdd(&s_n[tid], 1u);
              if (lane == 0 && a.tile_cost) a.tile_cost[tile] = 1u;
              continue;
          }
          pre = 1u | (pre_target ? 2u : 0u) | (pre_rx ? 4u : 0u);
      }
      const long long tile_t0 = wall_clock64();
      const long long tile_s0 = COUNT ? clock64() : 0;
      if (!COOP) atomicAnd(&s_n[tid], 0x003fffffu);
      if (!COOP && lane == 0) { const uint32_t z_ = RTS_OPAQUE_S(0u); s_walk[2u * wave_u] = z_; s_walk[2u * wave_u + 1u] = z_; }
      const unsigned long long tl_tile = (COUNT && a.timeline && lane == 0) ? wall_clock64() : 0ULL;
      if (slot < a.n_rays) {
          rts_trace_unit<COUNT, KEEP_ALL, REFR, COOP, VERS>(a, lc, ul, tid, gtid, lane, slot, pre_on, mask_on, D, max_refr, origin, n_nodes, n_tris, hard_overflow, lane_stats, pre);
      }
      const unsigned long long dt = RTS_COST_UNITS(wall_clock64() - tile_t0);
      if (COUNT && !COOP && lane == 0 && clock64() - tile_s0 < 0) {
          uint32_t xcc; asm volatile("s_getreg_b32 %0, hwreg(HW_REG_XCC_ID)" : "=s"(xcc));
          atomicAdd(&a.counters[14], 1ULL); atomicOr(&a.counters[14], 1ULL << (56u + (xcc & 7u)));
      }
      bool long_walks = false, longish_walks = false;
      if (!COOP && a.tile_cost && dt >= a.coop_min_cost) {
          const uint32_t wsteps = __builtin_amdgcn_readfirstlane(s_walk[2u * wave_u]), walks = __builtin_amdgcn_readfirstlane(s_walk[2u * wave_u + 1u]);
          long_walks = walks != 0u && (unsigned long long)wsteps >= (unsigned long long)a.coop_walk_steps * walks;
          longish_walks = walks != 0u && (unsigned long long)wsteps >= (unsigned long long)a.coop_walk_steps_lo * walks;
      }
      if (lane == 0) {
          if (a.tile_cost && dt >= (1ULL << 26)) atomicAdd(&a.counters[12], 1ULL);
          if (a.tile_cost && dt < (1ULL << 26)) {
              if (COOP) { atomicAdd(&a.tile_cost[tile], ((unsigned int)(dt > 0x00fffffeULL ? 0x00fffffeULL : dt) + 1u) * RPU); if ((vpos & 63u) == 0u) atomicOr(&a.tile_cost[tile], 0x80000000u); }
              else a.tile_cost[tile] = ((unsigned int)(dt > 0x3ffffffeULL ? 0x3ffffffeULL : dt) + 1u) | (long_walks ? 0x80000000u : 0u) | (longish_walks ? 0x40000000u : 0u);
          }
          if (COUNT && a.timeline && !coop_unit) { a.timeline[(size_t)gridDim.x * 2 + tile] = wall_clock64() - tl_tile; a.timeline[(size_t)gridDim.x * 2 + n_tiles + tile] = tl_tile; }
      }
     }
      if (!ahead && lane == 0) RTS_DRAW()
    }
    if (!COOP && a.timeline && tid == 0) a.timeline[(size_t)blockIdx.x * 2 + 1] = wall_clock64();

    if (COUNT && !COOP && lane == 0 && lane_stats[0]) { atomicAdd(&a.counters[8], lane_stats[0]); atomicAdd(&a.counters[9], lane_stats[1]); atomicAdd(&a.counters[10], lane_stats[2]); }
    if (COUNT && (lane & (CG - 1u)) == 0u && lane_stats[3]) atomicAdd(&a.counters[11], lane_stats[3]);
    if (COUNT && !COOP && lane == 0 && lane_stats[4]) atomicAdd(&a.counters[15], lane_stats[4]);
    if (COUNT && lane_stats[5]) atomicAdd(&a.counters[16], lane_stats[5]);
    if (COUNT && !COOP && lane_stats[8]) { atomicAdd(&a.counters[17], lane_stats[6]); atomicAdd(&a.counters[18], lane_stats[7]); atomicAdd(&a.counters[19], lane_stats[8]); }
    if (COUNT && !COOP && lane_stats[10]) { atomicAdd(&a.counters[20], lane_stats[9]); atomicAdd(&a.counters[21], lane_stats[10]); }
    const uint32_t tid_e = (wave_u << 6) | __builtin_amdgcn_mbcnt_hi(~0u, __builtin_amdgcn_mbcnt_lo(~0u, 0u));
    unsigned long long n_seg = s_n[tid_e] & 0x003fffffu, n_shaded = s_n[RTS_BLOCK + tid_e] & RTS_SHADED_MASK, n_spill = s_n[2 * RTS_BLOCK + tid_e], n_nodes_w = n_nodes, n_tris_w = n_tris;
    for (int off = 32; off > 0; off >>= 1) {
        n_seg += __shfl_down(n_seg, off); n_shaded += __shfl_down(n_shaded, off);
        if (COUNT) { n_nodes_w += __shfl_down(n_nodes_w, off); n_tris_w += __shfl_down(n_tris_w, off); }
        n_spill += __shfl_down(n_spill, off);
    }
    __syncthreads();
    unsigned long long* s_cnt = reinterpret_cast<unsigned long long*>(s_stack);
    const int wave = (int)wave_u;
    if ((tid_e & 63) == 0) {
        s_cnt[wave * 8 + 1] = n_seg; s_cnt[wave * 8 + 2] = n_shaded; s_cnt[wave * 8 + 3] = COUNT ? n_nodes_w : 0ULL;
        s_cnt[wave * 8 + 4] = COUNT ? n_tris_w : 0ULL; s_cnt[wave * 8 + 5] = n_spill;
    }
    const bool any_overflow = __syncthreads_or(hard_overflow ? 1 : 0) != 0;
    if (tid_e >= 1 && tid_e <= 6) {
        unsigned long long v = 0;
        if (tid_e <= 5) { for (int w = 0; w < RTS_BLOCK / 64; w++) v += s_cnt[w * 8 + tid_e]; }
        else v = any_overflow ? 1ULL : 0ULL;
        a.block_counters[((size_t)(COOP ? a.total_threads / RTS_BLOCK : 0u) + blockIdx.x) * 8 + tid_e] = v;
    }
}

__global__ void k_sum_counters(const unsigned long long* __restrict__ block_counters, unsigned int n_blocks, unsigned long long* __restrict__ counters, const uint32_t* __restrict__ head_count,
                               unsigned long long* __restrict__ host_cnt)
{
    __shared__ unsigned long long s[256];
    const uint32_t t = threadIdx.x;
#define RTS_LD64(p) __hip_atomic_load((p), __ATOMIC_RELAXED, __HIP_MEMORY_SCOPE_AGENT)
    if (t == 7) { const unsigned long long h = head_count ? (unsigned long long)__hip_atomic_load(head_count, __ATOMIC_RELAXED, __HIP_MEMORY_SCOPE_AGENT) : 0ULL; counters[7] = h; host_cnt[7] = h; }
    if (t == 0) host_cnt[0] = RTS_LD64(&counters[0]);
    if ((t >= 8 && t <= 12) || (t >= 14 && t <= 21)) host_cnt[t] = RTS_LD64(&counters[t]);
    const unsigned int k = t & 7u, lane = t >> 3;
    unsigned long long v = 0;
    unsigned long long poisoned = 0;
    if (k >= 1 && k <= 6) for (unsigned int b = lane; b < n_blocks; b += 32) { const unsigned long long x = RTS_LD64(&block_counters[(size_t)b * 8 + k]); if (x == ~0ULL) poisoned++; else v += x; }
    s[t] = v;
    if (k == 1 && poisoned) { atomicAdd(&counters[13], poisoned); __threadfence(); }
    __syncthreads();
    if (t >= 1 && t <= 6) {
        unsigned long long sum = 0;
        for (unsigned int l = 0; l < 32; l++) sum += s[l * 8 + t];
        counters[t] = sum; host_cnt[t] = sum;
    }
    if (t == 13) host_cnt[13] = RTS_LD64(&counters[13]);
#undef RTS_LD64
}

template <bool COOP>
static void rts_trace_dispatch(const RtsTraceArgs& a, bool count_traversal, unsigned grid, hipStream_t st)
{
    const int sel = (a.max_refr ? 4 : 0) | (a.keep_all ? 2 : 0) | (count_traversal ? 1 : 0);
    if (!COOP && a.nodes4v) {
        switch (sel) {
            case 0: k_trace<false, false, false, false, true><<<grid, RTS_BLOCK, 0, st>>>(a); break;
            case 1: k_trace<true, false, false, false, true><<<grid, RTS_BLOCK, 0, st>>>(a); break;
            case 2: k_trace<false, true, false, false, true><<<grid, RTS_BLOCK, 0, st>>>(a); break;
            case 3: k_trace<true, true, false, false, true><<<grid, RTS_BLOCK, 0, st>>>(a); break;
            case 4: k_trace<false, false, true, false, true><<<grid, RTS_BLOCK, 0, st>>>(a); break;
            case 5: k_trace<true, false, true, false, true><<<grid, RTS_BLOCK, 0, st>>>(a); break;
            case 6: k_trace<false, true, true, false, true><<<grid, RTS_BLOCK, 0, st>>>(a); break;
            default: k_trace<true, true, true, false, true><<<grid, RTS_BLOCK, 0, st>>>(a); break;
        }
        return;
    }
    if (COOP && a.nodes4v && a.coop_versions && sel < 2) {
        if (sel == 0) k_trace<false, false, false, true, true><<<grid, RTS_BLOCK, 0, st>>>(a);
        else k_trace<true, false, false, true, true><<<grid, RTS_BLOCK, 0, st>>>(a);
        return;
    }
    switch (sel) {
        case 0: k_trace<false, false, false, COOP><<<grid, RTS_BLOCK, 0, st>>>(a); break;
        case 1: k_trace<true, false, false, COOP><<<grid, RTS_BLOCK, 0, st>>>(a); break;
        case 2: k_trace<false, true, false, COOP><<<grid, RTS_BLOCK, 0, st>>>(a); break;
        case 3: k_trace<true, true, false, COOP><<<grid, RTS_BLOCK, 0, st>>>(a); break;
        case 4: k_trace<false, false, true, COOP><<<grid, RTS_BLOCK, 0, st>>>(a); break;
        case 5: k_trace<true, false, true, COOP><<<grid, RTS_BLOCK, 0, st>>>(a); break;
        case 6: k_trace<false, true, true, COOP><<<grid, RTS_BLOCK, 0, st>>>(a); break;
        default: k_trace<true, true, true, COOP><<<grid, RTS_BLOCK, 0, st>>>(a); break;
    }
}

int rts_trace_launch(RtsContext* c, const RtsTraceArgs& a, bool count_traversal, unsigned coop_grid)
{
    if (a.n_rays == 0) {
        k_sum_counters<<<1, 256, 0, c->tstream_now>>>(a.block_counters, 0u, a.counters, nullptr, c->pin.dev->cnt);
        RTS_HIP(hipGetLastError());
        return RTS_OK;
    }
    const unsigned grid = a.total_threads / RTS_BLOCK;
    hipStream_t st = c->tstream_now;
    if (count_traversal) RTS_HIP(hipMemsetAsync(a.block_counters, 0xff, sizeof(unsigned long long) * 8 * ((size_t)grid + coop_grid), st));
    if (coop_grid) {
        if (!c->cstream) { int lo = 0, hi = 0; (void)hipDeviceGetStreamPriorityRange(&lo, &hi); RTS_HIP(hipStreamCreateWithPriority(&c->cstream, hipStreamNonBlocking, lo)); }
        RTS_HIP(hipEventRecord(c->ev_coop[0], st));
        RTS_HIP(hipStreamWaitEvent(c->cstream, c->ev_coop[0], 0));
        rts_trace_dispatch<true>(a, count_traversal, coop_grid, c->cstream);
        RTS_HIP(hipEventRecord(c->ev_coop[1], c->cstream));
    }
    rts_trace_dispatch<false>(a, count_traversal, grid, st);
    if (coop_grid) RTS_HIP(hipStreamWaitEvent(st, c->ev_coop[1], 0));
    k_sum_counters<<<1, 256, 0, st>>>(a.block_counters, grid + coop_grid, a.counters, a.tile_head_all, c->pin.dev->cnt);
    RTS_HIP(hipGetLastError());
    return RTS_OK;
}

void rts_trace_preload()
{
    hipFuncAttributes fa;
    (void)hipFuncGetAttributes(&fa, reinterpret_cast<const void*>(&k_trace<false, false, false, false>));
    (void)hipFuncGetAttributes(&fa, reinterpret_cast<const void*>(&k_trace<false, false, false, true>));
}
```

Before: 27280.

## Add per-quadrant horizon sectors to skip more target traversals

Replaces the two float horizon slopes per primitive with four 8-bit sector slopes per side, built from in-plane azimuth quadrants. When the global slope test fails, the trace kernel checks the quadrant matching the ray's in-plane direction and can still skip re-traversing the same target. This aims to cut BVH traversal for bounce rays, at the cost of a slightly heavier horizon build and a few extra dot products per hit. The quantised encoding rounds upward, which keeps the test conservative.

New measurement: 28290, median of 6. +3.7%, better.

```diff
diff --git a/include/rts_amd.h b/include/rts_amd.h
--- a/include/rts_amd.h
+++ b/include/rts_amd.h
@@ -34,6 +34,7 @@
 #define RTS_FLAG_HOST_BUILD 16u
 #define RTS_FLAG_NO_PREFILTER 8u
 #define RTS_FLAG_NO_HORIZON 32u
+#define RTS_FLAG_NO_HORIZON_SECTORS 64u
 #define RTS_FLAG_COUNT_TRAVERSAL 2u
 
 typedef struct RtsMesh {
@@ -128,6 +129,7 @@
 } RtsSceneInfo;
 int rts_scene_info(RtsHandle h, RtsSceneInfo* out);
 int rts_get_horizon(RtsHandle h, float* out, uint32_t capacity_prims);
+int rts_get_horizon_sectors(RtsHandle h, uint8_t* out, uint32_t capacity_prims);
 
 int rts_trace_pulse(RtsHandle h, const RtsPulse* pulse);
 
diff --git a/rts_amd/_lib.py b/rts_amd/_lib.py
--- a/rts_amd/_lib.py
+++ b/rts_amd/_lib.py
@@ -15,6 +15,7 @@
 RTS_FLAG_HOST_BUILD = 16
 RTS_FLAG_NO_PREFILTER = 8
 RTS_FLAG_NO_HORIZON = 32
+RTS_FLAG_NO_HORIZON_SECTORS = 64
 RTS_MAX_DEPTH = 16
 RTS_BASE_USE_ROWS = 0xffffffffffffffff
 
@@ -367,7 +368,7 @@
            "rts_finalise_uniform", "rts_trace_pulse_end_uniform", "rts_aggregate", "rts_group_count", "rts_get_groups", "rts_get_aggregated",
            "rts_merge_groups", "rts_groups_to_responses", "rts_kernel_wrapper", "rts_vertex_rotation",
            "rts_rotation_matrix", "rts_rect_mesh", "rts_sphere_mesh", "rts_file_mesh", "rts_rx_sphere", "rts_get_bvh",
-           "rts_build_id", "rts_bind_host_to_device", "rts_get_lane_stats", "rts_get_walk_stats", "rts_get_horizon", "rts_self_test_math", "rts_cube_attach", "rts_cube_accumulate", "rts_cube_get", "rts_cube_accumulate_paths", "rts_cube_doppler", "rts_cube_doppler_get", "rts_plan_cpi", "rts_cube_reduce", "rts_kernel_wrapper_on",
+           "rts_build_id", "rts_bind_host_to_device", "rts_get_lane_stats", "rts_get_walk_stats", "rts_get_horizon", "rts_get_horizon_sectors", "rts_self_test_math", "rts_cube_attach", "rts_cube_accumulate", "rts_cube_get", "rts_cube_accumulate_paths", "rts_cube_doppler", "rts_cube_doppler_get", "rts_plan_cpi", "rts_cube_reduce", "rts_kernel_wrapper_on",
            "rts_received_prefetch", "rts_received_view", "rts_finalise_values", "rts_aggregated_view", "rts_build_hierarchy_host",
            "rts_tile_records_get", "rts_tile_records_set", "rts_deal_tiles", "rts_set_tile_list",
            "rts_set_patterns", "rts_finalise_patterns", "rts_trace_pulse_end_patterns", "rts_pattern_eval",
@@ -439,7 +440,7 @@
         "rts_get_bvh": [vp, vp, vp, vp, u32, u32, vp],
         "rts_cube_attach": [vp, C.POINTER(RtsCubeParams), vp],
         "rts_cube_accumulate": [vp, u32, dbl, dbl],
-        "rts_cube_get": [vp, vp, u64], "rts_get_lane_stats": [vp, vp], "rts_get_walk_stats": [vp, vp, C.c_uint32], "rts_get_horizon": [vp, vp, u32], "rts_bind_host_to_device": [C.c_int, C.POINTER(C.c_int)],
+        "rts_cube_get": [vp, vp, u64], "rts_get_lane_stats": [vp, vp], "rts_get_walk_stats": [vp, vp, C.c_uint32], "rts_get_horizon": [vp, vp, u32], "rts_get_horizon_sectors": [vp, vp, u32], "rts_bind_host_to_device": [C.c_int, C.POINTER(C.c_int)],
         "rts_cube_accumulate_paths": [vp, u32], "rts_cube_doppler": [vp, u32, vp], "rts_cube_doppler_get": [vp, vp, u64],
         "rts_plan_cpi": [u64, u32, u32, u32, u32, u32, u32, vp, u32, C.POINTER(u32)],
         "rts_cube_reduce": [vp, u32, C.c_int],
diff --git a/rts_amd/api.py b/rts_amd/api.py
--- a/rts_amd/api.py
+++ b/rts_amd/api.py
@@ -706,11 +706,11 @@
 
 class Tracer:
 
-    def __init__(self, width, max_refl, max_refr=0, smooth=True, device=0, keep_all=False, count_traversal=False, device_build=None, pre_filter=True, horizon=True):
+    def __init__(self, width, max_refl, max_refr=0, smooth=True, device=0, keep_all=False, count_traversal=False, device_build=None, pre_filter=True, horizon=True, horizon_sectors=True):
         p = L.RtsParams(width, max_refl, max_refr, 1 if smooth else 0, device,
                         (L.RTS_FLAG_KEEP_ALL_RAYS if keep_all else 0) | (L.RTS_FLAG_COUNT_TRAVERSAL if count_traversal else 0) |
                         (0 if device_build is None else (L.RTS_FLAG_DEVICE_BUILD if device_build else L.RTS_FLAG_HOST_BUILD)) |
-                         (0 if pre_filter else L.RTS_FLAG_NO_PREFILTER) | (0 if horizon else L.RTS_FLAG_NO_HORIZON))
+                         (0 if pre_filter else L.RTS_FLAG_NO_PREFILTER) | (0 if horizon else L.RTS_FLAG_NO_HORIZON) | (0 if horizon_sectors else L.RTS_FLAG_NO_HORIZON_SECTORS))
         self.h = C.c_void_p()
         check(L.lib().rts_create(C.byref(p), C.byref(self.h)))
         self.width = width; self.max_refl = max_refl; self.depth = max_refl + (2 if max_refr else 0)
@@ -744,9 +744,14 @@
         check(L.lib().rts_get_horizon(self.h, ptr(out), int(n_prims)))
         return out
 
+    def horizon_sectors(self, n_prims):
+        out = np.zeros((int(n_prims), 2, 4), np.uint8)
+        check(L.lib().rts_get_horizon_sectors(self.h, ptr(out), int(n_prims)))
+        return out
+
     def walk_stats(self):
-        ls = (C.c_uint64 * 11)()
-        check(L.lib().rts_get_walk_stats(self.h, ls, 11))
+        ls = (C.c_uint64 * 12)()
+        check(L.lib().rts_get_walk_stats(self.h, ls, 12))
         return [int(v) for v in ls]
 
     def share_scene(self, other):
diff --git a/rts_amd/csrc/rts_api.hip b/rts_amd/csrc/rts_api.hip
--- a/rts_amd/csrc/rts_api.hip
+++ b/rts_amd/csrc/rts_api.hip
@@ -499,7 +499,7 @@
     a.recv_records = c->d_recv.p; a.all_records = c->d_all.p; a.counters = c->p_counters; a.block_counters = c->d_block_counters.p; a.dir_hist = c->d_dir_hist.p;
     a.hit_prim = c->d_hit_prim.p; a.hit_t = c->d_hit_t.p; a.stack_ovf = c->d_stack_ovf.p; a.child = c->d_child.p;
     a.rx_window_screen = c->tune.rx_window_screen ? 1u : 0u;
-    a.horizon = (c->params.flags & RTS_FLAG_NO_HORIZON) ? 0u : 1u;
+    a.horizon = (c->params.flags & RTS_FLAG_NO_HORIZON) ? 0u : (c->params.flags & RTS_FLAG_NO_HORIZON_SECTORS) ? 1u : 2u;
     a.coop_versions = c->tune.coop_versions ? 1u : 0u;
     a.tile_ctr = c->d_tile_ctr.p;
     return RTS_OK;
diff --git a/rts_amd/csrc/rts_bvh.hip b/rts_amd/csrc/rts_bvh.hip
--- a/rts_amd/csrc/rts_bvh.hip
+++ b/rts_amd/csrc/rts_bvh.hip
@@ -111,7 +111,7 @@
                                                 double ox, double oy, double oz, RtsMaskFrame f, uint32_t* __restrict__ mask,
                                                 const RtsTargetMotion* __restrict__ motion = nullptr, uint32_t prim_blocks = 0, const double* __restrict__ n_local = nullptr,
                                                 double* __restrict__ n_world = nullptr, const uint32_t* __restrict__ n_targ = nullptr, uint32_t n_normals = 0,
-                                                const float* __restrict__ horizon = nullptr)
+                                                const uint32_t* __restrict__ horizon = nullptr)
 {
     __shared__ __attribute__((aligned(16))) uint32_t s_raw[MASK ? sizeof(RtsMaskLds) / 4 : 1];
     if (PLACE && blockIdx.x >= prim_blocks) {
@@ -138,7 +138,7 @@
             RtsLeafTri L;
             L.p0x = p[0]; L.p0y = p[1]; L.p0z = p[2]; L.e0x = e0.x; L.e0y = e0.y; L.e0z = e0.z; L.e1x = e1.x; L.e1y = e1.y; L.e1z = e1.z;
             L.nx = nn.x; L.ny = nn.y; L.nz = nn.z;
-            L.prim = g; L.targ = prim_targ[g]; L.hz[0] = horizon ? horizon[2*(size_t)g] : 1.0f; L.hz[1] = horizon ? horizon[2*(size_t)g+1] : 1.0f;
+            L.prim = g; L.targ = prim_targ[g]; L.hz[0] = horizon ? horizon[2*(size_t)g] : 0xffffffffu; L.hz[1] = horizon ? horizon[2*(size_t)g+1] : 0xffffffffu;
             leaves[g] = L;
         }
     }
diff --git a/rts_amd/csrc/rts_horizon.hip b/rts_amd/csrc/rts_horizon.hip
--- a/rts_amd/csrc/rts_horizon.hip
+++ b/rts_amd/csrc/rts_horizon.hip
@@ -1,4 +1,6 @@
+#include <algorithm>
 #include <cmath>
+#include <vector>
 #include "rts_internal.h"
 #include "rts_ray_ops.h"
 
@@ -6,7 +8,7 @@
 #define RTS_HZ_WORK_CAP (1ull << 31)
 #define RTS_HZ_SLICES 8u
 
-struct RtsHzPrim { double cx, cy, cz, r, nx, ny, nz, d; };
+struct RtsHzPrim { double cx, cy, cz, r, nx, ny, nz, d, ux, uy, uz, wx, wy, wz; };
 struct RtsHzBlk { double cx, cy, cz, r; uint32_t tlo, thi; };
 
 __global__ void k_hz_prims(const uint32_t* __restrict__ order, const uint32_t* __restrict__ tri_vidx, const double* __restrict__ verts, const uint32_t* __restrict__ prim_targ,
@@ -33,6 +35,9 @@
     q.r = sqrt(r2) * (1.0 + 1e-12);
     const double inv = good ? 1.0 / nl : 0.0;
     q.nx = nn.x * inv; q.ny = nn.y * inv; q.nz = nn.z * inv; q.d = q.nx * p[0] + q.ny * p[1] + q.nz * p[2];
+    const double iu = (good && l0 > 0.0) ? 1.0 / l0 : 0.0;
+    q.ux = e0.x * iu; q.uy = e0.y * iu; q.uz = e0.z * iu;
+    q.wx = q.ny * q.uz - q.nz * q.uy; q.wy = q.nz * q.ux - q.nx * q.uz; q.wz = q.nx * q.uy - q.ny * q.ux;
     hp[i] = q;
 }
 
@@ -56,25 +61,47 @@
     return s;
 }
 
+__device__ __forceinline__ uint32_t hz_reach(double pu, double pw, double dist, double R)
+{
+    const double m = R + (dist + R) * (RTS_HZ_EPS_AZ + 1e-9);
+    const bool up = !(pu + m < 0.0), un = !(m - pu < 0.0), wp = !(pw + m < 0.0), wn = !(m - pw < 0.0);
+    return (up && wp ? 1u : 0u) | (un && wp ? 2u : 0u) | (up && wn ? 4u : 0u) | (un && wn ? 8u : 0u);
+}
+
+__device__ __forceinline__ uint32_t hz_encode(double s)
+{
+    if (!(s < 1.0)) return 255u;
+    uint32_t b = s > 0.0 ? (uint32_t)ceil(s * 255.0) : 0u;
+    if (b > 255u) b = 255u;
+    while (b < 255u && RTS_HZ_DECODE(b) < s) b++;
+    return b;
+}
+
 __global__ void __launch_bounds__(256) k_hz_main(const uint32_t* __restrict__ order, const uint32_t* __restrict__ prim_targ, uint32_t n, uint32_t n_blocks, const RtsHorizonMesh* __restrict__ mesh,
                                                  const uint32_t* __restrict__ mesh_off, const RtsHzPrim* __restrict__ hp, const RtsHzBlk* __restrict__ hb, const double* __restrict__ pv,
-                                                 uint32_t* __restrict__ horizon)
+                                                 uint32_t* __restrict__ acc)
 {
     const uint32_t i = blockIdx.x * blockDim.x + threadIdx.x, slice = blockIdx.y;
     if (i >= n) return;
     const uint32_t g = order[i], t = prim_targ[g];
-    double sp = 0.0, sm = 0.0;
-    if (mesh_off[t]) { sp = 1.0; sm = 1.0; }
+    double s[8] = {0.0, 0.0, 0.0, 0.0, 0.0, 0.0, 0.0, 0.0};
+    if (mesh_off[t]) { for (int k = 0; k < 8; k++) s[k] = 1.0; }
     else {
         const RtsHzPrim T = hp[i];
         const double h0 = RTS_HZ_H0 * mesh[t].extent, rho = RTS_HZ_RHO * mesh[t].extent;
-        for (uint32_t b = slice; b < n_blocks && !(sp >= 1.0 && sm >= 1.0); b += RTS_HZ_SLICES) {
+        for (uint32_t b = slice; b < n_blocks; b += RTS_HZ_SLICES) {
+            bool closed = true;
+            for (int k = 0; k < 8; k++) closed = closed && s[k] >= 1.0;
+            if (closed) break;
             const RtsHzBlk B = hb[b];
             if (t < B.tlo || t > B.thi) continue;
             const double hc = T.nx * B.cx + T.ny * B.cy + T.nz * B.cz - T.d;
             const double dx = B.cx - T.cx, dy = B.cy - T.cy, dz = B.cz - T.cz;
-            const double gap = sqrt(dx * dx + dy * dy + dz * dz) - B.r - T.r - rho;
-            if (hz_raise(sp, hc + B.r, gap, h0) <= sp && hz_raise(sm, -hc + B.r, gap, h0) <= sm) continue;
+            const double dist = sqrt(dx * dx + dy * dy + dz * dz), gap = dist - B.r - T.r - rho;
+            const uint32_t reach = hz_reach(dx * T.ux + dy * T.uy + dz * T.uz, dx * T.wx + dy * T.wy + dz * T.wz, dist, B.r + T.r + rho);
+            bool raises = false;
+            for (int k = 0; k < 4; k++) if (reach >> k & 1u) raises = raises || hz_raise(s[k], hc + B.r, gap, h0) > s[k] || hz_raise(s[4 + k], -hc + B.r, gap, h0) > s[4 + k];
+            if (!raises) continue;
             const uint32_t j0 = b * RTS_HZ_BLOCK, j1 = min(n, j0 + RTS_HZ_BLOCK);
             for (uint32_t j = j0; j < j1; j++) {
                 if (j == i || prim_targ[order[j]] != t) continue;
@@ -82,16 +109,24 @@
                 const double* u = pv + (size_t)j * 9;
                 const double a0 = T.nx * u[0] + T.ny * u[1] + T.nz * u[2] - T.d, a1 = T.nx * u[3] + T.ny * u[4] + T.nz * u[5] - T.d, a2 = T.nx * u[6] + T.ny * u[7] + T.nz * u[8] - T.d;
                 const double ex = U.cx - T.cx, ey = U.cy - T.cy, ez = U.cz - T.cz;
-                const double pg = sqrt(ex * ex + ey * ey + ez * ez) - U.r - T.r - rho;
-                sp = hz_raise(sp, fmax(a0, fmax(a1, a2)), pg, h0);
-                sm = hz_raise(sm, fmax(-a0, fmax(-a1, -a2)), pg, h0);
+                const double pd = sqrt(ex * ex + ey * ey + ez * ez), pg = pd - U.r - T.r - rho;
+                const uint32_t pr = hz_reach(ex * T.ux + ey * T.uy + ez * T.uz, ex * T.wx + ey * T.wy + ez * T.wz, pd, U.r + T.r + rho);
+                const double hp_ = fmax(a0, fmax(a1, a2)), hm_ = fmax(-a0, fmax(-a1, -a2));
+                for (int k = 0; k < 4; k++) if (pr >> k & 1u) { s[k] = hz_raise(s[k], hp_, pg, h0); s[4 + k] = hz_raise(s[4 + k], hm_, pg, h0); }
             }
         }
     }
-    float fp = (float)sp, fm = (float)sm;
-    if ((double)fp < sp) fp = __uint_as_float(__float_as_uint(fp) + 1u);
-    if ((double)fm < sm) fm = __uint_as_float(__float_as_uint(fm) + 1u);
-    atomicMax(&horizon[2 * (size_t)g], __float_as_uint(fminf(fp, 1.0f))); atomicMax(&horizon[2 * (size_t)g + 1], __float_as_uint(fminf(fm, 1.0f)));
+    for (int k = 0; k < 8; k++) { const uint32_t b = hz_encode(s[k]); if (b) atomicMax(&acc[8 * (size_t)g + k], b); }
+}
+
+__global__ void k_hz_pack(const uint32_t* __restrict__ acc, uint32_t n, uint32_t* __restrict__ horizon)
+{
+    const uint32_t g = blockIdx.x * blockDim.x + threadIdx.x;
+    if (g >= n) return;
+    for (int side = 0; side < 2; side++) {
+        const uint32_t* a = acc + 8 * (size_t)g + 4 * side;
+        horizon[2 * (size_t)g + side] = (a[0] & 0xffu) | (a[1] & 0xffu) << 8 | (a[2] & 0xffu) << 16 | (a[3] & 0xffu) << 24;
+    }
 }
 
 int rts_horizon_build(RtsContext* c, RtsScene* ns, const RtsSceneFlat& flat)
@@ -108,16 +143,17 @@
         ns->hz[t].extent = E; ns->hz[t].h0 = RTS_HZ_H0 * E; ns->hz[t].rho = RTS_HZ_RHO * E;
         if (!(E > 0.0) || !std::isfinite(E) || (unsigned long long)ns->meshes[t].n_tris * n_blocks > RTS_HZ_WORK_CAP) off[t] = 1u;
     }
-    DevBuf<RtsHorizonMesh> d_mesh; DevBuf<uint32_t> d_off; DevBuf<RtsHzPrim> d_hp; DevBuf<RtsHzBlk> d_hb; DevBuf<double> d_pv;
-    RTS_HIP(d_mesh.reserve(n_targets)); RTS_HIP(d_off.reserve(n_targets)); RTS_HIP(d_hp.reserve(n)); RTS_HIP(d_hb.reserve(n_blocks)); RTS_HIP(d_pv.reserve((size_t)n * 9));
+    DevBuf<RtsHorizonMesh> d_mesh; DevBuf<uint32_t> d_off; DevBuf<RtsHzPrim> d_hp; DevBuf<RtsHzBlk> d_hb; DevBuf<double> d_pv; DevBuf<uint32_t> d_acc;
+    RTS_HIP(d_mesh.reserve(n_targets)); RTS_HIP(d_off.reserve(n_targets)); RTS_HIP(d_hp.reserve(n)); RTS_HIP(d_hb.reserve(n_blocks)); RTS_HIP(d_pv.reserve((size_t)n * 9)); RTS_HIP(d_acc.reserve((size_t)n * 8));
     RTS_HIP(ns->d_horizon.reserve((size_t)n * 2));
     RTS_HIP(hipStreamSynchronize(c->stream));
     RTS_HIP(hipMemcpy(d_mesh.p, ns->hz.data(), sizeof(RtsHorizonMesh) * n_targets, hipMemcpyHostToDevice));
     RTS_HIP(hipMemcpy(d_off.p, off.data(), sizeof(uint32_t) * n_targets, hipMemcpyHostToDevice));
     k_hz_prims<<<(n + 255u) / 256u, 256, 0, c->stream>>>(ns->d_prim_order.p, ns->d_tri_vidx.p, ns->d_verts_local.p, ns->d_prim_targ.p, n, d_mesh.p, d_off.p, d_hp.p, d_pv.p);
     k_hz_blocks<<<(n_blocks + 255u) / 256u, 256, 0, c->stream>>>(ns->d_prim_order.p, ns->d_prim_targ.p, n, n_blocks, d_hp.p, d_hb.p);
-    RTS_HIP(hipMemsetAsync(ns->d_horizon.p, 0, sizeof(float) * 2 * (size_t)n, c->stream));
-    k_hz_main<<<dim3((n + 255u) / 256u, RTS_HZ_SLICES), 256, 0, c->stream>>>(ns->d_prim_order.p, ns->d_prim_targ.p, n, n_blocks, d_mesh.p, d_off.p, d_hp.p, d_hb.p, d_pv.p, reinterpret_cast<uint32_t*>(ns->d_horizon.p));
+    RTS_HIP(hipMemsetAsync(d_acc.p, 0, sizeof(uint32_t) * 8 * (size_t)n, c->stream));
+    k_hz_main<<<dim3((n + 255u) / 256u, RTS_HZ_SLICES), 256, 0, c->stream>>>(ns->d_prim_order.p, ns->d_prim_targ.p, n, n_blocks, d_mesh.p, d_off.p, d_hp.p, d_hb.p, d_pv.p, d_acc.p);
+    k_hz_pack<<<(n + 255u) / 256u, 256, 0, c->stream>>>(d_acc.p, n, ns->d_horizon.p);
     RTS_HIP(hipGetLastError());
     RTS_HIP(hipMemcpyAsync(off.data(), d_off.p, sizeof(uint32_t) * n_targets, hipMemcpyDeviceToHost, c->stream));
     RTS_HIP(hipStreamSynchronize(c->stream));
@@ -125,13 +161,37 @@
     return RTS_OK;
 }
 
+static int hz_fetch(RtsContext* c, const char* who, const void* out, uint32_t capacity_prims, std::vector<uint32_t>& w)
+{
+    if (!out) { rts_set_error("%s: null argument", who); return RTS_ERR_INVALID; }
+    const RtsScene* sc = c->scene;
+    if (capacity_prims < sc->n_prims) { rts_set_error("%s: capacity too small (%u primitives)", who, sc->n_prims); return RTS_ERR_CAPACITY; }
+    RTS_HIP(hipStreamSynchronize(c->stream));
+    w.resize(2 * (size_t)sc->n_prims);
+    if (sc->n_prims) RTS_HIP(hipMemcpy(w.data(), sc->d_horizon.p, sizeof(uint32_t) * 2 * (size_t)sc->n_prims, hipMemcpyDeviceToHost));
+    return RTS_OK;
+}
+
 extern "C" int rts_get_horizon(RtsHandle c, float* out, uint32_t capacity_prims)
 {
     CHECK_HANDLE(c);
-    if (!out) { rts_set_error("rts_get_horizon: null argument"); return RTS_ERR_INVALID; }
-    const RtsScene* sc = c->scene;
-    if (capacity_prims < sc->n_prims) { rts_set_error("rts_get_horizon: capacity too small (%u primitives)", sc->n_prims); return RTS_ERR_CAPACITY; }
-    RTS_HIP(hipStreamSynchronize(c->stream));
-    if (sc->n_prims) RTS_HIP(hipMemcpy(out, sc->d_horizon.p, sizeof(float) * 2 * (size_t)sc->n_prims, hipMemcpyDeviceToHost));
+    std::vector<uint32_t> w;
+    const int rc = hz_fetch(c, "rts_get_horizon", out, capacity_prims, w); if (rc != RTS_OK) return rc;
+    for (size_t k = 0; k < w.size(); k++) {
+        const uint32_t b = std::max(std::max(w[k] & 0xffu, w[k] >> 8 & 0xffu), std::max(w[k] >> 16 & 0xffu, w[k] >> 24));
+        const double s = RTS_HZ_DECODE(b);
+        float f = b == 255u ? 1.0f : (float)s;
+        if ((double)f < s) f = std::nextafterf(f, 2.0f);
+        out[k] = f;
+    }
     return RTS_OK;
 }
+
+extern "C" int rts_get_horizon_sectors(RtsHandle c, uint8_t* out, uint32_t capacity_prims)
+{
+    CHECK_HANDLE(c);
+    std::vector<uint32_t> w;
+    const int rc = hz_fetch(c, "rts_get_horizon_sectors", out, capacity_prims, w); if (rc != RTS_OK) return rc;
+    for (size_t k = 0; k < w.size(); k++) for (int j = 0; j < 4; j++) out[4 * k + j] = (uint8_t)(w[k] >> (8 * j) & 0xffu);
+    return RTS_OK;
+}
diff --git a/rts_amd/csrc/rts_internal.h b/rts_amd/csrc/rts_internal.h
--- a/rts_amd/csrc/rts_internal.h
+++ b/rts_amd/csrc/rts_internal.h
@@ -36,12 +36,14 @@
     double p0x, p0y, p0z, e0x, e0y, e0z, e1x, e1y, e1z, nx, ny, nz;
     uint32_t prim;
     uint32_t targ;
-    float hz[2];
+    uint32_t hz[2];
 };
 static_assert(sizeof(RtsLeafTri) == 112, "leaf size");
 #define RTS_HZ_H0 9.5367431640625e-07
 #define RTS_HZ_RHO 0.00390625
 #define RTS_HZ_DEGEN 9.5367431640625e-07
+#define RTS_HZ_EPS_AZ 0.015625
+#define RTS_HZ_DECODE(b) ((double)(b) * (1.0 / 255.0))
 #define RTS_HZ_MARGIN 0.00390625f
 struct RtsHorizonMesh { double extent, h0, rho; };
 static_assert(offsetof(RtsLeafTri, p0x) == 0 && offsetof(RtsLeafTri, p0z) == 16 && offsetof(RtsLeafTri, e0y) == 32 && offsetof(RtsLeafTri, e1x) == 48 &&
@@ -200,7 +202,7 @@
     DevBuf<RtsNode4> d_nodes4; DevBuf<uint32_t> d_leaf_prim;
     DevBuf<uint32_t> d_prim_order;
     DevBuf<RtsNode4> d_nodes4v;
-    DevBuf<float> d_horizon;
+    DevBuf<uint32_t> d_horizon;
     std::vector<RtsHorizonMesh> hz;
     double build_ms = 0; uint32_t builder = 0;
     size_t device_bytes() const {
diff --git a/rts_amd/csrc/rts_results_api.hip b/rts_amd/csrc/rts_results_api.hip
--- a/rts_amd/csrc/rts_results_api.hip
+++ b/rts_amd/csrc/rts_results_api.hip
@@ -41,8 +41,8 @@
 {
     if (!c || !out) { rts_set_error("%s: null argument", who); return RTS_ERR_INVALID; }
     CHECK_CLOSED(c);
-    const int src[11] = {8, 9, 10, 11, 15, 16, 17, 18, 19, 20, 21};
-    for (uint32_t k = 0; k < n && k < 11u; k++) out[k] = c->pin.p->cnt[src[k]];
+    const int src[12] = {8, 9, 10, 11, 15, 16, 17, 18, 19, 20, 21, 22};
+    for (uint32_t k = 0; k < n && k < 12u; k++) out[k] = c->pin.p->cnt[src[k]];
     return RTS_OK;
 }
 extern "C" int rts_get_lane_stats(RtsHandle c, uint64_t* out3) { return rts_walk_counters(c, "rts_get_lane_stats", out3, 3); }
diff --git a/rts_amd/csrc/rts_scene.hip b/rts_amd/csrc/rts_scene.hip
--- a/rts_amd/csrc/rts_scene.hip
+++ b/rts_amd/csrc/rts_scene.hip
@@ -203,7 +203,7 @@
     out->n_targets = (uint32_t)sc->meshes.size(); out->n_prims = sc->n_prims; out->n_nodes = sc->n_nodes; out->n_leaves = sc->n_leaves;
     out->handles_sharing = (uint32_t)sc->refs.load(); out->builder = sc->builder; out->build_ms = sc->build_ms;
     out->shared_device_bytes = sc->device_bytes(); out->version_bytes = sc->d_nodes4v.cap * sizeof(RtsNode4);
-    out->horizon_bytes = sc->d_horizon.cap * sizeof(float);
+    out->horizon_bytes = sc->d_horizon.cap * sizeof(uint32_t);
     out->handle_device_bytes = c->d_leaves.cap * sizeof(RtsLeafTri) + c->d_verts_world.cap * 8 + c->d_normals_world.cap * 8 + c->d_params.cap;
     return RTS_OK;
 }
diff --git a/rts_amd/csrc/rts_trace.hip b/rts_amd/csrc/rts_trace.hip
--- a/rts_amd/csrc/rts_trace.hip
+++ b/rts_amd/csrc/rts_trace.hip
@@ -285,7 +285,8 @@
 #define RTS_RXP_N 16
 struct RtsUnitLds { int32_t* stack; int32_t* exch; double* first; unsigned long long* path; uint32_t* n; const RtsRxDev* rx; const float (*rxp)[RTS_RXP_N]; uint32_t* lane_scratch; uint32_t* walk; };
 #define RTS_SKIP_SHIFT 23
-#define RTS_SHADED_MASK 0x007fffffu
+#define RTS_SECTOR_BIT 22
+#define RTS_SHADED_MASK 0x003fffffu
 struct RtsRay { dvec3 dir, prev; double rayLength, power, doppler, refx, refy; uint32_t reflDepth, refrDepth; int received; bool end, chain_start; };
 
 template <bool KEEP_ALL, bool REFR, bool COOP, uint32_t CG = 64u>
@@ -467,13 +468,23 @@
             uint32_t skip = 0u;
             if (a.horizon) {
                 const double dn = dir.x*L.nx + dir.y*L.ny + dir.z*L.nz, dl = sqrt(dir.x*dir.x + dir.y*dir.y + dir.z*dir.z), nl = sqrt(L.nx*L.nx + L.ny*L.ny + L.nz*L.nz);
-                const double c = fabs(dn) / (dl * nl), S = (double)(dn > 0.0 ? L.hz[0] : L.hz[1]);
+                const uint32_t hw = dn > 0.0 ? L.hz[0] : L.hz[1];
+                const double c = fabs(dn) / (dl * nl), S = RTS_HZ_DECODE(max(max(hw & 0xffu, (hw >> 8) & 0xffu), max((hw >> 16) & 0xffu, hw >> 24)));
                 const double ht = fabs((double)hit_t);
                 const double delta = ht * 0x1p-22 + (fmax(fmax(fabs(prev.x), fabs(prev.y)), fabs(prev.z)) + ht) * 0x1p-45;
                 const double reach = dl * (double)SCENE_EPS_R;
-                if ((c - delta / reach > S + (double)RTS_HZ_MARGIN) && (c * reach >= 2.0 * ((double)T.hz_h0 + delta)) && (4.0 * delta <= (double)T.hz_rho)) skip = L.targ + 1u;
-            }
-            atomicAnd(&s_n[RTS_BLOCK + tid], RTS_SHADED_MASK); if (skip) atomicOr(&s_n[RTS_BLOCK + tid], skip << RTS_SKIP_SHIFT);
+                const double lhs = c - delta / reach;
+                if ((c * reach >= 2.0 * ((double)T.hz_h0 + delta)) && (4.0 * delta <= (double)T.hz_rho)) {
+                    if (lhs > S + (double)RTS_HZ_MARGIN) skip = (L.targ + 1u) << 1;
+                    else if (a.horizon > 1u) {
+                        const double du = dir.x*L.e0x + dir.y*L.e0y + dir.z*L.e0z;
+                        const double dw = dir.x*(L.ny*L.e0z - L.nz*L.e0y) + dir.y*(L.nz*L.e0x - L.nx*L.e0z) + dir.z*(L.nx*L.e0y - L.ny*L.e0x);
+                        const uint32_t k = (du < 0.0 ? 1u : 0u) | (dw < 0.0 ? 2u : 0u);
+                        if (du == du && dw == dw && lhs > RTS_HZ_DECODE((hw >> (8u * k)) & 0xffu) + (double)RTS_HZ_MARGIN) skip = ((L.targ + 1u) << 1) | 1u;
+                    }
+                }
+            }
+            atomicAnd(&s_n[RTS_BLOCK + tid], RTS_SHADED_MASK); if (skip) atomicOr(&s_n[RTS_BLOCK + tid], skip << RTS_SECTOR_BIT);
         }
         {
             const size_t plane = REFR ? (size_t)chain * (a.max_refl + 1) + reflDepth : (size_t)(reflDepth - 1);
@@ -640,7 +651,7 @@
 template <bool COUNT, bool KEEP_ALL, bool REFR, bool COOP, bool VERS = false>
 __device__ __forceinline__ void rts_trace_unit(const RtsTraceArgs& a, const RtsLaunchConsts& lc, const RtsUnitLds& L_, const uint32_t tid, const uint32_t gtid, const uint32_t lane,
                                                const uint32_t slot, const bool pre_on, const bool mask_on, const uint32_t D, const uint32_t max_refr, const dvec3& origin,
-                                               uint32_t& n_nodes, uint32_t& n_tris, bool& hard_overflow, unsigned long long (&lane_stats)[11],
+                                               uint32_t& n_nodes, uint32_t& n_tris, bool& hard_overflow, unsigned long long (&lane_stats)[12],
                                                const uint32_t pre = 0u)
 {
       int32_t* const s_stack = L_.stack; int32_t* const s_exch = L_.exch; double* const s_first = L_.first; unsigned long long* const s_path = L_.path; uint32_t* const s_n = L_.n;
@@ -683,13 +694,13 @@
             const bool primary = chain == 0 && chain_start;
             const bool may_hit = primary ? may_target : a.n_prims > 0;
             uint32_t steps = 0;
-            bool escaped = false;
+            uint32_t escaped = 0u;
             if (may_hit) {
                 float t_prune = RTS_DEFAULT_TMAX;
                 for (uint32_t targ = 0; targ < a.n_targets; targ++) {
                     const RtsTargetDev& TG = a.targets[targ];
                     if (TG.root < 0) continue;
-                    if (!REFR && (s_n[RTS_BLOCK + tid] >> RTS_SKIP_SHIFT) == targ + 1u) { if (COUNT) escaped = true; continue; }
+                    if (!REFR && (s_n[RTS_BLOCK + tid] >> RTS_SKIP_SHIFT) == targ + 1u) { if (COUNT) escaped = 1u + ((s_n[RTS_BLOCK + tid] >> RTS_SECTOR_BIT) & 1u); continue; }
                     {
                         const dvec3 q = mk3(TG.cx - prev.x, TG.cy - prev.y, TG.cz - prev.z);
                         const double qq = q.x*q.x + q.y*q.y + q.z*q.z, b = q.x*dir.x + q.y*dir.y + q.z*dir.z;
@@ -736,7 +747,7 @@
                 lane_stats[3] += (unsigned long long)__popcll(__ballot(steps > 0u));
                 lane_stats[4] += (unsigned long long)__popcll(__ballot(steps == 0u)) * smax;
             }
-            if (COUNT && escaped && (!COOP || (lane & (CG - 1u)) == 0u)) lane_stats[5] += 1ull;
+            if (COUNT && escaped && (!COOP || (lane & (CG - 1u)) == 0u)) lane_stats[escaped == 1u ? 5 : 11] += 1ull;
             if (COUNT && !COOP) {
                 const unsigned long long act_ = __ballot(true);
                 if (lane == (uint32_t)(__ffsll((long long)act_) - 1)) {
@@ -820,7 +831,7 @@
     __shared__ uint32_t s_lane_scratch[COUNT ? 2 * (RTS_BLOCK / 64) : 1];
     __shared__ uint32_t s_walk[2 * (RTS_BLOCK / 64)];
     const RtsUnitLds ul = {s_stack, s_exch, s_first, s_path, s_n, s_rx, s_rxp, s_lane_scratch, s_walk};
-    unsigned long long lane_stats[11] = {0ull, 0ull, 0ull, 0ull, 0ull, 0ull, 0ull, 0ull, 0ull, 0ull, 0ull};
+    unsigned long long lane_stats[12] = {0ull, 0ull, 0ull, 0ull, 0ull, 0ull, 0ull, 0ull, 0ull, 0ull, 0ull, 0ull};
 #define RTS_OPAQUE_S(x) ({ uint32_t o_ = (x); asm volatile("" : "+s"(o_)); o_; })
     uint32_t coop_x = 0, coop_sweep = 0, coop_len = 0;
     const uint32_t coop_P = COOP ? a.coop_spread : 1u, coop_G = RTS_XCD / coop_P;
@@ -956,6 +967,7 @@
     if (COUNT && !COOP && lane == 0 && lane_stats[0]) { atomicAdd(&a.counters[8], lane_stats[0]); atomicAdd(&a.counters[9], lane_stats[1]); atomicAdd(&a.counters[10], lane_stats[2]); }
     if (COUNT && (lane & (CG - 1u)) == 0u && lane_stats[3]) atomicAdd(&a.counters[11], lane_stats[3]);
     if (COUNT && !COOP && lane == 0 && lane_stats[4]) atomicAdd(&a.counters[15], lane_stats[4]);
+    if (COUNT && lane_stats[11]) atomicAdd(&a.counters[22], lane_stats[11]);
     if (COUNT && lane_stats[5]) atomicAdd(&a.counters[16], lane_stats[5]);
     if (COUNT && !COOP && lane_stats[8]) { atomicAdd(&a.counters[17], lane_stats[6]); atomicAdd(&a.counters[18], lane_stats[7]); atomicAdd(&a.counters[19], lane_stats[8]); }
     if (COUNT && !COOP && lane_stats[10]) { atomicAdd(&a.counters[20], lane_stats[9]); atomicAdd(&a.counters[21], lane_stats[10]); }
@@ -990,7 +1002,7 @@
 #define RTS_LD64(p) __hip_atomic_load((p), __ATOMIC_RELAXED, __HIP_MEMORY_SCOPE_AGENT)
     if (t == 7) { const unsigned long long h = head_count ? (unsigned long long)__hip_atomic_load(head_count, __ATOMIC_RELAXED, __HIP_MEMORY_SCOPE_AGENT) : 0ULL; counters[7] = h; host_cnt[7] = h; }
     if (t == 0) host_cnt[0] = RTS_LD64(&counters[0]);
-    if ((t >= 8 && t <= 12) || (t >= 14 && t <= 21)) host_cnt[t] = RTS_LD64(&counters[t]);
+    if ((t >= 8 && t <= 12) || (t >= 14 && t <= 22)) host_cnt[t] = RTS_LD64(&counters[t]);
     const unsigned int k = t & 7u, lane = t >> 3;
     unsigned long long v = 0;
     unsigned long long poisoned = 0;
```
